# google-deepmind/spriteworld

Hardware: AMD Instinct MI355X
Metric: env-steps/sec (incl. 64x64 RGB render) at 8192 envs (higher is better)
Workload: dtype i32 fixed-point raster/resample + f64 state

## Files before the change

include/swb.h:

```cpp
#ifndef SWB_H_
#define SWB_H_

#include <stdint.h>

#ifdef __cplusplus
extern "C" {
#endif

#define SWB_MAX_SPRITES 64
#define SWB_MAX_TASKS 8
#define SWB_MAX_SHAPES 32
#define SWB_MAX_SHAPE_VERTS 64
#define SWB_MAX_CUTS 4
#define SWB_MAX_CELLS ((SWB_MAX_CUTS + 1) * (SWB_MAX_CUTS + 1))

enum swb_status {
  SWB_OK = 0,
  SWB_ERR_INVALID = -1,
  SWB_ERR_HIP = -2,
  SWB_ERR_NO_DEVICE = -3,
  SWB_ERR_STATE = -4
};

enum swb_action_space {
// ... 213 lines not shown
int swb_upload_shapes(swb_handle h, const double* verts, const int32_t* offsets, int32_t n_shapes);

int swb_upload_resample(swb_handle h, int32_t axis , int32_t out_size,
                        int32_t ksize, const int32_t* bounds, const int32_t* coeffs);

int swb_set_pool(swb_handle h, const swb_pool* pool);

int swb_sample_pool(swb_handle h, const swb_sampler* spec, int32_t n_entries, const int32_t* pool_base_host,
                    const int32_t* pool_len_host, uint64_t seed, uint64_t first_entry, void* stream);

int swb_resample_pool(swb_handle h, uint64_t seed, uint64_t first_entry, void* stream);

int swb_sample_pool_tree(swb_handle h, const swb_tree_sampler* spec, int32_t n_entries, const int32_t* pool_base_host,
                         const int32_t* pool_len_host, uint64_t seed, uint64_t first_entry, void* stream);

int swb_sampler_exhausted(swb_handle h, int64_t* sprites, void* stream);

int swb_get_pool(swb_handle h, const swb_pool* pool_host);

int swb_reset_all(swb_handle h, void* stream);

int swb_step(swb_handle h, const void* actions_dev, const swb_outputs* out, void* stream);

int swb_step_masked(swb_handle h, const void* actions_dev, const uint8_t* active_dev, const swb_outputs* out, void* stream);

int swb_reset_envs(swb_handle h, const uint8_t* mask_dev, void* stream);

int swb_render(swb_handle h, uint8_t* obs_dev, void* stream);

int swb_evaluate(swb_handle h, uint8_t* success_dev, void* stream);

typedef struct swb_rollout_outputs {
  double* reward;
  float* discount;
  uint8_t* step_type;
  uint8_t* success;
  uint8_t* error;
  double* x;
  double* y;
  int32_t* n_sprites;
} swb_rollout_outputs;
int swb_rollout(swb_handle h, const void* actions_dev, int32_t M, int32_t K, const swb_rollout_outputs* out, void* stream);

int swb_rollout_frames(swb_handle h, int32_t M, const int32_t* cand_dev, uint8_t* obs_dev, uint8_t* error_dev, void* stream);

typedef struct swb_rollout_step_outputs {
  double* x;
  double* y;
  int32_t* n_sprites;
} swb_rollout_step_outputs;
int swb_rollout_trajectory(swb_handle h, const void* actions_dev, int32_t M, int32_t K, const swb_rollout_outputs* out,
                           const swb_rollout_step_outputs* steps, void* stream);

#define SWB_ALL_STEPS (-1)
int swb_rollout_step_frames(swb_handle h, int32_t M, int32_t step, const int32_t* cand_dev, uint8_t* obs_dev, uint8_t* error_dev,
                            void* stream);

#define SWB_CONTAINED_MAX_TRIES 1024
enum swb_action_sampling { SWB_SAMPLE_UNIFORM = 0, SWB_SAMPLE_ON_SPRITE = 1 };
typedef struct swb_sampled_actions {
  void* actions;
  double* position;
  int32_t* sprite;
  int32_t* tries;
} swb_sampled_actions;
int swb_sample_actions(swb_handle h, int32_t mode, uint64_t seed, uint64_t first_env, const swb_sampled_actions* out, void* stream);

typedef struct swb_rollout_sampled_outputs {
  void*    actions;
  int32_t* sprite;
  int32_t* tries;
} swb_rollout_sampled_outputs;
int swb_rollout_sampled(swb_handle h, int32_t mode , uint64_t seed, uint64_t first_env,
                        int32_t M, int32_t K, int32_t keep_steps, const swb_rollout_outputs* out,
                        const swb_rollout_step_outputs* steps, const swb_rollout_sampled_outputs* sampled, void* stream);

int swb_trim_run_lists(swb_handle h, int32_t* run_cap_out, void* stream);

int swb_list_stats(swb_handle h, int64_t* kept, int64_t* built, void* stream);

int swb_frame_stats(swb_handle h, int64_t* copied, int64_t* filled, int64_t* resampled, void* stream);
int swb_frame_cycles(swb_handle h, int64_t* out3, void* stream);

int swb_split_stats(swb_handle h, int64_t* whole, int64_t* bands, int64_t* whole_copies, void* stream);

int swb_factors(swb_handle h, double* factors_dev, void* stream);

int swb_get_env_state(swb_handle h, int32_t env, int32_t* out5, void* stream);
int swb_get_sprite_types(swb_handle h, int32_t env, int32_t sprite, int32_t* flags, void* stream);

int swb_get_state(swb_handle h, const swb_state* host_state, void* stream);
int swb_set_positions(swb_handle h, const double* x_host, const double* y_host, void* stream);

typedef struct swb_snapshot {
  double *x, *y;
  int32_t *n_sprites, *pool_entry, *step_count, *episode, *pool_base, *pool_len;
  uint8_t *reset_next;
} swb_snapshot;
enum swb_state_source { SWB_STATE_LIVE = 0, SWB_STATE_ROLLOUT_END = 1 };
int swb_pool_id(swb_handle h, uint64_t* id);
int swb_save_state(swb_handle h, int32_t source, const int32_t* index_dev, int32_t C, const swb_snapshot* snap, void* stream);
int swb_load_state(swb_handle h, const swb_snapshot* snap, int32_t C, const int32_t* slot_dev, uint64_t pool_id,
                   int32_t* rejected_dev, void* stream);

int swb_copy_pool(swb_handle dst, swb_handle src, const int32_t* pool_base_host, const int32_t* pool_len_host, void* stream);

enum swb_sprite_attr { SWB_ATTR_SHAPE = 0, SWB_ATTR_ANGLE = 1, SWB_ATTR_SCALE = 2 };
int swb_set_sprite_attr(swb_handle h, int32_t env, int32_t sprite, int32_t attr, double value, const double* delta,
                        const int8_t* label, void* stream);

int swb_set_sprite_cell_labels(swb_handle h, int32_t env, int32_t sprite, const int8_t* cells, void* stream);

int swb_get_sprite(swb_handle h, int32_t env, int32_t sprite, int32_t* shape, double* angle, double* scale, int32_t* n_verts,
                   double* path_xy, void* stream);

int swb_sprite_path_op(int32_t attr, double a, double b, int32_t n, const double* in_xy, double* out_xy);

typedef struct swb_variant_info {
  int32_t nw;
  int32_t ncol;
  int32_t vs;
  int32_t lds_bytes_per_wave;
  int32_t waves_per_simd;
  int32_t resample_waves_per_simd;
  int32_t n_bands;
  int32_t n_column_groups;
  int32_t run_cap;
  int32_t paint_in_cover;
  int32_t arena_units;
  int32_t large_frames;
  int32_t many_sprites;
  int32_t reserved_;
  int64_t run_list_bytes;
  int64_t frame_cache_bytes;
  int32_t split_bands;
  int32_t split_pad_;
} swb_variant_info;
int swb_variant(swb_handle h, swb_variant_info* out);
const char* swb_build_id(void);

int swb_timing_enable(swb_handle h, int32_t enable);
int swb_step_time_ms(swb_handle h, double* total_ms, int64_t* launches);
int swb_kernel_times_ms(swb_handle h, double* cover_ms, double* resample_ms, int64_t* launches);

#ifdef __cplusplus
}
#endif
#endif
```

spriteworld_amd/_abi.py:

```python
import ctypes as C

SWB_MAX_SPRITES = 64
SWB_TUNED_SPRITES = 16
SWB_MAX_TASKS = 8
SWB_MAX_SHAPES = 32
SWB_MAX_SHAPE_VERTS = 64
SWB_MAX_GROUPS = 8
SWB_MAX_CUTS = 4
SWB_MAX_CELLS = (SWB_MAX_CUTS + 1) * (SWB_MAX_CUTS + 1)
SWB_MAX_CANDIDATES = 12

ACTION_SELECT_MOVE, ACTION_DRAG_AND_DROP, ACTION_EMBODIED = 0, 1, 2
TASK_NO_REWARD, TASK_FIND_GOAL, TASK_CLUSTERING = 0, 1, 2
AGG_SUM, AGG_MAX, AGG_MIN, AGG_MEAN = 0, 1, 2, 3
TERM_ALL, TERM_ANY = 0, 1
STEP_FIRST, STEP_MID, STEP_LAST = 0, 1, 2
ENV_ERR_DB_ZERO, ENV_ERR_DB_LABELS, ENV_ERR_SPAN_OVERFLOW = 1, 2, 4
ATTR_SHAPE, ATTR_ANGLE, ATTR_SCALE = 0, 1, 2
SAMPLE_UNIFORM, SAMPLE_ON_SPRITE = 0, 1
SWB_CONTAINED_MAX_TRIES = 1024


class SwbTask(C.Structure):
  _fields_ = [
# ... 67 lines not shown
      ('discount', C.c_void_p),
      ('step_type', C.c_void_p),
      ('success', C.c_void_p),
      ('error', C.c_void_p),
  ]


class SwbRolloutOutputs(C.Structure):
  _fields_ = [
      ('reward', C.c_void_p),
      ('discount', C.c_void_p),
      ('step_type', C.c_void_p),
      ('success', C.c_void_p),
      ('error', C.c_void_p),
      ('x', C.c_void_p),
      ('y', C.c_void_p),
      ('n_sprites', C.c_void_p),
  ]


class SwbRolloutStepOutputs(C.Structure):
  _fields_ = [
      ('x', C.c_void_p),
      ('y', C.c_void_p),
      ('n_sprites', C.c_void_p),
  ]


SWB_ALL_STEPS = -1


class SwbSampledActions(C.Structure):
  _fields_ = [
      ('actions', C.c_void_p),
      ('position', C.c_void_p),
      ('sprite', C.c_void_p),
      ('tries', C.c_void_p),
  ]


class SwbRolloutSampledOutputs(C.Structure):
  _fields_ = [
      ('actions', C.c_void_p),
      ('sprite', C.c_void_p),
      ('tries', C.c_void_p),
  ]


class SwbState(C.Structure):
  _fields_ = [
      ('x', C.c_void_p),
      ('y', C.c_void_p),
      ('n_sprites', C.c_void_p),
      ('pool_entry', C.c_void_p),
      ('step_count', C.c_void_p),
      ('reset_next', C.c_void_p),
      ('episode', C.c_void_p),
  ]


class SwbSnapshot(C.Structure):
  _fields_ = [
      ('x', C.c_void_p),
      ('y', C.c_void_p),
      ('n_sprites', C.c_void_p),
      ('pool_entry', C.c_void_p),
      ('step_count', C.c_void_p),
      ('episode', C.c_void_p),
      ('pool_base', C.c_void_p),
      ('pool_len', C.c_void_p),
      ('reset_next', C.c_void_p),
  ]


STATE_LIVE, STATE_ROLLOUT_END = 0, 1


class SwbVariantInfo(C.Structure):
  _fields_ = [('nw', C.c_int32), ('ncol', C.c_int32), ('vs', C.c_int32), ('lds_bytes_per_wave', C.c_int32),
              ('waves_per_simd', C.c_int32), ('resample_waves_per_simd', C.c_int32), ('n_bands', C.c_int32),
              ('n_column_groups', C.c_int32), ('run_cap', C.c_int32), ('paint_in_cover', C.c_int32),
              ('arena_units', C.c_int32), ('large_frames', C.c_int32), ('many_sprites', C.c_int32), ('reserved_', C.c_int32),
              ('run_list_bytes', C.c_int64), ('frame_cache_bytes', C.c_int64),
              ('split_bands', C.c_int32), ('split_pad_', C.c_int32)]


FACTOR_UNIFORM_F32, FACTOR_UNIFORM_INT, FACTOR_DISCRETE = 0, 1, 2


class SwbFactor(C.Structure):
  _fields_ = [
      ('kind', C.c_int32),
      ('n', C.c_int32),
      ('lo', C.c_double),
      ('hi', C.c_double),
      ('cand', C.c_double * SWB_MAX_CANDIDATES),
  ]


FACTOR_ORDER = ('x', 'y', 'scale', 'angle', 'c0', 'c1', 'c2', 'x_vel', 'y_vel')
SWB_N_FACTORS = len(FACTOR_ORDER)
SWB_MAX_HOLDOUTS = 2


class SwbHoldout(C.Structure):
  _fields_ = [
      ('redraw_mask', C.c_uint32),
      ('box_mask', C.c_uint32),
      ('lo', C.c_double * SWB_N_FACTORS),
      ('hi', C.c_double * SWB_N_FACTORS),
  ]


class SwbSpriteGroup(C.Structure):

  def factor(self, key):
    return self.factors[FACTOR_ORDER.index(key)]

  _fields_ = [
      ('count_min', C.c_int32),
      ('count_max', C.c_int32),
      ('factors', SwbFactor * SWB_N_FACTORS),
      ('n_holdouts', C.c_int32),
      ('reserved', C.c_int32),
      ('holdouts', SwbHoldout * SWB_MAX_HOLDOUTS),
      ('n_shapes', C.c_int32),
      ('shapes', C.c_int32 * SWB_MAX_CANDIDATES),
      ('cos_a', C.c_double * SWB_MAX_CANDIDATES),
      ('sin_a', C.c_double * SWB_MAX_CANDIDATES),
      ('label', C.c_int8 * SWB_MAX_TASKS),
  ]


SWB_MAX_ALTERNATIVES = 16


class SwbAlternative(C.Structure):
  _fields_ = [
      ('n', C.c_int32),
      ('group', C.c_int32 * SWB_MAX_GROUPS),
  ]


class SwbSampler(C.Structure):
  _fields_ = [
      ('n_groups', C.c_int32),
      ('shuffle', C.c_int32),
      ('color_map', C.c_int32),
      ('n_alternatives', C.c_int32),
      ('alternatives', SwbAlternative * SWB_MAX_ALTERNATIVES),
      ('deg_cos', C.c_double * 360),
      ('deg_sin', C.c_double * 360),
      ('groups', SwbSpriteGroup * SWB_MAX_GROUPS),
  ]


SWB_TREE_MAX_LEAVES, SWB_TREE_MAX_PRED_NODES, SWB_TREE_MAX_PREDS, SWB_TREE_MAX_OPS = 64, 128, 64, 128
SWB_TREE_MAX_CHOICES, SWB_TREE_MAX_STACK, SWB_TREE_MAX_CLUSTERS = 16, 32, 16
SWB_F_SHAPE = SWB_N_FACTORS
SWB_TREE_N_FACTORS = SWB_N_FACTORS + 1
TREE_FACTOR_ORDER = FACTOR_ORDER + ('shape',)
SWB_TREE_DEFAULT_MAX_TRIES = 10000
PRED_LEAF, PRED_AND, PRED_OR, PRED_ANDNOT, PRED_TRUE = 0, 1, 2, 3, 4
OP_DRAW, OP_CHOOSE, OP_JUMP, OP_TEST = 0, 1, 2, 3


class SwbTreeLeaf(C.Structure):
# ... 35 lines not shown
      ('target', C.c_int32 * SWB_MAX_CANDIDATES),
      ('cdf', C.c_double * SWB_MAX_CANDIDATES),
  ]


class SwbTreeGroup(C.Structure):
  _fields_ = [
      ('count_min', C.c_int32),
      ('count_max', C.c_int32),
      ('first_op', C.c_int32),
      ('n_ops', C.c_int32),
      ('defaults', C.c_double * SWB_TREE_N_FACTORS),
      ('default_cos', C.c_double),
      ('default_sin', C.c_double),
  ]


class SwbTreeTask(C.Structure):
  _fields_ = [
      ('kind', C.c_int32),
      ('n_preds', C.c_int32),
      ('pred', C.c_int16 * SWB_TREE_MAX_CLUSTERS),
  ]


class SwbTreeSampler(C.Structure):
  _fields_ = [
      ('n_groups', C.c_int32),
      ('shuffle', C.c_int32),
      ('color_map', C.c_int32),
      ('n_alternatives', C.c_int32),
      ('alternatives_weighted', C.c_int32),
      ('max_tries', C.c_int32),
      ('n_leaves', C.c_int32),
      ('n_pred_nodes', C.c_int32),
      ('n_preds', C.c_int32),
      ('n_ops', C.c_int32),
      ('n_choices', C.c_int32),
      ('n_tasks', C.c_int32),
      ('alternatives', SwbAlternative * SWB_MAX_ALTERNATIVES),
      ('alternative_cdf', C.c_double * SWB_MAX_ALTERNATIVES),
      ('deg_cos', C.c_double * 360),
      ('deg_sin', C.c_double * 360),
      ('groups', SwbTreeGroup * SWB_MAX_GROUPS),
      ('tasks', SwbTreeTask * SWB_MAX_TASKS),
      ('choices', SwbTreeChoice * SWB_TREE_MAX_CHOICES),
      ('preds', SwbTreePred * SWB_TREE_MAX_PREDS),
      ('pred_nodes', SwbPredNode * SWB_TREE_MAX_PRED_NODES),
      ('ops', SwbTreeOp * SWB_TREE_MAX_OPS),
      ('leaves', SwbTreeLeaf * SWB_TREE_MAX_LEAVES),
  ]


_P, _h, _p, _i32, _u64, _f64 = C.POINTER, C.c_void_p, C.c_void_p, C.c_int32, C.c_uint64, C.c_double

PROTOTYPES = {
    'swb_last_error': (C.c_char_p, []),
    'swb_version': (None, []),
    'swb_create': (None, [_P(SwbConfig), C.c_int, _P(C.c_void_p)]),
    'swb_destroy': (None, [_h]),
    'swb_upload_shapes': (None, [_h, _p, _p, _i32]),
    'swb_upload_resample': (None, [_h, _i32, _i32, _i32, _p, _p]),
    'swb_set_pool': (None, [_h, _P(SwbPool)]),
    'swb_sample_pool': (None, [_h, _P(SwbSampler), _i32, _p, _p, _u64, _u64, _h]),
    'swb_resample_pool': (None, [_h, _u64, _u64, _h]),
    'swb_sample_pool_tree': (None, [_h, _P(SwbTreeSampler), _i32, _p, _p, _u64, _u64, _h]),
    'swb_sampler_exhausted': (None, [_h, _P(C.c_int64), _h]),
    'swb_get_pool': (None, [_h, _P(SwbPool)]),
    'swb_reset_all': (None, [_h, _h]),
    'swb_step': (None, [_h, _p, _P(SwbOutputs), _h]),
    'swb_step_masked': (None, [_h, _p, _p, _P(SwbOutputs), _h]),
    'swb_reset_envs': (None, [_h, _p, _h]),
    'swb_render': (None, [_h, _p, _h]),
    'swb_evaluate': (None, [_h, _p, _h]),
    'swb_rollout': (None, [_h, _p, _i32, _i32, _P(SwbRolloutOutputs), _h]),
    'swb_rollout_frames': (None, [_h, _i32, _p, _p, _p, _h]),
    'swb_rollout_trajectory': (None, [_h, _p, _i32, _i32, _P(SwbRolloutOutputs), _P(SwbRolloutStepOutputs), _h]),
    'swb_rollout_step_frames': (None, [_h, _i32, _i32, _p, _p, _p, _h]),
    'swb_sample_actions': (None, [_h, _i32, _u64, _u64, _P(SwbSampledActions), _h]),
    'swb_rollout_sampled': (None, [_h, _i32, _u64, _u64, _i32, _i32, _i32, _P(SwbRolloutOutputs), _P(SwbRolloutStepOutputs),
                                   _P(SwbRolloutSampledOutputs), _h]),
    'swb_trim_run_lists': (None, [_h, _P(_i32), _h]),
    'swb_list_stats': (None, [_h, _P(C.c_int64), _P(C.c_int64), _h]),
    'swb_frame_stats': (None, [_h, _P(C.c_int64), _P(C.c_int64), _P(C.c_int64), _h]),
    'swb_split_stats': (None, [_h, _P(C.c_int64), _P(C.c_int64), _P(C.c_int64), _h]),
    'swb_frame_cycles': (None, [_h, _P(C.c_int64), _h]),
    'swb_factors': (None, [_h, _p, _h]),
    'swb_get_env_state': (None, [_h, _i32, _p, _h]),
    'swb_get_sprite_types': (None, [_h, _i32, _i32, _P(_i32), _h]),
    'swb_get_state': (None, [_h, _P(SwbState), _h]),
    'swb_set_positions': (None, [_h, _p, _p, _h]),
    'swb_pool_id': (None, [_h, _P(_u64)]),
    'swb_save_state': (None, [_h, _i32, _p, _i32, _P(SwbSnapshot), _h]),
    'swb_load_state': (None, [_h, _P(SwbSnapshot), _i32, _p, _u64, _p, _h]),
    'swb_copy_pool': (None, [_h, _h, _p, _p, _h]),
    'swb_set_sprite_attr': (None, [_h, _i32, _i32, _i32, _f64, _p, _p, _h]),
    'swb_set_sprite_cell_labels': (None, [_h, _i32, _i32, _p, _h]),
    'swb_get_sprite': (None, [_h, _i32, _i32, _p, _p, _p, _p, _p, _h]),
    'swb_sprite_path_op': (None, [_i32, _f64, _f64, _i32, _p, _p]),
    'swb_variant': (None, [_h, _P(SwbVariantInfo)]),
    'swb_build_id': (C.c_char_p, []),
    'swb_timing_enable': (None, [_h, _i32]),
    'swb_step_time_ms': (None, [_h, _P(_f64), _P(C.c_int64)]),
    'swb_kernel_times_ms': (None, [_h, _P(_f64), _P(_f64), _P(C.c_int64)]),
}


def declare(lib, tolerate_missing=False):
  for name, (restype, argtypes) in PROTOTYPES.items():
    if tolerate_missing and not hasattr(lib, name):
      continue
    fn = getattr(lib, name)
    fn.argtypes = argtypes
    if restype is not None:
      fn.restype = restype
  return lib


del _P, _h, _p, _i32, _u64, _f64
```

spriteworld_amd/csrc/swb.hip:

```cpp
#include <hip/hip_runtime.h>

#include <algorithm>
#include <atomic>
#include <cmath>
#include <cstdarg>
#include <cstdio>
#include <cstdlib>
#include <cstring>
#include <memory>
#include <string>
#include <vector>

#include "swb_kernels.hip.inc"
#include "swb_pow.hip.inc"
#include "swb_sampler.hip.inc"

extern template __global__ void swb_cover_kernel<20, false>(const swb_params);
extern template __global__ void swb_cover_kernel<20, true>(const swb_params);

namespace {

thread_local std::string g_err;

int fail(int code, const char* fmt, ...) {
// ... 27 lines not shown
  }
  int fill(const T* src, size_t n) {
    release();
    if (n == 0) n = 1;
    HIP_TRY(hipMalloc(reinterpret_cast<void**>(&ptr), n * sizeof(T)));
    count = n;
    if (src) HIP_TRY(hipMemcpy(ptr, src, n * sizeof(T), hipMemcpyHostToDevice));
    else HIP_TRY(hipMemset(ptr, 0, n * sizeof(T)));
    return 0;
  }
  int clone(const T* src, size_t n, hipStream_t st) {
    release();
    if (n == 0) n = 1;
    HIP_TRY(hipMalloc(reinterpret_cast<void**>(&ptr), n * sizeof(T)));
    count = n;
    HIP_TRY(hipMemcpyAsync(ptr, src, n * sizeof(T), hipMemcpyDeviceToDevice, st));
    return 0;
  }
  void swap(dev_buf& o) { std::swap(ptr, o.ptr); std::swap(count, o.count); }
};

std::atomic<uint64_t> g_pool_ids{0};
uint64_t next_pool_id() { return g_pool_ids.fetch_add(1) + 1; }

}

struct swb_engine {
  swb_config cfg;
  int device = 0;
  swb_params p;
  bool have_shapes = false, have_h = false, have_v = false, have_pool = false;
  int vslots = SWB_VSLOTS;
  int nbands = 1;
  bool tables_dirty = true;
  std::vector<int32_t> v_ymin_host, v_end_host, h_xmin_host, h_cnt_host;
  std::vector<int> shape_nverts;
  int ovf_lds_bytes = 0;
  void (*ovf_fn)(const swb_params) = nullptr;
  size_t lds_block = 0;
  dev_buf<double> d_shape_verts, d_shape_dmin;
  dev_buf<int32_t> d_shape_off;
  dev_buf<int32_t> d_h_xmin, d_h_cnt, d_h_tbl, d_h_pfx;
  dev_buf<int32_t> d_v_tab, d_v_end, d_v_pfx;
  dev_buf<int32_t> d_p_n;
  dev_buf<double> d_p_x, d_p_y, d_p_xv, d_p_yv, d_p_scale, d_p_ca, d_p_sa;
  dev_buf<int32_t> d_p_shape;
  dev_buf<uint32_t> d_p_rgb;
  dev_buf<int8_t> d_p_label;
  dev_buf<int8_t> d_p_cell_label;
  bool keyed = false;
  dev_buf<uint8_t> d_p_attr;
  dev_buf<int32_t> d_pool_base, d_pool_len;
  dev_buf<double> d_p_angle, d_p_color;
  dev_buf<swb_sampler> d_sampler;
  int pool_entries = 0;
  uint64_t pool_id = 0;
  bool pool_sampled = false, pool_uniform = false;
  dev_buf<swb_tree_dev> d_tree;
  dev_buf<unsigned long long> d_exhausted;
  bool pool_tree = false;
  dev_buf<double> d_x, d_y;
  dev_buf<int32_t> d_nspr, d_entry, d_step_count, d_episode;
  dev_buf<uint8_t> d_reset_next;
  dev_buf<uint32_t> d_ovf, d_ovf_bitmap;
  int ovf_slots = 0;
  dev_buf<uint32_t> d_cost_cnt;
  dev_buf<int32_t> d_cost_list;
  dev_buf<int32_t> d_ccost_list;
  bool cover_lists_filed = false;
  int launch_phase = 0;
  int launch_parity = 0;
  dev_buf<uint32_t> d_runs, d_rhdr, d_arena_head;
  dev_buf<int32_t> d_env_state;
  int arena_override = -1;
  int run_cap_worst = 0;
  bool lists_trimmed = false;
  bool lists_valid = false;
  uint32_t list_epoch = 1;
  bool no_keep_lists = false;
  dev_buf<unsigned long long> d_list_stats;
  dev_buf<uint8_t> d_frame_cache;
  int copy_cost = 0;
  dev_buf<unsigned long long> d_frame_stats;
  bool split_bands = false;
  dev_buf<unsigned long long> d_split_stats;
  dev_buf<int32_t> d_band_y0, d_band_first, d_band_lo, d_cg_lo, d_cg_hi;
  dev_buf<uint32_t> d_v_break;
  dev_buf<uint8_t> d_ov_flag;
  dev_buf<int32_t> d_ov_shape;
  dev_buf<double> d_ov_scale, d_ov_angle, d_ov_cpath;
  dev_buf<int8_t> d_ov_label;
  dev_buf<int8_t> d_ov_cell_label;
  bool timing = false;
  struct step_events { hipEvent_t e0, e1, e2; };
  std::vector<step_events> events;
  std::vector<step_events> event_pool;
  int cus = 0;
  bool no_paint_in_cover = false, force_cover_order = false;
  bool large_frames = false;
  bool many_sprites = false;
  size_t lf_scratch_budget = (size_t)256 << 20;
  dev_buf<int32_t> d_lf_hb, d_lf_hpo, d_lf_hp, d_lf_vb, d_lf_vk;
  int lf_vks = 0;
  dev_buf<uint8_t> d_lf_tmp;
  double timed_ms = 0.0, timed_cover_ms = 0.0;
  int64_t timed_launches = 0;
  dev_buf<unsigned char> d_rollout;
  dev_buf<swb_params> d_rollout_steps;
  int rollout_M = 0;
  bool rollout_stale = false;
  dev_buf<unsigned char> d_rollout_pick;
  dev_buf<unsigned char> d_rollout_traj;
  int rollout_kept_K = 0;
};

namespace {

typedef void (*kernel_fn)(const swb_params);

struct variant { int nw; kernel_fn fn, fn_ov, fn_paint, fn_paint_ov; size_t lds_fixed, outrow_bytes; };

template <int NW>
variant make_variant() {
  const size_t outrow = 528;
  kernel_fn paint = nullptr, paint_ov = nullptr;
  if constexpr (NW == 2) { paint = swb_cover_kernel<NW, false, true>; paint_ov = swb_cover_kernel<NW, true, true>; }
  return {NW, swb_cover_kernel<NW>, swb_cover_kernel<NW, true>, paint, paint_ov, (sizeof(wave_lds<NW>) + outrow + 15) & ~(size_t)15, outrow};
}

const variant kVariants[] = {make_variant<2>(), make_variant<4>(), make_variant<5>(), make_variant<10>(), make_variant<20>()};

const variant* pick_variant(int Wc) {
  for (const variant& v : kVariants)
    if (32 * v.nw >= Wc) return &v;
  return nullptr;
}

kernel_fn pick_resample(int AA, int vslots, int* vs_out) {
  if (AA == 1) { if (vs_out) *vs_out = 0; return swb_fill_kernel; }
  if (vslots <= 6) { if (vs_out) *vs_out = 6; return swb_resample_kernel<6>; }
  if (vs_out) *vs_out = 8;
  return swb_resample_kernel<8>;
}

size_t lds_per_wave(const swb_engine* h, const variant* v, int* cpath_in_masks) {
  const swb_params& p = h->p;
  const size_t cpath_bytes = (size_t)p.max_edges * 16;
  const int in_masks = (2 * (size_t)SWB_NWA(v->nw) * SWB_WAVE * 4 >= cpath_bytes) ? 1 : 0;
  if (cpath_in_masks) *cpath_in_masks = in_masks;
  return (v->lds_fixed + (((size_t)p.max_edges * sizeof(edge_rec) + 15) & ~(size_t)15) +
          (size_t)p.max_spans * SWB_WAVE * 4 + 15) & ~(size_t)15;
}

void bump_list_epoch(swb_engine* h) {
  if (++h->list_epoch == 0u) h->list_epoch = 1u;
}

int ensure_overflow_slots(swb_engine* h, kernel_fn fn, kernel_fn fn_alt, size_t lds_bytes) {
  if (h->d_ovf) return 0;
  int per_cu = 0;
  for (kernel_fn f : {fn, fn_alt}) {
    int n = 0;
    if (!f) continue;
    if (hipOccupancyMaxActiveBlocksPerMultiprocessor(&n, reinterpret_cast<const void*>(f), SWB_WAVE, lds_bytes) != hipSuccess || n < 1)
      n = 32;
    per_cu = std::max(per_cu, n);
  }
  long long slots = (long long)per_cu * h->cus;
  slots = std::min<long long>(2 * slots, (long long)h->p.N);
  slots = (slots + 31) / 32 * 32;
  h->ovf_slots = (int)slots;
  if (h->d_ovf.fill(nullptr, (size_t)slots * 64 * h->p.ovf_cap) || h->d_ovf_bitmap.fill(nullptr, (size_t)slots / 32)) return SWB_ERR_HIP;
  h->p.ovf = h->d_ovf; h->p.ovf_bitmap = h->d_ovf_bitmap; h->p.ovf_slots = h->ovf_slots;
  return 0;
}

int ensure_handoff_tables(swb_engine* h, bool need_lists = true) {
  if (!h->tables_dirty && (h->d_runs || !need_lists)) return 0;
  bump_list_epoch(h);
  swb_params& p = h->p;
  int nb = h->nbands;
  int vs = 0;
  (void)pick_resample(p.AA, h->vslots, &vs);
  auto first_in_flight = [&](int o_lo) {
    int f = o_lo;
    while (f > 0 && h->v_end_host[f - 1] >= h->v_ymin_host[o_lo]) --f;
    return f;
  };
  std::vector<int32_t> blo(1, 0);
  for (int b = 1; b < nb; ++b) {
    int want = (int)((long long)b * p.Ho / nb), best = -1;
    if (p.AA == 1) best = want;
    else
      for (int d = 0; d < p.Ho && best < 0; ++d)
        for (int c : {want + d, want - d})
          if (c > blo.back() && c < p.Ho && first_in_flight(c) % vs == 0) { best = c; break; }
    if (best > blo.back() && best < p.Ho) blo.push_back(best);
  }
  nb = (int)blo.size();
  blo.push_back(p.Ho);
  p.nbands = nb;
  std::vector<int32_t> y0(nb, 0), first(nb, 0), lo(p.ncg, 0), hi(p.ncg, 0);
  const size_t brk_words = (size_t)(p.Hc + 31) / 32 + 3;
  std::vector<uint32_t> brk(2 * brk_words, 0u);
  auto set_break = [&](int y) { if (y >= 0 && y < p.Hc) brk[y >> 5] |= 1u << (y & 31); };
  for (int b = 0; b < nb; ++b) {
    const int o_lo = blo[b];
    if (p.AA == 1) { y0[b] = o_lo; first[b] = o_lo; }
    else { y0[b] = h->v_ymin_host[o_lo]; first[b] = first_in_flight(o_lo); }
    set_break(y0[b]);
    if (y0[b] >= 0 && y0[b] < p.Hc) brk[brk_words + (y0[b] >> 5)] |= 1u << (y0[b] & 31);
  }
  if (p.AA != 1)
    for (int o = 0; o < p.Ho; ++o) set_break(h->v_end_host[o] + 1);
  for (int g = 0; g < p.ncg; ++g) {
    if (p.AA == 1) { lo[g] = 64 * g; hi[g] = std::min(64 * g + 64, p.Wo); continue; }
    lo[g] = 1 << 30; hi[g] = 0;
    for (int o = 64 * g; o < std::min(64 * g + 64, p.Wo); ++o) {
      lo[g] = std::min(lo[g], h->h_xmin_host[o]);
      hi[g] = std::max(hi[g], h->h_xmin_host[o] + h->h_cnt_host[o]);
    }
  }
  if (h->d_band_y0.fill(y0.data(), y0.size()) || h->d_band_first.fill(first.data(), first.size()) ||
      h->d_band_lo.fill(blo.data(), blo.size()) || h->d_v_break.fill(brk.data(), brk.size()) ||
      h->d_cg_lo.fill(lo.data(), lo.size()) || h->d_cg_hi.fill(hi.data(), hi.size()))
    return SWB_ERR_HIP;
  p.band_lo = h->d_band_lo;
  p.band_y0 = h->d_band_y0; p.band_first = h->d_band_first; p.v_break = h->d_v_break; p.cg_lo = h->d_cg_lo; p.cg_hi = h->d_cg_hi;
  if (!h->d_runs && need_lists) {
    const size_t fixed = (size_t)p.N * p.ncg * p.run_cap;
    size_t arena = std::max(h->lists_trimmed ? fixed / 2 : (size_t)0, (size_t)16 * h->run_cap_worst);
    if (h->arena_override >= 0) arena = (size_t)h->arena_override;
    const size_t units = fixed + arena + 4;
    if (units * 8 >= ((size_t)1 << 32))
      return fail(SWB_ERR_INVALID, "run lists of %zu MB (%d environments x %d column groups x %d units + an arena of %zu units) exceed "
                  "the 4 GB a list position can address: step fewer environments per engine", units * 8 >> 20, p.N, p.ncg, p.run_cap, arena);
    size_t free_b = 0, total_b = 0;
    if (hipMemGetInfo(&free_b, &total_b) == hipSuccess && units * 8 + (size_t)p.N * SWB_RHDR_DWORDS * 4 > free_b)
      return fail(SWB_ERR_HIP, "run lists need %zu MB of device memory (%d environments x %d column groups x %d units of 8 bytes + an "
                  "arena of %zu units), %zu MB are free", units * 8 >> 20, p.N, p.ncg, p.run_cap, arena, free_b >> 20);
    if (h->d_runs.fill(nullptr, units * 2) || h->d_rhdr.fill(nullptr, (size_t)p.N * SWB_RHDR_DWORDS) || h->d_arena_head.fill(nullptr, 2))
      return SWB_ERR_HIP;
    p.runs = h->d_runs; p.rhdr = h->d_rhdr;
    p.arena_head = h->d_arena_head;
    p.arena_base = (int64_t)fixed;
    p.arena_units = (int32_t)std::min(arena, (size_t)0x7fffffff);
  }
  h->tables_dirty = false;
  return 0;
}

int drop_run_lists(swb_engine* h) {
  if (!h->d_runs) return 0;
  HIP_TRY(hipDeviceSynchronize());
  h->d_runs.release(); h->d_rhdr.release(); h->d_arena_head.release();
  h->p.runs = nullptr; h->p.rhdr = nullptr; h->p.arena_head = nullptr;
  bump_list_epoch(h);
  h->lists_valid = false;
  h->tables_dirty = true;
  return 0;
}

int restore_run_list_reservation(swb_engine* h) {
  if (!h->lists_trimmed) return 0;
  if (int rc = drop_run_lists(h)) return rc;
  h->lists_trimmed = false;
  if (!getenv("SWB_RUN_CAP")) h->p.run_cap = h->run_cap_worst;
  return 0;
}

int flush_timing(swb_engine* h) {
  for (auto& ev : h->events) {
    HIP_TRY(hipEventSynchronize(ev.e2));
    float ms = 0.f, ms_cover = 0.f;
    HIP_TRY(hipEventElapsedTime(&ms, ev.e0, ev.e2));
    HIP_TRY(hipEventElapsedTime(&ms_cover, ev.e0, ev.e1));
    h->timed_ms += ms;
    h->timed_cover_ms += ms_cover;
    h->timed_launches += 1;
    h->event_pool.push_back(ev);
  }
  h->events.clear();
  return 0;
}


int check_ready(const swb_engine* h, const void* actions, int render_only) {
  if (!h->have_shapes) return fail(SWB_ERR_STATE, "swb_upload_shapes has not been called");
  if (!h->have_pool) return fail(SWB_ERR_STATE, "swb_set_pool has not been called");
  if (h->p.AA != 1 && !(h->have_h && h->have_v))
    return fail(SWB_ERR_STATE, "swb_upload_resample (both axes) is required when anti_aliasing > 1");
  if (!render_only && actions == nullptr) return fail(SWB_ERR_INVALID, "actions is NULL");
  return 0;
}

swb_params bind_step(const swb_engine* h, const void* actions, const swb_outputs* out, int render_only, const uint8_t* active) {
  swb_params p = h->p;
  p.actions = actions;
  p.active = active;
  p.obs = out ? out->obs : nullptr;
  p.reward = out ? out->reward : nullptr;
  p.discount = out ? out->discount : nullptr;
  p.step_type = out ? out->step_type : nullptr;
  p.success = out ? out->success : nullptr;
  p.error = out ? out->error : nullptr;
  p.render_only = render_only;
  return p;
}

void bind_view(swb_params* p, const swb_state_view* view) {
  if (!view) return;
  p->x = view->x; p->y = view->y; p->nspr = view->nspr; p->entry = view->entry; p->step_count = view->step_count;
  p->episode = view->episode; p->pool_base = view->pool_base; p->pool_len = view->pool_len; p->reset_next = view->reset_next;
}

int cover_launch_config(const swb_engine* h, const variant* v, kernel_fn fn, swb_params* p, size_t* lds_out) {
  int cpath_in_masks = 0;
  const size_t lds = lds_per_wave(h, v, &cpath_in_masks);
  p->cpath_in_masks = cpath_in_masks;
  p->lds_per_wave = (int32_t)lds;
  p->outrow_bytes = (int32_t)v->outrow_bytes;
  if (lds > 160 * 1024) return fail(SWB_ERR_INVALID, "LDS request %zu B exceeds 160 KiB", lds);
  if (lds > 64 * 1024)
    HIP_TRY(hipFuncSetAttribute(reinterpret_cast<const void*>(fn), hipFuncAttributeMaxDynamicSharedMemorySize, (int)lds));
  *lds_out = lds;
  return 0;
}

struct step_timer {
  swb_engine* h;
  hipStream_t stream;
  swb_engine::step_events ev = {nullptr, nullptr, nullptr};
  bool held = false;
  step_timer(swb_engine* h_, hipStream_t stream_) : h(h_), stream(stream_) {}
  ~step_timer() { if (held) h->event_pool.push_back(ev); }
  int begin() {
    if (!h->timing) return 0;
    if (!h->event_pool.empty()) { ev = h->event_pool.back(); h->event_pool.pop_back(); }
    else
      for (hipEvent_t* e : {&ev.e0, &ev.e1, &ev.e2}) HIP_TRY(hipEventCreate(e));
    held = true;
    HIP_TRY(hipEventRecord(ev.e0, stream));
    return 0;
  }
  int mid() {
    if (held) HIP_TRY(hipEventRecord(ev.e1, stream));
    return 0;
  }
  int end(bool counted) {
    if (!held) return 0;
    HIP_TRY(hipEventRecord(ev.e2, stream));
    if (!counted) return 0;
    held = false;
    h->events.push_back(ev);
    return h->events.size() >= 4096 ? flush_timing(h) : 0;
  }
};

bool paints_in_cover(const swb_engine* h, const variant* v, bool honour_switch = true) {
  return h->p.AA == 1 && h->p.ncg == 1 && v && v->fn_paint && !(honour_switch && h->no_paint_in_cover);
}

int launch_large(swb_engine* h, const void* actions, const swb_outputs* out, int render_only, hipStream_t stream,
                 const swb_state_view* view, const uint8_t* active);

int launch(swb_engine* h, const void* actions, const swb_outputs* out, int render_only, hipStream_t stream,
           const swb_state_view* view = nullptr, const uint8_t* active = nullptr) {
  if (h->large_frames) return launch_large(h, actions, out, render_only, stream, view, active);
  if (int rc = check_ready(h, actions, render_only)) return rc;
  const variant* v = pick_variant(h->p.Wc);
  if (!v) return fail(SWB_ERR_INVALID, "canvas %dx%d not supported", h->p.Wc, h->p.Hc);
  if (int rc = ensure_handoff_tables(h, !paints_in_cover(h, v))) return rc;
  int vs = 0;
  const kernel_fn fn2 = pick_resample(h->p.AA, h->vslots, &vs);
  swb_params p = bind_step(h, actions, out, render_only, active);
  bind_view(&p, view);
  if (p.v_tab && vs == 8) {
    p.v_tab += (size_t)p.Hc * SWB_VSLOTS;
    p.v_pfx += (size_t)(p.Hc + 1) * SWB_VSLOTS;
  }
  const bool paint = p.obs && paints_in_cover(h, v);
  const kernel_fn fn = paint ? (h->d_ov_flag ? v->fn_paint_ov : v->fn_paint) : (h->d_ov_flag ? v->fn_ov : v->fn);
  size_t lds = 0;
  if (int rc = cover_launch_config(h, v, fn, &p, &lds)) return rc;
  const kernel_fn fn_family = h->d_ov_flag ? v->fn_ov : v->fn;
  if (!h->d_ovf || (int)lds < h->ovf_lds_bytes || fn_family != h->ovf_fn) {
    if (h->d_ovf) {
      HIP_TRY(hipDeviceSynchronize());
      h->d_ovf.release(); h->d_ovf_bitmap.release();
    }
    if (int rc = ensure_overflow_slots(h, fn_family, h->d_ov_flag ? v->fn_paint_ov : v->fn_paint, lds)) return rc;
    bump_list_epoch(h);
    h->ovf_lds_bytes = (int)lds;
    h->ovf_fn = fn_family;
    p.ovf = h->p.ovf; p.ovf_bitmap = h->p.ovf_bitmap; p.ovf_slots = h->p.ovf_slots;
  }
// ... 398 lines not shown
      return fail(SWB_ERR_INVALID, "task %d: between 0 and %d position thresholds per axis supported", t, SWB_MAX_CUTS);
    for (int k = 1; k < tk.n_xcuts; ++k) if (!(tk.xcuts[k - 1] < tk.xcuts[k])) return fail(SWB_ERR_INVALID, "task %d: xcuts must ascend", t);
    for (int k = 1; k < tk.n_ycuts; ++k) if (!(tk.ycuts[k - 1] < tk.ycuts[k])) return fail(SWB_ERR_INVALID, "task %d: ycuts must ascend", t);
    if (tk.n_xcuts + tk.n_ycuts > 0) h->keyed = true;
  }
  {
    const char* lf = getenv("SWB_LARGE_FRAMES");
    const char* ms = getenv("SWB_MANY_SPRITES");
    h->many_sprites = p.S > SWB_TUNED_SPRITES || (ms && atoi(ms) != 0);
    h->large_frames = !pick_variant(p.Wc) || p.Wo > 64 * SWB_MAX_CG || (lf && atoi(lf) != 0) || h->many_sprites;
    if (const char* x = getenv("SWB_LF_SCRATCH_BYTES")) h->lf_scratch_budget = (size_t)std::max(1ll, atoll(x));
  }
  if (h->large_frames) {
    if (p.Wc > SWB_LF_MAX_CANVAS || p.Hc > SWB_LF_MAX_CANVAS)
      return fail(SWB_ERR_INVALID, "canvas %dx%d too large: at most %d px in either direction (anti_aliasing * image_size)", p.Wc, p.Hc,
                  SWB_LF_MAX_CANVAS);
    if (p.Wo > SWB_LF_MAX_COLUMNS) return fail(SWB_ERR_INVALID, "image width %d too large: at most %d columns", p.Wo, SWB_LF_MAX_COLUMNS);
  } else if (p.Hc > 65535) {
    return fail(SWB_ERR_INVALID, "canvas %dx%d too large", p.Wc, p.Hc);
  }
  const int ncg = (p.Wo + 63) / 64;
  if (!h->large_frames) p.ncg = ncg;
  const int cus = std::max(h->cus, 1);
  {
    const long long resident = (long long)cus * 4 * SWB_RS_WAVES_PER_SIMD;
    const long long tasks = (long long)p.N * ncg;
    int nb = 1;
    while (nb < SWB_MAX_BANDS && tasks * nb < resident && (p.Ho / (2 * nb) >= 16 || (p.Ho / (2 * nb) >= 8 && tasks * nb * 2 <= resident))) nb *= 2;
    if (const char* x = getenv("SWB_BANDS")) nb = std::max(1, std::min(atoi(x), (int)SWB_MAX_BANDS));
    h->nbands = std::min(nb, p.Ho);
    const bool cache_wanted = p.AA != 1 && !h->large_frames && !h->no_keep_lists && !getenv("SWB_NO_FRAME_CACHE");
    const bool cost_ordered = !getenv("SWB_NO_COST_ORDER") && p.N < (1 << 24) && !h->large_frames;
    int split = (nb == 1 && tasks <= 2 * resident && p.action_space != SWB_ACTION_EMBODIED) ? SWB_SPLIT_BANDS_DEFAULT : 0;
    if (const char* x = getenv("SWB_SPLIT_BANDS")) split = atoi(x) >= 2 ? std::min(atoi(x), (int)SWB_MAX_BANDS) : 0;
    if (getenv("SWB_BANDS") || !cache_wanted || !cost_ordered || std::min(split, p.Ho) < 2) split = 0;
    if (split) {
      h->split_bands = true;
      h->nbands = std::min(split, p.Ho);
      p.split_bands = 1;
      p.split_when = 2 * cus * 4;
      if (const char* x = getenv("SWB_SPLIT_WHEN")) p.split_when = (int32_t)std::max(0ll, std::min(atoll(x), 0x7fffffffll));
    }
  }
  const long long rs_waves = (long long)p.N * ncg * (h->split_bands ? 1 : h->nbands);
  p.cost_range0 = std::max(8 * p.Hc, SWB_KEY_BUCKETS_FITTED);
  if (!getenv("SWB_NO_COST_ORDER") && p.N < (1 << 24) && !h->large_frames) {
    p.band_tasks = (h->nbands > 1 && rs_waves >= 4ll * cus * 4 && !getenv("SWB_NO_BAND_TASKS")) ? 1 : 0;
    if (const char* x = getenv("SWB_BAND_TASKS")) p.band_tasks = (h->nbands > 1 && atoi(x) != 0) ? 1 : 0;
    if (h->split_bands) p.band_tasks = 1;
    p.cost_cap = ncg * ((p.N + SWB_COST_SHARDS - 1) / SWB_COST_SHARDS) * (p.band_tasks ? h->nbands : 1);
    std::vector<uint32_t> cnt0(5 * SWB_COST_SET + SWB_COST_WORDS, 0u);
    for (int par = 0; par < 2; ++par) cnt0[SWB_COST_WORD_SPLIT(par)] = (h->split_bands && p.split_when > 0 && (long long)p.N * ncg <= p.split_when) ? 1u : 0u;
    for (int ph = 0; ph < 3; ++ph) cnt0[SWB_COST_WORD_COVER_SHIFT(ph)] = 12;
    for (int par = 0; par < 2; ++par) {
      cnt0[SWB_COST_WORD_KEY_LO(par)] = 0u;
      cnt0[SWB_COST_WORD_KEY_RANGE(par)] = (uint32_t)p.cost_range0;
      cnt0[SWB_COST_WORD_KEY_SCALE(par)] = (uint32_t)(((unsigned long long)SWB_KEY_BUCKETS_FITTED << 16) / (uint32_t)p.cost_range0);
    }
    p.prio_div = 4;
    if (const char* x = getenv("SWB_PRIO_DIV")) p.prio_div = std::max(1, atoi(x));
    p.prio_levels = (!getenv("SWB_NO_PRIO") && rs_waves <= 2ll * cus * 4 * SWB_RS_WAVES_PER_SIMD) ? 1 : 0;
    if (!getenv("SWB_NO_COVER_PRIO")) p.prio_levels |= 2;
    const size_t ccap = (size_t)(p.N + SWB_COST_SHARDS - 1) / SWB_COST_SHARDS;
    if (h->d_cost_cnt.fill(cnt0.data(), cnt0.size()) ||
        h->d_ccost_list.fill(nullptr, (size_t)3 * SWB_COST_SHARDS * SWB_COST_BUCKETS * ccap) ||
        h->d_cost_list.fill(nullptr, (size_t)2 * SWB_COST_SHARDS * SWB_COST_BUCKETS * p.cost_cap))
      return SWB_ERR_HIP;
    p.cost_cnt = h->d_cost_cnt; p.cost_list = h->d_cost_list;
    if (!getenv("SWB_NO_COVER_ORDER")) p.ccost_list = h->d_ccost_list;
    const int per_xcd = h->cus / SWB_COST_SHARDS;
    if (per_xcd >= 2 && (per_xcd & (per_xcd - 1)) == 0 && rs_waves <= (long long)h->cus * 4 * SWB_RS_WAVES_PER_SIMD && !getenv("SWB_NO_SNAKE"))
      while ((1 << p.deal_shift) < per_xcd) ++p.deal_shift;
    if (const char* x = getenv("SWB_DEAL_SHIFT")) p.deal_shift = std::max(0, atoi(x));
  }
  h->run_cap_worst = std::max(4, p.S + 1) * p.Hc + 1;
  p.run_cap = h->run_cap_worst;
  if (const char* x = getenv("SWB_RUN_CAP")) p.run_cap = std::max(8, atoi(x));
  if (const char* x = getenv("SWB_ARENA_UNITS")) h->arena_override = std::max(0, atoi(x));
  const size_t NS = (size_t)p.N * p.S;
  if (h->d_x.fill(nullptr, NS) || h->d_y.fill(nullptr, NS) || h->d_nspr.fill(nullptr, p.N) || h->d_entry.fill(nullptr, p.N) ||
      h->d_step_count.fill(nullptr, p.N) || h->d_episode.fill(nullptr, p.N) || h->d_reset_next.fill(nullptr, p.N))
    return SWB_ERR_HIP;
  if (getenv("SWB_LIST_STATS")) {
    if (h->d_list_stats.fill(nullptr, 2) || h->d_frame_stats.fill(nullptr, 6)) return SWB_ERR_HIP;
    p.list_stats = h->d_list_stats;
    p.frame_stats = h->d_frame_stats;
    if (h->split_bands) {
      if (h->d_split_stats.fill(nullptr, 3)) return SWB_ERR_HIP;
      p.split_stats = h->d_split_stats;
    }
  }
  h->copy_cost = h->split_bands ? SWB_SPLIT_COPY_COST : SWB_COPY_COST;
  if (const char* x = getenv("SWB_COPY_COST")) h->copy_cost = std::max(0, atoi(x));
  if (p.AA != 1 && !h->large_frames && !h->no_keep_lists && !getenv("SWB_NO_FRAME_CACHE")) {
    const size_t bytes = (size_t)p.N * p.Wo * p.Ho * 3;
    if (hipMalloc(reinterpret_cast<void**>(&h->d_frame_cache.ptr), bytes) == hipSuccess) {
      h->d_frame_cache.count = bytes;
      p.frame_cache = h->d_frame_cache;
    } else {
      h->d_frame_cache.ptr = nullptr;
      (void)hipGetLastError();
    }
  }
  p.max_spans = SWB_MIN_SPANS;
  if (const char* ms = getenv("SWB_MAX_SPANS")) p.max_spans = atoi(ms) < SWB_MIN_SPANS ? SWB_MIN_SPANS : atoi(ms);
  p.span_cap = p.max_spans;
  if (const char* sc = getenv("SWB_LDS_SPAN_CAP")) p.span_cap = std::max(0, std::min(atoi(sc), p.max_spans));
  p.ovf_cap = std::min(p.Wc / 2 + 1, 32);
  p.ovf = nullptr;
  p.x = h->d_x; p.y = h->d_y; p.nspr = h->d_nspr; p.entry = h->d_entry; p.step_count = h->d_step_count;
  p.episode = h->d_episode; p.reset_next = h->d_reset_next;
  *out = owner.release();
  return SWB_OK;
}

int swb_destroy(swb_handle h) {
  if (!h) return SWB_OK;
  (void)hipSetDevice(h->device);
  for (auto* list : {&h->events, &h->event_pool})
    for (auto& ev : *list) { (void)hipEventDestroy(ev.e0); (void)hipEventDestroy(ev.e1); (void)hipEventDestroy(ev.e2); }
  delete h;
  return SWB_OK;
}

int swb_upload_shapes(swb_handle h, const double* verts, const int32_t* offsets, int32_t n_shapes) {
  if (!h || !verts || !offsets) return fail(SWB_ERR_INVALID, "null argument");
  bump_list_epoch(h);
  if (n_shapes < 1 || n_shapes > SWB_MAX_SHAPES) return fail(SWB_ERR_INVALID, "n_shapes must be in [1, %d]", SWB_MAX_SHAPES);
  HIP_TRY(hipSetDevice(h->device));
  int maxv = 0;
  for (int i = 0; i < n_shapes; ++i) {
    const int n = offsets[i + 1] - offsets[i];
    if (n < 3 || n > SWB_MAX_SHAPE_VERTS) return fail(SWB_ERR_INVALID, "shape %d has %d vertices (3..%d supported)", i, n, SWB_MAX_SHAPE_VERTS);
    if (n > maxv) maxv = n;
  }
  std::vector<double> dmin(n_shapes, 0.0);
  for (int i = 0; i < n_shapes; ++i) {
    double best = 1e300;
    for (int a = offsets[i]; a < offsets[i + 1]; ++a)
      for (int b = a + 1; b < offsets[i + 1]; ++b)
        best = std::min(best, std::hypot(verts[2 * a] - verts[2 * b], verts[2 * a + 1] - verts[2 * b + 1]));
    dmin[i] = best;
  }
  dmin.resize(SWB_MAX_SHAPES, 0.0);
  std::vector<int32_t> off_padded(offsets, offsets + n_shapes + 1);
  off_padded.resize(SWB_MAX_SHAPES + 1, offsets[n_shapes]);
  if (h->d_shape_dmin.fill(dmin.data(), dmin.size())) return SWB_ERR_HIP;
  h->p.shape_dmin = h->d_shape_dmin;
  if (h->d_shape_verts.fill(verts, (size_t)offsets[n_shapes] * 2)) return SWB_ERR_HIP;
  if (h->d_shape_off.fill(off_padded.data(), off_padded.size())) return SWB_ERR_HIP;
  h->p.shape_verts = h->d_shape_verts;
  h->p.shape_off = h->d_shape_off;
  h->p.max_verts = maxv;
  h->p.max_edges = maxv * h->p.S;
  h->shape_nverts.resize(n_shapes);
  for (int i = 0; i < n_shapes; ++i) h->shape_nverts[i] = offsets[i + 1] - offsets[i];
  h->have_shapes = true;
  return SWB_OK;
}

int swb_upload_resample(swb_handle h, int32_t axis, int32_t out_size, int32_t ksize, const int32_t* bounds,
                        const int32_t* coeffs) {
  if (!h || !bounds || !coeffs) return fail(SWB_ERR_INVALID, "null argument");
  bump_list_epoch(h);
  HIP_TRY(hipSetDevice(h->device));
  if (h->large_frames) return upload_resample_large(h, axis, out_size, ksize, bounds, coeffs);
  const swb_params& p = h->p;
  if (axis == 0) {
    if (out_size != p.Wo) return fail(SWB_ERR_INVALID, "horizontal table has %d outputs, image width is %d", out_size, p.Wo);
    std::vector<int32_t> xmin(out_size), cnt(out_size), tbl(out_size), pfx;
    std::vector<std::vector<int32_t>> uniq;
    std::vector<int32_t> uniq_off;
    for (int o = 0; o < out_size; ++o) {
      xmin[o] = bounds[2 * o]; cnt[o] = bounds[2 * o + 1];
      if (cnt[o] < 0 || cnt[o] > ksize || xmin[o] < 0 || xmin[o] + cnt[o] > p.Wc)
        return fail(SWB_ERR_INVALID, "bad horizontal bounds at %d", o);
      std::vector<int32_t> v(cnt[o] + 1, 0);
      for (int j = 0; j < cnt[o]; ++j) v[j + 1] = v[j] + coeffs[(size_t)o * ksize + j];
      int found = -1;
      for (size_t u = 0; u < uniq.size(); ++u) if (uniq[u] == v) { found = (int)u; break; }
      if (found < 0) { found = (int)uniq.size(); uniq.push_back(v); uniq_off.push_back((int32_t)pfx.size()); pfx.insert(pfx.end(), v.begin(), v.end()); }
      tbl[o] = uniq_off[found];
    }
    if (pfx.size() * 4 > 32 * 1024) return fail(SWB_ERR_INVALID, "horizontal prefix table too large (%zu entries)", pfx.size());
    if (h->d_h_xmin.fill(xmin.data(), xmin.size()) || h->d_h_cnt.fill(cnt.data(), cnt.size()) ||
        h->d_h_tbl.fill(tbl.data(), tbl.size()) || h->d_h_pfx.fill(pfx.data(), pfx.size()))
      return SWB_ERR_HIP;
    h->p.h_xmin = h->d_h_xmin; h->p.h_cnt = h->d_h_cnt; h->p.h_tbl = h->d_h_tbl; h->p.h_pfx = h->d_h_pfx;
    h->p.h_pfx_len = (int32_t)pfx.size();
    h->h_xmin_host = xmin; h->h_cnt_host = cnt;
    h->tables_dirty = true;
    h->have_h = true;
  } else if (axis == 1) {
    if (out_size != p.Ho) return fail(SWB_ERR_INVALID, "vertical table has %d outputs, image height is %d", out_size, p.Ho);
    const size_t tab_len = (size_t)p.Hc * SWB_VSLOTS;
    std::vector<int32_t> vend(out_size), vtab(2 * tab_len, 0);
    for (int r = 0; r < out_size; ++r) {
      const int ymin = bounds[2 * r], c = bounds[2 * r + 1];
      if (c < 1 || c > ksize || ymin < 0 || ymin + c > p.Hc) return fail(SWB_ERR_INVALID, "bad vertical bounds at %d", r);
      vend[r] = ymin + c - 1;
      if (r > 0 && (vend[r] < vend[r - 1] || ymin < bounds[2 * (r - 1)])) return fail(SWB_ERR_INVALID, "vertical windows are not monotone");
    }
    int used = 1;
    for (int y = 0; y < p.Hc; ++y) {
      int rf = 0;
      while (rf < out_size && vend[rf] < y) ++rf;
      for (int r = 0; r < out_size; ++r) {
        const int ymin = bounds[2 * r];
        if (y < ymin || y > vend[r]) continue;
        const int k = r - rf;
        if (k < 0 || k >= SWB_VSLOTS) return fail(SWB_ERR_INVALID, "more than %d output rows in flight at canvas row %d", SWB_VSLOTS, y);
        const int32_t cf = coeffs[(size_t)r * ksize + (y - ymin)];
        vtab[(size_t)y * SWB_VSLOTS + (r % 6)] = cf;
        vtab[tab_len + (size_t)y * SWB_VSLOTS + (r % 8)] = cf;
        if (k + 1 > used) used = k + 1;
      }
    }
    const size_t pfx_len = (size_t)(p.Hc + 1) * SWB_VSLOTS;
    std::vector<int32_t> vpfx(2 * pfx_len, 0);
    for (int t = 0; t < 2; ++t)
      for (int y = 0; y < p.Hc; ++y)
        for (int k = 0; k < SWB_VSLOTS; ++k)
          vpfx[t * pfx_len + (size_t)(y + 1) * SWB_VSLOTS + k] =
              vpfx[t * pfx_len + (size_t)y * SWB_VSLOTS + k] + vtab[t * tab_len + (size_t)y * SWB_VSLOTS + k];
    std::vector<int32_t> vend_padded(vend);
    vend_padded.push_back(0x7fffffff); vend_padded.push_back(0x7fffffff);
    if (h->d_v_tab.fill(vtab.data(), vtab.size()) || h->d_v_end.fill(vend_padded.data(), vend_padded.size()) ||
        h->d_v_pfx.fill(vpfx.data(), vpfx.size()))
      return SWB_ERR_HIP;
    h->p.v_tab = h->d_v_tab; h->p.v_end = h->d_v_end; h->p.v_pfx = h->d_v_pfx;
    h->vslots = used;
    h->v_end_host = vend;
    h->v_ymin_host.resize(out_size);
    for (int r = 0; r < out_size; ++r) h->v_ymin_host[r] = bounds[2 * r];
    h->tables_dirty = true;
    h->have_v = true;
  } else {
    return fail(SWB_ERR_INVALID, "axis must be 0 or 1");
  }
  return SWB_OK;
}

int swb_set_pool(swb_handle h, const swb_pool* pool) {
  if (!h || !pool) return fail(SWB_ERR_INVALID, "null argument");
  bump_list_epoch(h);
  HIP_TRY(hipSetDevice(h->device));
  const int P = pool->n_entries, S = h->p.S, T = h->p.n_tasks, N = h->p.N;
  if (P < 1) return fail(SWB_ERR_INVALID, "pool is empty");
  for (int i = 0; i < P; ++i)
    if (pool->n_sprites[i] < 0 || pool->n_sprites[i] > S) return fail(SWB_ERR_INVALID, "pool entry %d has %d sprites (max %d)", i, pool->n_sprites[i], S);
  for (int i = 0; i < N; ++i)
    if (pool->pool_len[i] < 1 || pool->pool_base[i] < 0 || pool->pool_base[i] + pool->pool_len[i] > P)
      return fail(SWB_ERR_INVALID, "env %d: pool range [%d, +%d) outside the pool of %d", i, pool->pool_base[i], pool->pool_len[i], P);
  const size_t PS = (size_t)P * S;
  int most_verts = -1;
  if (h->have_shapes) {
    int most = 1;
    for (int e = 0; e < P; ++e) {
      int tot = 0;
      for (int s2 = 0; s2 < pool->n_sprites[e]; ++s2) {
        const int sh = pool->shape[(size_t)e * S + s2];
        if (sh < 0 || sh >= (int)h->shape_nverts.size()) return fail(SWB_ERR_INVALID, "pool entry %d uses shape %d, %zu shapes uploaded", e, sh, h->shape_nverts.size());
        tot += h->shape_nverts[sh];
      }
      most = std::max(most, tot);
    }
    most_verts = (most + 3) & ~3;
    if (int rc = lf_check_vertices(h, most_verts, "swb_set_pool")) return rc;
  }
  std::vector<uint32_t> rgb(PS);
  for (size_t i = 0; i < PS; ++i)
    rgb[i] = (uint32_t)pool->rgb[4 * i] | ((uint32_t)pool->rgb[4 * i + 1] << 8) | ((uint32_t)pool->rgb[4 * i + 2] << 16);
  for (size_t i = 0; i < PS; ++i)
    if (pool->shape[i] < 0 || (h->have_shapes && pool->shape[i] >= SWB_MAX_SHAPES)) return fail(SWB_ERR_INVALID, "bad shape index in pool");
  int rc = 0;
  h->rollout_stale = true;
  h->pool_id = next_pool_id();
  rc |= h->d_p_n.fill(pool->n_sprites, P);
  rc |= h->d_p_x.fill(pool->x, PS); rc |= h->d_p_y.fill(pool->y, PS);
  rc |= h->d_p_xv.fill(pool->x_vel, PS); rc |= h->d_p_yv.fill(pool->y_vel, PS);
  rc |= h->d_p_scale.fill(pool->scale, PS); rc |= h->d_p_ca.fill(pool->cos_a, PS); rc |= h->d_p_sa.fill(pool->sin_a, PS);
  rc |= h->d_p_shape.fill(pool->shape, PS);
  rc |= h->d_p_rgb.fill(rgb.data(), PS);
  rc |= h->d_p_label.fill(pool->label, (size_t)P * T * S);
  if (h->keyed) {
    if (!pool->cell_label) return fail(SWB_ERR_INVALID, "a task of this handle keys on position (swb_task::n_xcuts / n_ycuts): swb_pool::cell_label is required");
    rc |= h->d_p_cell_label.fill(pool->cell_label, (size_t)P * T * S * SWB_MAX_CELLS);
  }
  rc |= h->d_p_attr.fill(pool->attr_f32, PS);
  rc |= h->d_pool_base.fill(pool->pool_base, N);
  rc |= h->d_pool_len.fill(pool->pool_len, N);
  if (pool->angle) rc |= h->d_p_angle.fill(pool->angle, PS);
  if (pool->color) rc |= h->d_p_color.fill(pool->color, PS * 3);
  if (rc) return SWB_ERR_HIP;
  bind_pool(h, pool->angle != nullptr, pool->color != nullptr);
  h->pool_entries = P;
  h->pool_sampled = false;
  if (most_verts > 0) h->p.max_edges = most_verts;
  HIP_TRY(hipMemset(h->d_reset_next, 1, N));
  HIP_TRY(hipMemset(h->d_episode, 0, sizeof(int32_t) * N));
  HIP_TRY(hipMemset(h->d_step_count, 0, sizeof(int32_t) * N));
  h->have_pool = true;
  if (int rc2 = restore_run_list_reservation(h)) return rc2;
  return SWB_OK;
}

int swb_sample_pool(swb_handle h, const swb_sampler* spec, int32_t n_entries, const int32_t* pool_base_host,
                    const int32_t* pool_len_host, uint64_t seed, uint64_t first_entry, void* stream) {
  if (!h || !spec || !pool_base_host || !pool_len_host) return fail(SWB_ERR_INVALID, "null argument");
  bump_list_epoch(h);
  HIP_TRY(hipSetDevice(h->device));
  const int P = n_entries, S = h->p.S, N = h->p.N;
  if (P < 1) return fail(SWB_ERR_INVALID, "pool is empty");
  if (h->keyed) return fail(SWB_ERR_INVALID, "a task of this handle keys on position: its labels depend on where a sprite is drawn -- sample such "
                            "generators on the host (swb_set_pool with swb_pool::cell_label)");
  if (spec->n_groups < 1 || spec->n_groups > SWB_MAX_GROUPS) return fail(SWB_ERR_INVALID, "n_groups must be in [1, %d]", SWB_MAX_GROUPS);
  if (spec->shuffle < 0) return fail(SWB_ERR_INVALID, "shuffle must be >= 0");
  if (spec->n_alternatives < 0 || spec->n_alternatives > SWB_MAX_ALTERNATIVES)
    return fail(SWB_ERR_INVALID, "n_alternatives must be in [0, %d]", SWB_MAX_ALTERNATIVES);
  for (int i = 0; i < spec->n_alternatives; ++i) {
    const swb_alternative& alt = spec->alternatives[i];
    if (alt.n < 1 || alt.n > SWB_MAX_GROUPS) return fail(SWB_ERR_INVALID, "alternative %d: 1..%d groups", i, SWB_MAX_GROUPS);
    for (int g = 0; g < alt.n; ++g)
      if (alt.group[g] < 0 || alt.group[g] >= spec->n_groups) return fail(SWB_ERR_INVALID, "alternative %d: bad group index", i);
  }
  int max_total = 0;
  for (int g = 0; g < spec->n_groups; ++g) {
    const swb_sprite_group& grp = spec->groups[g];
    if (grp.count_min < 0 || grp.count_max < grp.count_min) return fail(SWB_ERR_INVALID, "group %d: bad sprite count range", g);
    if (grp.n_shapes < 1 || grp.n_shapes > SWB_MAX_CANDIDATES)
      return fail(SWB_ERR_INVALID, "group %d: 1..%d shape candidates", g, SWB_MAX_CANDIDATES);
    for (const swb_factor* f = grp.factors; f != grp.factors + SWB_N_FACTORS; ++f) {
      if (f->kind < SWB_FACTOR_UNIFORM_F32 || f->kind > SWB_FACTOR_DISCRETE) return fail(SWB_ERR_INVALID, "group %d: bad factor kind", g);
      if (f->kind == SWB_FACTOR_DISCRETE && (f->n < 1 || f->n > SWB_MAX_CANDIDATES))
        return fail(SWB_ERR_INVALID, "group %d: Discrete factors take 1..%d candidates", g, SWB_MAX_CANDIDATES);
    }
    if (grp.factors[SWB_F_X].kind != SWB_FACTOR_UNIFORM_F32 || grp.factors[SWB_F_Y].kind != SWB_FACTOR_UNIFORM_F32)
      return fail(SWB_ERR_INVALID, "group %d: x and y must be float32 Continuous factors", g);
    const swb_factor& ang = grp.factors[SWB_F_ANGLE];
    if (ang.kind == SWB_FACTOR_UNIFORM_F32 ||
        (ang.kind == SWB_FACTOR_UNIFORM_INT && !(ang.lo >= 0.0 && ang.hi <= 360.0 && ang.lo <= ang.hi)))
      return fail(SWB_ERR_INVALID, "group %d: angle must be Discrete or integer degrees within [0, 360]", g);
    if (grp.n_holdouts < 0 || grp.n_holdouts > SWB_MAX_HOLDOUTS) return fail(SWB_ERR_INVALID, "group %d: at most %d hold-outs", g, SWB_MAX_HOLDOUTS);
    for (int i = 0; i < grp.n_holdouts; ++i)
      if (grp.holdouts[i].box_mask == 0 || (grp.holdouts[i].box_mask & ~grp.holdouts[i].redraw_mask) ||
          (grp.holdouts[i].redraw_mask >> SWB_N_FACTORS))
        return fail(SWB_ERR_INVALID, "group %d: hold-out keys must be a non-empty subset of the redrawn keys", g);
    if (spec->color_map == 1 && (grp.factors[SWB_F_C0].kind == SWB_FACTOR_UNIFORM_INT || grp.factors[SWB_F_C1].kind == SWB_FACTOR_UNIFORM_INT ||
                                 grp.factors[SWB_F_C2].kind == SWB_FACTOR_UNIFORM_INT))
      return fail(SWB_ERR_INVALID, "group %d: hsv colours must be float factors", g);
    for (int i = 0; i < grp.n_shapes; ++i)
      if (grp.shapes[i] < 0 || grp.shapes[i] >= SWB_MAX_SHAPES) return fail(SWB_ERR_INVALID, "group %d: bad shape index", g);
    max_total += grp.count_max;
  }
  if (spec->n_alternatives > 0) {
    max_total = 0;
    for (int i = 0; i < spec->n_alternatives; ++i) {
      int tot = 0;
      for (int g = 0; g < spec->alternatives[i].n; ++g) tot += spec->groups[spec->alternatives[i].group[g]].count_max;
      if (tot > max_total) max_total = tot;
    }
  }
  if (max_total > S) return fail(SWB_ERR_INVALID, "sampler can emit %d sprites (max_sprites %d)", max_total, S);
  if (h->have_shapes) {
    auto group_verts = [&](const swb_sprite_group& grp) {
      int mv = 0;
      for (int i = 0; i < grp.n_shapes; ++i)
        if (grp.shapes[i] < (int)h->shape_nverts.size()) mv = std::max(mv, h->shape_nverts[grp.shapes[i]]);
      return mv * grp.count_max;
    };
    int most = 0;
    if (spec->n_alternatives > 0) {
      for (int i = 0; i < spec->n_alternatives; ++i) {
        int tot = 0;
        for (int g = 0; g < spec->alternatives[i].n; ++g) tot += group_verts(spec->groups[spec->alternatives[i].group[g]]);
        most = std::max(most, tot);
      }
    } else {
      for (int g = 0; g < spec->n_groups; ++g) most += group_verts(spec->groups[g]);
    }
    if (int rc = lf_check_vertices(h, (std::max(most, 1) + 3) & ~3, "swb_sample_pool")) return rc;
    h->p.max_edges = (std::max(most, 1) + 3) & ~3;
  }
  for (int i = 0; i < N; ++i)
    if (pool_len_host[i] < 1 || pool_base_host[i] < 0 || pool_base_host[i] + pool_len_host[i] > P)
      return fail(SWB_ERR_INVALID, "env %d: pool range [%d, +%d) outside the pool of %d", i, pool_base_host[i], pool_len_host[i], P);
  if (alloc_sampled_pool(h, P, pool_base_host, pool_len_host) || h->d_sampler.fill(spec, 1)) return SWB_ERR_HIP;
  const swb_sampler_args a = sampler_args(h, seed, first_entry, false);
  hipStream_t st = (hipStream_t)stream;
  hipLaunchKernelGGL(swb_sample_pool_kernel, dim3((P + 255) / 256), dim3(256), 0, st, a);
  HIP_TRY(hipGetLastError());
  h->pool_tree = false;
  return finish_sampled_pool(h, pool_base_host, pool_len_host, st);
}

int swb_resample_pool(swb_handle h, uint64_t seed, uint64_t first_entry, void* stream) {
  if (!h) return fail(SWB_ERR_INVALID, "null handle");
  bump_list_epoch(h);
  if (!h->have_pool || !h->pool_sampled) return fail(SWB_ERR_STATE, "swb_sample_pool has not been called");
  if (!h->pool_uniform)
    return fail(SWB_ERR_STATE, "swb_resample_pool needs the env-major layout pool_base[n] = n * pool_len, equal pool_len");
  HIP_TRY(hipSetDevice(h->device));
  h->rollout_stale = true;
  h->pool_id = next_pool_id();
  if (h->pool_tree) return launch_tree_sampler(h, seed, first_entry, true, (hipStream_t)stream);
  const swb_sampler_args a = sampler_args(h, seed, first_entry, true);
  hipLaunchKernelGGL(swb_sample_pool_kernel, dim3((h->pool_entries + 255) / 256), dim3(256), 0, (hipStream_t)stream, a);
  HIP_TRY(hipGetLastError());
  return SWB_OK;
}

int swb_sample_pool_tree(swb_handle h, const swb_tree_sampler* spec, int32_t n_entries, const int32_t* pool_base_host,
                         const int32_t* pool_len_host, uint64_t seed, uint64_t first_entry, void* stream) {
  if (!h || !spec || !pool_base_host || !pool_len_host) return fail(SWB_ERR_INVALID, "null argument");
  bump_list_epoch(h);
  HIP_TRY(hipSetDevice(h->device));
  const int P = n_entries, S = h->p.S, N = h->p.N;
  if (P < 1) return fail(SWB_ERR_INVALID, "pool is empty");
  if (!h->cfg.pos_is_f32) return fail(SWB_ERR_INVALID, "the device sampler draws float32 positions (swb_config::pos_is_f32)");
  if (int rc = check_tree_sampler(h, spec)) return rc;
  auto over_lists = [&](auto per_group) {
    int most = 0;
    if (spec->n_alternatives > 0) {
      for (int i = 0; i < spec->n_alternatives; ++i) {
        int tot = 0;
        for (int g = 0; g < spec->alternatives[i].n; ++g) tot += per_group(spec->groups[spec->alternatives[i].group[g]]);
        most = std::max(most, tot);
      }
    } else {
      for (int g = 0; g < spec->n_groups; ++g) most += per_group(spec->groups[g]);
    }
    return most;
  };
  const int max_total = over_lists([](const swb_tree_group& grp) { return grp.count_max; });
  if (max_total > S) return fail(SWB_ERR_INVALID, "sampler can emit %d sprites (max_sprites %d)", max_total, S);
  if (h->have_shapes) {
    auto verts_of = [&](double shape) { return (int)shape < (int)h->shape_nverts.size() ? h->shape_nverts[(int)shape] : 0; };
    const int most = over_lists([&](const swb_tree_group& grp) {
      int mv = 0;
      bool drawn = false;
      for (int pc = grp.first_op; pc < grp.first_op + grp.n_ops; ++pc) {
        if (spec->ops[pc].kind != SWB_OP_DRAW || spec->leaves[spec->ops[pc].a].factor != SWB_F_SHAPE) continue;
        const swb_tree_leaf& lf = spec->leaves[spec->ops[pc].a];
        for (int i = 0; i < lf.n; ++i) mv = std::max(mv, verts_of(lf.cand[i]));
        drawn = true;
      }
      if (!drawn) mv = verts_of(grp.defaults[SWB_F_SHAPE]);
      return mv * grp.count_max;
    });
    if (int rc = lf_check_vertices(h, (std::max(most, 1) + 3) & ~3, "swb_sample_pool_tree")) return rc;
    h->p.max_edges = (std::max(most, 1) + 3) & ~3;
  }
  for (int i = 0; i < N; ++i)
    if (pool_len_host[i] < 1 || pool_base_host[i] < 0 || pool_base_host[i] + pool_len_host[i] > P)
      return fail(SWB_ERR_INVALID, "env %d: pool range [%d, +%d) outside the pool of %d", i, pool_base_host[i], pool_len_host[i], P);
  auto dev = std::make_unique<swb_tree_dev>();
  memset(dev.get(), 0, sizeof(swb_tree_dev));
  dev->spec = *spec;
  for (int t = 0; t < h->p.n_tasks; ++t) {
    const swb_task& tk = h->cfg.tasks[t];
    dev->n_xcuts[t] = tk.n_xcuts; dev->n_ycuts[t] = tk.n_ycuts;
    for (int k = 0; k < SWB_MAX_CUTS; ++k) { dev->xcuts[t][k] = tk.xcuts[k]; dev->ycuts[t][k] = tk.ycuts[k]; }
  }
  if (alloc_sampled_pool(h, P, pool_base_host, pool_len_host) || h->d_tree.fill(dev.get(), 1) ||
      (!h->d_exhausted && h->d_exhausted.fill(nullptr, 1)))
    return SWB_ERR_HIP;
  hipStream_t st = (hipStream_t)stream;
  if (int rc = launch_tree_sampler(h, seed, first_entry, false, st)) return rc;
  h->pool_tree = true;
  return finish_sampled_pool(h, pool_base_host, pool_len_host, st);
}

int swb_sampler_exhausted(swb_handle h, int64_t* sprites, void* stream) {
  if (!h || !sprites) return fail(SWB_ERR_INVALID, "null argument");
  *sprites = 0;
  if (!h->d_exhausted) return SWB_OK;
  HIP_TRY(hipSetDevice(h->device));
  HIP_TRY(hipStreamSynchronize((hipStream_t)stream));
  unsigned long long n = 0;
  HIP_TRY(hipMemcpy(&n, h->d_exhausted, sizeof(n), hipMemcpyDeviceToHost));
  *sprites = (int64_t)n;
  return SWB_OK;
}

int swb_get_pool(swb_handle h, const swb_pool* pool) {
  if (!h || !pool) return fail(SWB_ERR_INVALID, "null argument");
  if (!h->have_pool) return fail(SWB_ERR_STATE, "no pool on the device");
  if (pool->n_entries != h->pool_entries) return fail(SWB_ERR_INVALID, "pool has %d entries, not %d", h->pool_entries, pool->n_entries);
  HIP_TRY(hipSetDevice(h->device));
  HIP_TRY(hipDeviceSynchronize());
  const int P = h->pool_entries, S = h->p.S, T = h->p.n_tasks, N = h->p.N;
  const size_t PS = (size_t)P * S;
#define SWB_D2H(dst, src, count) \
  if (dst) HIP_TRY(hipMemcpy((void*)(dst), (src), (count) * sizeof(*(src)), hipMemcpyDeviceToHost))
  SWB_D2H(pool->n_sprites, h->d_p_n, (size_t)P);
  SWB_D2H(pool->x, h->d_p_x, PS); SWB_D2H(pool->y, h->d_p_y, PS);
  SWB_D2H(pool->x_vel, h->d_p_xv, PS); SWB_D2H(pool->y_vel, h->d_p_yv, PS);
  SWB_D2H(pool->scale, h->d_p_scale, PS); SWB_D2H(pool->cos_a, h->d_p_ca, PS); SWB_D2H(pool->sin_a, h->d_p_sa, PS);
// ... 272 lines not shown
    const swb_state_view picked = rollout_state_view(h->d_rollout_pick.ptr, (size_t)nk * N, S);
    hipLaunchKernelGGL(swb_rollout_pick_steps_kernel, dim3((unsigned)(((size_t)nk * N * S + 255) / 256)), dim3(256), 0, st, traj, scratch,
                       picked, cand_dev, (int)N, (int)S, (int)M, k0, nk);
    HIP_TRY(hipGetLastError());
    for (size_t kk = 0; kk < (size_t)nk; ++kk) {
      const swb_state_view chunk = advanced(picked, kk * N, kk * N, S);
      out.obs = obs_dev + kk * N * frame;
      out.error = error_dev ? error_dev + kk * N : nullptr;
      if (int rc = launch(h, nullptr, &out, 1, st, &chunk)) return rc;
    }
    return SWB_OK;
  }
  for (size_t c = 0; c < (size_t)M; ++c) {
    const swb_state_view chunk = advanced(traj, (size_t)step * NV + c * N, c * N, S);
    out.obs = obs_dev + c * N * frame;
    out.error = error_dev ? error_dev + c * N : nullptr;
    if (int rc = launch(h, nullptr, &out, 1, st, &chunk)) return rc;
  }
  return SWB_OK;
}

int swb_sample_actions(swb_handle h, int32_t mode, uint64_t seed, uint64_t first_env, const swb_sampled_actions* out, void* stream) {
  if (!h) return fail(SWB_ERR_INVALID, "null handle");
  if (mode != SWB_SAMPLE_UNIFORM && mode != SWB_SAMPLE_ON_SPRITE) return fail(SWB_ERR_INVALID, "swb_sample_actions: unknown mode %d", mode);
  if (!out || (!out->actions && !out->position && !out->sprite && !out->tries))
    return fail(SWB_ERR_INVALID, "swb_sample_actions: every output is NULL");
  if (mode == SWB_SAMPLE_UNIFORM && (out->position || out->sprite || out->tries))
    return fail(SWB_ERR_INVALID, "swb_sample_actions: position, sprite and tries are outputs of SWB_SAMPLE_ON_SPRITE only");
  if (mode == SWB_SAMPLE_ON_SPRITE) {
    if (!h->have_shapes) return fail(SWB_ERR_STATE, "swb_upload_shapes has not been called");
    if (!h->have_pool) return fail(SWB_ERR_STATE, "swb_set_pool has not been called");
  }
  HIP_TRY(hipSetDevice(h->device));
  swb_sample_actions_args a;
  memset(&a, 0, sizeof(a));
  a.mode = mode; a.seed = seed; a.first_env = first_env;
  a.actions = out->actions; a.position = out->position; a.sprite = out->sprite; a.tries = out->tries;
  hipLaunchKernelGGL(swb_sample_actions_kernel, dim3((unsigned)h->p.N), dim3(SWB_WAVE), SWB_MAX_SHAPE_VERTS * sizeof(double2),
                     (hipStream_t)stream, h->p, a);
  HIP_TRY(hipGetLastError());
  return SWB_OK;
}

int swb_trim_run_lists(swb_handle h, int32_t* run_cap_out, void* stream) {
  if (!h) return fail(SWB_ERR_INVALID, "null handle");
  HIP_TRY(hipSetDevice(h->device));
  if (h->large_frames) {
    if (run_cap_out) *run_cap_out = 0;
    return SWB_OK;
  }
  if (run_cap_out) *run_cap_out = h->p.run_cap;
  if (h->lists_trimmed || getenv("SWB_RUN_CAP") || getenv("SWB_NO_TRIM")) return SWB_OK;
  if (!h->d_runs && paints_in_cover(h, pick_variant(h->p.Wc), false)) return SWB_OK;
  if (!h->d_runs || !h->lists_valid) return fail(SWB_ERR_STATE, "swb_trim_run_lists: the last launch listed no runs (step or render first)");
  HIP_TRY(hipStreamSynchronize((hipStream_t)stream));
  const swb_params& p = h->p;
  std::vector<uint32_t> hdr((size_t)p.N * SWB_RHDR_DWORDS);
  HIP_TRY(hipMemcpy(hdr.data(), h->d_rhdr, hdr.size() * 4, hipMemcpyDeviceToHost));
  uint32_t longest = 0;
  for (int n = 0; n < p.N; ++n)
    for (int g = 0; g < p.ncg; ++g) longest = std::max(longest, hdr[(size_t)n * SWB_RHDR_DWORDS + SWB_RHDR_GROUPS + g * SWB_RHDR_GSTRIDE]);
  if (longest >= (uint32_t)p.run_cap) return SWB_OK;
  const int want = std::max(p.Hc / 2, (int)(longest + longest / 4 + 16)) + 1;
  if (want >= p.run_cap) return SWB_OK;
  if (int rc = drop_run_lists(h)) return rc;
  h->p.run_cap = want;
  h->lists_trimmed = true;
  if (int rc = ensure_handoff_tables(h)) return rc;
  if (run_cap_out) *run_cap_out = h->p.run_cap;
  return SWB_OK;
}

int swb_list_stats(swb_handle h, int64_t* kept, int64_t* built, void* stream) {
  if (!h || !kept || !built) return fail(SWB_ERR_INVALID, "null argument");
  if (!h->d_list_stats) return fail(SWB_ERR_STATE, "swb_list_stats: SWB_LIST_STATS was not set when the handle was created");
  HIP_TRY(hipSetDevice(h->device));
  HIP_TRY(hipStreamSynchronize((hipStream_t)stream));
  unsigned long long w[2] = {0ull, 0ull};
  HIP_TRY(hipMemcpy(w, h->d_list_stats, sizeof(w), hipMemcpyDeviceToHost));
  *kept = (int64_t)w[0]; *built = (int64_t)w[1];
  return SWB_OK;
}

int swb_frame_stats(swb_handle h, int64_t* copied, int64_t* filled, int64_t* resampled, void* stream) {
  if (!h || !copied || !filled || !resampled) return fail(SWB_ERR_INVALID, "null argument");
  if (!h->d_frame_stats) return fail(SWB_ERR_STATE, "swb_frame_stats: SWB_LIST_STATS was not set when the handle was created");
  HIP_TRY(hipSetDevice(h->device));
  HIP_TRY(hipStreamSynchronize((hipStream_t)stream));
  unsigned long long w[3] = {0ull, 0ull, 0ull};
  HIP_TRY(hipMemcpy(w, h->d_frame_stats, sizeof(w), hipMemcpyDeviceToHost));
  *copied = (int64_t)w[0]; *filled = (int64_t)w[1]; *resampled = (int64_t)w[2];
  return SWB_OK;
}

int swb_split_stats(swb_handle h, int64_t* whole, int64_t* bands, int64_t* whole_copies, void* stream) {
  if (!h || !whole || !bands || !whole_copies) return fail(SWB_ERR_INVALID, "null argument");
  if (!h->d_split_stats)
    return fail(SWB_ERR_STATE, "swb_split_stats: the handle is not in split-bands mode, or SWB_LIST_STATS was not set when it was created");
  HIP_TRY(hipSetDevice(h->device));
  HIP_TRY(hipStreamSynchronize((hipStream_t)stream));
  unsigned long long w[3] = {0ull, 0ull, 0ull};
  HIP_TRY(hipMemcpy(w, h->d_split_stats, sizeof(w), hipMemcpyDeviceToHost));
  *whole = (int64_t)w[0]; *bands = (int64_t)w[1]; *whole_copies = (int64_t)w[2];
  return SWB_OK;
}

int swb_frame_cycles(swb_handle h, int64_t* out3, void* stream) {
  if (!h || !out3) return fail(SWB_ERR_INVALID, "null argument");
  if (!h->d_frame_stats) return fail(SWB_ERR_STATE, "swb_frame_cycles: SWB_LIST_STATS was not set when the handle was created");
  HIP_TRY(hipSetDevice(h->device));
  HIP_TRY(hipStreamSynchronize((hipStream_t)stream));
  unsigned long long w[3] = {0ull, 0ull, 0ull};
  HIP_TRY(hipMemcpy(w, h->d_frame_stats + 3, sizeof(w), hipMemcpyDeviceToHost));
  for (int i = 0; i < 3; ++i) out3[i] = (int64_t)w[i];
  return SWB_OK;
}

int swb_factors(swb_handle h, double* factors_dev, void* stream) {
  if (!h || !factors_dev) return fail(SWB_ERR_INVALID, "null argument");
  if (!h->have_pool) return fail(SWB_ERR_STATE, "swb_set_pool has not been called");
  HIP_TRY(hipSetDevice(h->device));
  const int total = h->p.N * h->p.S;
  hipLaunchKernelGGL(swb_factors_kernel, dim3((total + 255) / 256), dim3(256), 0, (hipStream_t)stream, h->p, factors_dev);
  HIP_TRY(hipGetLastError());
  return SWB_OK;
}

int swb_get_state(swb_handle h, const swb_state* st, void* stream) {
  if (!h || !st) return fail(SWB_ERR_INVALID, "null argument");
  HIP_TRY(hipSetDevice(h->device));
  HIP_TRY(hipStreamSynchronize((hipStream_t)stream));
  const size_t N = h->p.N, NS = N * h->p.S;
  if (st->x) HIP_TRY(hipMemcpy(st->x, h->d_x, NS * 8, hipMemcpyDeviceToHost));
  if (st->y) HIP_TRY(hipMemcpy(st->y, h->d_y, NS * 8, hipMemcpyDeviceToHost));
  if (st->n_sprites) HIP_TRY(hipMemcpy(st->n_sprites, h->d_nspr, N * 4, hipMemcpyDeviceToHost));
  if (st->pool_entry) HIP_TRY(hipMemcpy(st->pool_entry, h->d_entry, N * 4, hipMemcpyDeviceToHost));
  if (st->step_count) HIP_TRY(hipMemcpy(st->step_count, h->d_step_count, N * 4, hipMemcpyDeviceToHost));
  if (st->reset_next) HIP_TRY(hipMemcpy(st->reset_next, h->d_reset_next, N, hipMemcpyDeviceToHost));
  if (st->episode) HIP_TRY(hipMemcpy(st->episode, h->d_episode, N * 4, hipMemcpyDeviceToHost));
  return SWB_OK;
}

int swb_get_env_state(swb_handle h, int32_t env, int32_t* out5, void* stream) {
  if (!h || !out5) return fail(SWB_ERR_INVALID, "null argument");
  if (env < 0 || env >= h->p.N) return fail(SWB_ERR_INVALID, "environment %d out of range", env);
  HIP_TRY(hipSetDevice(h->device));
  if (!h->d_env_state && h->d_env_state.fill(nullptr, 8)) return SWB_ERR_HIP;
  hipLaunchKernelGGL(swb_env_state_kernel, dim3(1), dim3(64), 0, (hipStream_t)stream, h->p, env, h->d_env_state);
  HIP_TRY(hipGetLastError());
  HIP_TRY(hipMemcpyAsync(out5, h->d_env_state, 5 * sizeof(int32_t), hipMemcpyDeviceToHost, (hipStream_t)stream));
  HIP_TRY(hipStreamSynchronize((hipStream_t)stream));
  return SWB_OK;
}

int swb_get_sprite_types(swb_handle h, int32_t env, int32_t sprite, int32_t* flags, void* stream) {
  if (!h || !flags) return fail(SWB_ERR_INVALID, "null argument");
  if (!h->have_pool) return fail(SWB_ERR_STATE, "no pool on the device");
  if (env < 0 || env >= h->p.N) return fail(SWB_ERR_INVALID, "environment %d out of range", env);
  if (sprite < 0 || sprite >= h->p.S) return fail(SWB_ERR_INVALID, "sprite %d out of range", sprite);
  HIP_TRY(hipSetDevice(h->device));
  HIP_TRY(hipStreamSynchronize((hipStream_t)stream));
  int32_t en = 0;
  uint8_t f = 0;
  HIP_TRY(hipMemcpy(&en, h->d_entry + env, 4, hipMemcpyDeviceToHost));
  if (en < 0 || en >= h->pool_entries) return fail(SWB_ERR_STATE, "environment %d has not been reset yet", env);
  HIP_TRY(hipMemcpy(&f, h->d_p_attr + (size_t)en * h->p.S + sprite, 1, hipMemcpyDeviceToHost));
  *flags = f;
  return SWB_OK;
}

int swb_set_positions(swb_handle h, const double* x_host, const double* y_host, void* stream) {
  if (!h || !x_host || !y_host) return fail(SWB_ERR_INVALID, "null argument");
  bump_list_epoch(h);
  HIP_TRY(hipSetDevice(h->device));
  HIP_TRY(hipStreamSynchronize((hipStream_t)stream));
  const size_t NS = (size_t)h->p.N * h->p.S;
  HIP_TRY(hipMemcpy(h->d_x, x_host, NS * 8, hipMemcpyHostToDevice));
  HIP_TRY(hipMemcpy(h->d_y, y_host, NS * 8, hipMemcpyHostToDevice));
  return SWB_OK;
}

static swb_state_view live_state_view(swb_engine* h) {
  swb_state_view v;
  v.x = h->d_x; v.y = h->d_y; v.nspr = h->d_nspr; v.entry = h->d_entry; v.step_count = h->d_step_count; v.episode = h->d_episode;
  v.pool_base = h->d_pool_base; v.pool_len = h->d_pool_len; v.reset_next = h->d_reset_next;
  return v;
}

static int check_snapshot_call(swb_handle h, const char* name, const swb_snapshot* snap, int32_t C, swb_state_view* v) {
  if (!h) return fail(SWB_ERR_INVALID, "%s: null handle", name);
  if (!snap) return fail(SWB_ERR_INVALID, "%s: snapshot is NULL", name);
  if (!snap->x || !snap->y || !snap->n_sprites || !snap->pool_entry || !snap->step_count || !snap->episode || !snap->pool_base ||
      !snap->pool_len || !snap->reset_next)
    return fail(SWB_ERR_INVALID, "%s: a pointer of the snapshot is NULL (every array is required)", name);
  if (C < 1) return fail(SWB_ERR_INVALID, "%s: C must be positive (C = %d)", name, C);
  if ((long long)C * h->p.S > 0x7fffffffll)
    return fail(SWB_ERR_INVALID, "%s: C x max_sprites = %d x %d does not fit an int (the slots are indexed with one)", name, C, h->p.S);
  v->x = snap->x; v->y = snap->y; v->nspr = snap->n_sprites; v->entry = snap->pool_entry; v->step_count = snap->step_count;
  v->episode = snap->episode; v->pool_base = snap->pool_base; v->pool_len = snap->pool_len; v->reset_next = snap->reset_next;
  return 0;
}

int swb_pool_id(swb_handle h, uint64_t* id) {
  if (!h || !id) return fail(SWB_ERR_INVALID, "swb_pool_id: null argument");
  *id = h->have_pool ? h->pool_id : 0;
  return SWB_OK;
}

int swb_save_state(swb_handle h, int32_t source, const int32_t* index_dev, int32_t C, const swb_snapshot* snap, void* stream) {
  swb_state_view dst;
  if (int rc = check_snapshot_call(h, "swb_save_state", snap, C, &dst)) return rc;
  if (source != SWB_STATE_LIVE && source != SWB_STATE_ROLLOUT_END) return fail(SWB_ERR_INVALID, "swb_save_state: unknown source %d", source);
  if (!h->have_pool) return fail(SWB_ERR_STATE, "swb_save_state: swb_set_pool has not been called");
  if (h->d_ov_flag)
    return fail(SWB_ERR_STATE, "swb_save_state: sprite setters have been called on this handle; snapshots under live overrides are not supported");
  long long n_src = h->p.N;
  swb_state_view src = live_state_view(h);
  if (source == SWB_STATE_ROLLOUT_END) {
    if (!h->rollout_M) return fail(SWB_ERR_STATE, "swb_save_state: no rollout has run on this handle (swb_rollout first)");
    if (h->rollout_stale)
      return fail(SWB_ERR_STATE, "swb_save_state: the pool has changed since the last rollout (swb_set_pool, swb_sample_pool or "
                  "swb_resample_pool): its candidates may sit in entries that have been redrawn; roll out again");
    n_src = (long long)h->p.N * h->rollout_M;
    src = rollout_state_view(h->d_rollout.ptr, (size_t)n_src, (size_t)h->p.S);
  }
  if (!index_dev && C != n_src)
    return fail(SWB_ERR_INVALID, "swb_save_state: index is NULL (slot c takes element c) but C = %d and the source has %lld", C, n_src);
  HIP_TRY(hipSetDevice(h->device));
  const size_t threads = (size_t)C * h->p.S;
  hipLaunchKernelGGL(swb_state_save_kernel, dim3((unsigned)((threads + 255) / 256)), dim3(256), 0, (hipStream_t)stream, src, dst,
                     index_dev, (int)C, (int)h->p.S, (int)n_src);
  HIP_TRY(hipGetLastError());
  return SWB_OK;
}

int swb_load_state(swb_handle h, const swb_snapshot* snap, int32_t C, const int32_t* slot_dev, uint64_t pool_id,
                   int32_t* rejected_dev, void* stream) {
  swb_state_view src;
  if (int rc = check_snapshot_call(h, "swb_load_state", snap, C, &src)) return rc;
  if (!slot_dev && C != h->p.N)
    return fail(SWB_ERR_INVALID, "swb_load_state: slot is NULL (environment n takes slot n) but C = %d and the handle has %d environments",
                C, h->p.N);
  if (!h->have_pool) return fail(SWB_ERR_STATE, "swb_load_state: swb_set_pool has not been called");
  if (h->d_ov_flag)
    return fail(SWB_ERR_STATE, "swb_load_state: sprite setters have been called on this handle; snapshots under live overrides are not supported");
  if (pool_id != 0 && pool_id != h->pool_id)
    return fail(SWB_ERR_STATE, "swb_load_state: the snapshot was saved under pool %llu, the handle holds pool %llu (a pool call since "
                "may have redrawn the entries it plays; pool_id = 0 skips the check)", (unsigned long long)pool_id,
                (unsigned long long)h->pool_id);
  HIP_TRY(hipSetDevice(h->device));
  uint32_t* const rhdr = h->d_rhdr ? h->d_rhdr.ptr : nullptr;
  h->pool_uniform = false;
  const size_t threads = (size_t)h->p.N * h->p.S;
  hipLaunchKernelGGL(swb_state_load_kernel, dim3((unsigned)((threads + 255) / 256)), dim3(256), 0, (hipStream_t)stream, src,
                     live_state_view(h), slot_dev, (int)C, (int)h->p.N, (int)h->p.S, rhdr, rejected_dev);
  HIP_TRY(hipGetLastError());
  return SWB_OK;
}

int swb_copy_pool(swb_handle dst, swb_handle src, const int32_t* pool_base_host, const int32_t* pool_len_host, void* stream) {
  if (!dst || !src || !pool_base_host || !pool_len_host) return fail(SWB_ERR_INVALID, "swb_copy_pool: null argument");
  if (dst == src) return fail(SWB_ERR_INVALID, "swb_copy_pool: dst and src are the same handle");
  if (dst->device != src->device || dst->p.S != src->p.S || dst->p.n_tasks != src->p.n_tasks || dst->p.pos_is_f32 != src->p.pos_is_f32 ||
      dst->keyed != src->keyed)
    return fail(SWB_ERR_INVALID, "swb_copy_pool: the handles differ (device %d / %d, max_sprites %d / %d, n_tasks %d / %d, pos_is_f32 %d / %d, "
                "a task keys on position %d / %d)", dst->device, src->device, dst->p.S, src->p.S, dst->p.n_tasks, src->p.n_tasks,
                dst->p.pos_is_f32, src->p.pos_is_f32, (int)dst->keyed, (int)src->keyed);
  if (!src->have_pool) return fail(SWB_ERR_STATE, "swb_copy_pool: src has no pool (swb_set_pool has not been called on it)");
  if (dst->d_ov_flag || src->d_ov_flag)
    return fail(SWB_ERR_STATE, "swb_copy_pool: sprite setters have been called on one of the handles; snapshots under live overrides are not supported");
  const int P = src->pool_entries, N = dst->p.N;
  for (int i = 0; i < N; ++i)
    if (pool_len_host[i] < 1 || pool_base_host[i] < 0 || pool_base_host[i] + pool_len_host[i] > P)
      return fail(SWB_ERR_INVALID, "swb_copy_pool: env %d: pool range [%d, +%d) outside the pool of %d", i, pool_base_host[i], pool_len_host[i], P);
  const int verts = src->have_shapes ? src->p.max_edges : 0;
  if (verts > 0)
    if (int rc = lf_check_vertices(dst, verts, "swb_copy_pool")) return rc;
  HIP_TRY(hipSetDevice(dst->device));
  const hipStream_t st = (hipStream_t)stream;
  dev_buf<int32_t> t_n, t_shape, t_base, t_len;
  dev_buf<double> t_x, t_y, t_xv, t_yv, t_scale, t_ca, t_sa, t_angle, t_color;
  dev_buf<uint32_t> t_rgb;
  dev_buf<int8_t> t_label, t_cell_label;
  dev_buf<uint8_t> t_attr;
  const bool have_angle = src->p.p_angle != nullptr, have_color = src->p.p_color != nullptr;
  int made = 0, fail_at = -1;
  if (const char* x = getenv("SWB_COPY_POOL_FAIL_AT")) fail_at = atoi(x);
#define SWB_CLONE(tmp, from)                                                                                               \
  do {                                                                                                                     \
    if (made++ == fail_at) return fail(SWB_ERR_HIP, "swb_copy_pool: allocation %d refused (SWB_COPY_POOL_FAIL_AT)", made - 1); \
    if (tmp.clone(src->from.ptr, src->from.count, st)) return SWB_ERR_HIP;                                                 \
  } while (0)
  SWB_CLONE(t_n, d_p_n);
  SWB_CLONE(t_x, d_p_x); SWB_CLONE(t_y, d_p_y); SWB_CLONE(t_xv, d_p_xv); SWB_CLONE(t_yv, d_p_yv);
  SWB_CLONE(t_scale, d_p_scale); SWB_CLONE(t_ca, d_p_ca); SWB_CLONE(t_sa, d_p_sa);
  SWB_CLONE(t_shape, d_p_shape); SWB_CLONE(t_rgb, d_p_rgb); SWB_CLONE(t_label, d_p_label); SWB_CLONE(t_attr, d_p_attr);
  if (src->keyed) SWB_CLONE(t_cell_label, d_p_cell_label);
  if (have_angle) SWB_CLONE(t_angle, d_p_angle);
  if (have_color) SWB_CLONE(t_color, d_p_color);
#undef SWB_CLONE
  if (t_base.fill(pool_base_host, N) || t_len.fill(pool_len_host, N)) return SWB_ERR_HIP;
  HIP_TRY(hipDeviceSynchronize());
  dst->d_p_n.swap(t_n); dst->d_p_x.swap(t_x); dst->d_p_y.swap(t_y); dst->d_p_xv.swap(t_xv); dst->d_p_yv.swap(t_yv);
  dst->d_p_scale.swap(t_scale); dst->d_p_ca.swap(t_ca); dst->d_p_sa.swap(t_sa); dst->d_p_shape.swap(t_shape); dst->d_p_rgb.swap(t_rgb);
  dst->d_p_label.swap(t_label); dst->d_p_attr.swap(t_attr);
  if (src->keyed) dst->d_p_cell_label.swap(t_cell_label);
  if (have_angle) dst->d_p_angle.swap(t_angle);
  if (have_color) dst->d_p_color.swap(t_color);
  dst->d_pool_base.swap(t_base); dst->d_pool_len.swap(t_len);
  bump_list_epoch(dst);
  dst->rollout_stale = true;
  bind_pool(dst, have_angle, have_color);
  dst->pool_entries = P;
  dst->pool_id = src->pool_id;
  dst->pool_sampled = false;
  dst->pool_tree = false;
  dst->pool_uniform = false;
  if (verts > 0) dst->p.max_edges = verts;
  HIP_TRY(hipMemsetAsync(dst->d_reset_next, 1, N, st));
  HIP_TRY(hipMemsetAsync(dst->d_episode, 0, sizeof(int32_t) * N, st));
  HIP_TRY(hipMemsetAsync(dst->d_step_count, 0, sizeof(int32_t) * N, st));
  dst->have_pool = true;
  return restore_run_list_reservation(dst);
}

static void affine2(double sx, double shx, double shy, double sy, int n, const double* in, double* out) {
  for (int i = 0; i < n; ++i) {
    const double x = in[2 * i], y = in[2 * i + 1];
    double t0 = sx * x, t1 = shx * y;
    const double ox = t0 + t1 + 0.0;
    t0 = shy * x; t1 = sy * y;
    out[2 * i] = ox;
    out[2 * i + 1] = t0 + t1 + 0.0;
  }
}
static double deg2rad(double d) { return d * (3.14159265358979323846 / 180.0); }

int swb_sprite_path_op(int32_t attr, double a, double b, int32_t n, const double* in_xy, double* out_xy) {
  if (!in_xy || !out_xy || n < 0) return fail(SWB_ERR_INVALID, "bad argument");
  if (attr == SWB_ATTR_SHAPE) {
    const double th = deg2rad(b), ca = std::cos(th), sa = std::sin(th);
    affine2(ca * a, -sa * a, sa * a, ca * a, n, in_xy, out_xy);
  } else if (attr == SWB_ATTR_ANGLE) {
    const double th = deg2rad(a - b), ca = std::cos(th), sa = std::sin(th);
    affine2(ca, -sa, sa, ca, n, in_xy, out_xy);
  } else if (attr == SWB_ATTR_SCALE) {
    const double f = a - b;
    affine2(f, 0.0, 0.0, f, n, in_xy, out_xy);
  } else {
    return fail(SWB_ERR_INVALID, "unknown sprite attribute %d", attr);
  }
  return SWB_OK;
}

namespace {

struct env_override {
  std::vector<int32_t> shape;
  std::vector<double> scale, angle, cpath;
  std::vector<int8_t> label;
};

int ov_allocate(swb_engine* h) {
  if (h->d_ov_flag) return 0;
  const size_t N = h->p.N, NS = N * h->p.S, T = h->p.n_tasks;
  int rc = 0;
  rc |= h->d_ov_shape.fill(nullptr, NS);
  rc |= h->d_ov_scale.fill(nullptr, NS);
  rc |= h->d_ov_angle.fill(nullptr, NS);
  rc |= h->d_ov_label.fill(nullptr, NS * T);
  rc |= h->d_ov_cpath.fill(nullptr, NS * SWB_MAX_SHAPE_VERTS * 2);
  if (h->keyed) rc |= h->d_ov_cell_label.fill(nullptr, NS * T * SWB_MAX_CELLS);
  rc |= h->d_ov_flag.fill(nullptr, N);
  if (rc) return SWB_ERR_HIP;
  swb_params& p = h->p;
  p.ov_flag = h->d_ov_flag; p.ov_shape = h->d_ov_shape; p.ov_scale = h->d_ov_scale; p.ov_angle = h->d_ov_angle;
  p.ov_label = h->d_ov_label; p.ov_cpath = h->d_ov_cpath;
  p.ov_cell_label = h->d_ov_cell_label;
  return 0;
}

int ov_fetch(swb_engine* h, int env, env_override* r, int* n, bool* was_set, bool for_write = true) {
  const int S = h->p.S, T = h->p.n_tasks;
  r->shape.assign(S, 0); r->scale.assign(S, 1.0); r->angle.assign(S, 0.0);
  r->cpath.assign((size_t)S * SWB_MAX_SHAPE_VERTS * 2, 0.0); r->label.assign((size_t)T * S, 0);
  uint8_t flag = 0, rn = 0;
  int32_t en = 0, ns = 0;
  if (h->d_ov_flag) HIP_TRY(hipMemcpy(&flag, h->d_ov_flag + env, 1, hipMemcpyDeviceToHost));
  HIP_TRY(hipMemcpy(&rn, h->d_reset_next + env, 1, hipMemcpyDeviceToHost));
  HIP_TRY(hipMemcpy(&en, h->d_entry + env, 4, hipMemcpyDeviceToHost));
  HIP_TRY(hipMemcpy(&ns, h->d_nspr + env, 4, hipMemcpyDeviceToHost));
  int32_t ep = 0;
  HIP_TRY(hipMemcpy(&ep, h->d_episode + env, 4, hipMemcpyDeviceToHost));
  if (ep == 0) return fail(SWB_ERR_STATE, "environment %d has not been reset yet: it has no sprites", env);
  if (rn && for_write)
    return fail(SWB_ERR_STATE, "environment %d is about to reset (its episode ended): its sprites are gone at the next step", env);
  *n = ns;
  *was_set = flag != 0;
  const size_t o = (size_t)env * S, pe = (size_t)en * S;
  if (flag) {
    HIP_TRY(hipMemcpy(r->shape.data(), h->d_ov_shape + o, S * 4, hipMemcpyDeviceToHost));
    HIP_TRY(hipMemcpy(r->scale.data(), h->d_ov_scale + o, S * 8, hipMemcpyDeviceToHost));
    HIP_TRY(hipMemcpy(r->angle.data(), h->d_ov_angle + o, S * 8, hipMemcpyDeviceToHost));
    HIP_TRY(hipMemcpy(r->label.data(), h->d_ov_label + o * T, (size_t)T * S, hipMemcpyDeviceToHost));
    HIP_TRY(hipMemcpy(r->cpath.data(), h->d_ov_cpath + o * SWB_MAX_SHAPE_VERTS * 2, (size_t)S * SWB_MAX_SHAPE_VERTS * 16,
                      hipMemcpyDeviceToHost));
    return 0;
  }
  if (!h->p.p_angle) return fail(SWB_ERR_STATE, "the pool carries no angle column (swb_pool.angle)");
  std::vector<double> ca(S), sa(S);
  HIP_TRY(hipMemcpy(r->shape.data(), h->d_p_shape + pe, S * 4, hipMemcpyDeviceToHost));
  HIP_TRY(hipMemcpy(r->scale.data(), h->d_p_scale + pe, S * 8, hipMemcpyDeviceToHost));
  HIP_TRY(hipMemcpy(r->angle.data(), h->d_p_angle + pe, S * 8, hipMemcpyDeviceToHost));
  HIP_TRY(hipMemcpy(ca.data(), h->d_p_ca + pe, S * 8, hipMemcpyDeviceToHost));
  HIP_TRY(hipMemcpy(sa.data(), h->d_p_sa + pe, S * 8, hipMemcpyDeviceToHost));
  HIP_TRY(hipMemcpy(r->label.data(), h->d_p_label + pe * T, (size_t)T * S, hipMemcpyDeviceToHost));
  std::vector<double> sv((size_t)h->p.max_verts * 2 + 2);
  std::vector<int32_t> off(h->shape_nverts.size() + 1);
  HIP_TRY(hipMemcpy(off.data(), h->d_shape_off, off.size() * 4, hipMemcpyDeviceToHost));
  for (int s2 = 0; s2 < ns; ++s2) {
    const int sh = r->shape[s2];
    if (sh < 0 || sh >= (int)h->shape_nverts.size()) return fail(SWB_ERR_STATE, "pool entry %d uses shape %d", en, sh);
    const int nv = h->shape_nverts[sh];
    HIP_TRY(hipMemcpy(sv.data(), h->d_shape_verts + 2 * (size_t)off[sh], (size_t)nv * 16, hipMemcpyDeviceToHost));
    affine2(ca[s2] * r->scale[s2], -sa[s2] * r->scale[s2], sa[s2] * r->scale[s2], ca[s2] * r->scale[s2], nv, sv.data(),
            r->cpath.data() + (size_t)s2 * SWB_MAX_SHAPE_VERTS * 2);
  }
  return 0;
}

int ov_store(swb_engine* h, int env, const env_override& r) {
  const int S = h->p.S, T = h->p.n_tasks;
  const size_t o = (size_t)env * S;
  HIP_TRY(hipMemcpy(h->d_ov_shape + o, r.shape.data(), S * 4, hipMemcpyHostToDevice));
  HIP_TRY(hipMemcpy(h->d_ov_scale + o, r.scale.data(), S * 8, hipMemcpyHostToDevice));
  HIP_TRY(hipMemcpy(h->d_ov_angle + o, r.angle.data(), S * 8, hipMemcpyHostToDevice));
  HIP_TRY(hipMemcpy(h->d_ov_label + o * T, r.label.data(), (size_t)T * S, hipMemcpyHostToDevice));
  HIP_TRY(hipMemcpy(h->d_ov_cpath + o * SWB_MAX_SHAPE_VERTS * 2, r.cpath.data(), (size_t)S * SWB_MAX_SHAPE_VERTS * 16,
                    hipMemcpyHostToDevice));
  const uint8_t one = 1;
  HIP_TRY(hipMemcpy(h->d_ov_flag + env, &one, 1, hipMemcpyHostToDevice));
  return 0;
}

}

int swb_set_sprite_attr(swb_handle h, int32_t env, int32_t sprite, int32_t attr, double value, const double* delta,
                        const int8_t* label, void* stream) {
  if (!h) return fail(SWB_ERR_INVALID, "null handle");
  bump_list_epoch(h);
  if (!h->have_pool || !h->have_shapes) return fail(SWB_ERR_STATE, "no pool / shape table installed");
  if (env < 0 || env >= h->p.N) return fail(SWB_ERR_INVALID, "environment %d out of range", env);
  if (attr < SWB_ATTR_SHAPE || attr > SWB_ATTR_SCALE) return fail(SWB_ERR_INVALID, "unknown sprite attribute %d", attr);
  HIP_TRY(hipSetDevice(h->device));
  HIP_TRY(hipStreamSynchronize((hipStream_t)stream));
  env_override r;
  int n = 0;
  bool was_set = false;
  if (int rc = ov_fetch(h, env, &r, &n, &was_set)) return rc;
  if (sprite < 0 || sprite >= n) return fail(SWB_ERR_INVALID, "environment %d has %d sprites: sprite %d out of range", env, n, sprite);
  const int S = h->p.S, T = h->p.n_tasks;
  double* path = r.cpath.data() + (size_t)sprite * SWB_MAX_SHAPE_VERTS * 2;
  const int nv_old = h->shape_nverts[r.shape[sprite]];
  std::vector<double> out((size_t)SWB_MAX_SHAPE_VERTS * 2, 0.0);
  if (attr == SWB_ATTR_SHAPE) {
    const int sh = (int)value;
    if ((double)sh != value || sh < 0 || sh >= (int)h->shape_nverts.size()) return fail(SWB_ERR_INVALID, "bad shape index %g", value);
    const int nv = h->shape_nverts[sh];
    std::vector<int32_t> off(h->shape_nverts.size() + 1);
    HIP_TRY(hipMemcpy(off.data(), h->d_shape_off, off.size() * 4, hipMemcpyDeviceToHost));
    std::vector<double> sv((size_t)nv * 2);
    HIP_TRY(hipMemcpy(sv.data(), h->d_shape_verts + 2 * (size_t)off[sh], (size_t)nv * 16, hipMemcpyDeviceToHost));
    if (int rc = swb_sprite_path_op(SWB_ATTR_SHAPE, r.scale[sprite], r.angle[sprite], nv, sv.data(), out.data())) return rc;
    r.shape[sprite] = sh;
  } else if (attr == SWB_ATTR_ANGLE) {
    const double a = delta ? *delta : value, b = delta ? 0.0 : r.angle[sprite];
    if (int rc = swb_sprite_path_op(SWB_ATTR_ANGLE, a, b, nv_old, path, out.data())) return rc;
    r.angle[sprite] = value;
  } else {
    const double a = delta ? *delta : value, b = delta ? 0.0 : r.scale[sprite];
    if (int rc = swb_sprite_path_op(SWB_ATTR_SCALE, a, b, nv_old, path, out.data())) return rc;
    r.scale[sprite] = value;
  }
  memcpy(path, out.data(), out.size() * sizeof(double));
  if (label) for (int t = 0; t < T; ++t) r.label[(size_t)t * S + sprite] = label[t];
  int tot = 0;
  for (int s2 = 0; s2 < n; ++s2) tot += h->shape_nverts[r.shape[s2]];
  if (int rc = lf_check_vertices(h, std::max(h->p.max_edges, (tot + 3) & ~3), "swb_set_sprite_attr")) return rc;
  h->p.max_edges = std::max(h->p.max_edges, (tot + 3) & ~3);
  if (int rc = ov_allocate(h)) return rc;
  if (!was_set && h->keyed) {
    int32_t en = 0;
    HIP_TRY(hipMemcpy(&en, h->d_entry + env, 4, hipMemcpyDeviceToHost));
    const size_t blk = (size_t)T * S * SWB_MAX_CELLS;
    HIP_TRY(hipMemcpy(h->d_ov_cell_label + (size_t)env * blk, h->d_p_cell_label + (size_t)en * blk, blk, hipMemcpyDeviceToDevice));
  }
  return ov_store(h, env, r);
}

int swb_set_sprite_cell_labels(swb_handle h, int32_t env, int32_t sprite, const int8_t* cells, void* stream) {
  if (!h || !cells) return fail(SWB_ERR_INVALID, "null argument");
  bump_list_epoch(h);
  if (!h->keyed) return fail(SWB_ERR_INVALID, "no task of this handle keys on position");
  if (env < 0 || env >= h->p.N || sprite < 0 || sprite >= h->p.S) return fail(SWB_ERR_INVALID, "environment %d / sprite %d out of range", env, sprite);
  HIP_TRY(hipSetDevice(h->device));
  HIP_TRY(hipStreamSynchronize((hipStream_t)stream));
  uint8_t flag = 0;
  if (h->d_ov_flag) HIP_TRY(hipMemcpy(&flag, h->d_ov_flag + env, 1, hipMemcpyDeviceToHost));
  if (!flag) return fail(SWB_ERR_STATE, "swb_set_sprite_cell_labels follows swb_set_sprite_attr on the same environment");
  const int S = h->p.S, T = h->p.n_tasks;
  for (int t = 0; t < T; ++t)
    HIP_TRY(hipMemcpy(h->d_ov_cell_label + (((size_t)env * T + t) * S + sprite) * SWB_MAX_CELLS, cells + (size_t)t * SWB_MAX_CELLS,
                      SWB_MAX_CELLS, hipMemcpyHostToDevice));
  return SWB_OK;
}

int swb_get_sprite(swb_handle h, int32_t env, int32_t sprite, int32_t* shape, double* angle, double* scale, int32_t* n_verts,
                   double* path_xy, void* stream) {
  if (!h) return fail(SWB_ERR_INVALID, "null handle");
  if (!h->have_pool || !h->have_shapes) return fail(SWB_ERR_STATE, "no pool / shape table installed");
  if (env < 0 || env >= h->p.N) return fail(SWB_ERR_INVALID, "environment %d out of range", env);
  HIP_TRY(hipSetDevice(h->device));
  HIP_TRY(hipStreamSynchronize((hipStream_t)stream));
  env_override r;
  int n = 0;
  bool was_set = false;
  if (int rc = ov_fetch(h, env, &r, &n, &was_set, false)) return rc;
  if (sprite < 0 || sprite >= n) return fail(SWB_ERR_INVALID, "environment %d has %d sprites: sprite %d out of range", env, n, sprite);
  const int nv = h->shape_nverts[r.shape[sprite]];
  if (shape) *shape = r.shape[sprite];
  if (angle) *angle = r.angle[sprite];
  if (scale) *scale = r.scale[sprite];
  if (n_verts) *n_verts = nv;
  if (path_xy) memcpy(path_xy, r.cpath.data() + (size_t)sprite * SWB_MAX_SHAPE_VERTS * 2, (size_t)nv * 16);
  return SWB_OK;
}

int swb_variant(swb_handle h, swb_variant_info* out) {
  if (!h || !out) return fail(SWB_ERR_INVALID, "null argument");
  if (h->large_frames) {
    const variant* v0 = &kVariants[0];
    out->nw = v0->nw; out->ncol = 1; out->vs = 0;
    out->lds_bytes_per_wave = (int32_t)lds_per_wave(h, v0, nullptr);
    out->waves_per_simd = SWB_COVER_WAVES(v0->nw);
    out->resample_waves_per_simd = 0;
    out->n_bands = 0;
    out->n_column_groups = 0;
    out->run_cap = 0;
    out->paint_in_cover = 0;
    out->arena_units = 0;
    out->large_frames = 1;
    out->many_sprites = h->many_sprites ? 1 : 0;
    out->reserved_ = 0;
    if (h->many_sprites) {
      out->nw = 0;
      out->lds_bytes_per_wave = (int32_t)sizeof(swb_ms_lds);
      out->waves_per_simd = 0;
    }
    out->run_list_bytes = 0;
    out->frame_cache_bytes = 0;
    out->split_bands = 0;
    out->split_pad_ = 0;
    return SWB_OK;
  }
  const variant* v = pick_variant(h->p.Wc);
  if (!v) return fail(SWB_ERR_INVALID, "canvas %dx%d not supported", h->p.Wc, h->p.Hc);
  int vs = 0;
  (void)pick_resample(h->p.AA, h->vslots, &vs);
  out->nw = v->nw; out->ncol = 1; out->vs = vs;
  out->lds_bytes_per_wave = (int32_t)lds_per_wave(h, v, nullptr);
  out->waves_per_simd = SWB_COVER_WAVES(v->nw);
  out->resample_waves_per_simd = SWB_RS_WAVES_PER_SIMD;
  out->n_bands = h->split_bands ? 1 : (h->p.nbands ? h->p.nbands : h->nbands);
  out->split_bands = h->split_bands ? (h->p.nbands ? h->p.nbands : h->nbands) : 0;
  out->split_pad_ = 0;
  out->n_column_groups = h->p.ncg;
  out->run_cap = h->p.run_cap;
  out->paint_in_cover = paints_in_cover(h, v) ? 1 : 0;
  out->arena_units = h->d_runs ? h->p.arena_units : 0;
  out->large_frames = 0;
  out->many_sprites = 0;
  out->reserved_ = 0;
  out->run_list_bytes = h->d_runs ? ((int64_t)h->p.arena_base + h->p.arena_units + 4) * 8 : 0;
  out->frame_cache_bytes = (int64_t)h->d_frame_cache.count;
  return SWB_OK;
}

#ifndef SWB_BUILD_ID
#define SWB_BUILD_ID "unknown"
#endif
const char* swb_build_id(void) { return SWB_BUILD_ID; }

int swb_timing_enable(swb_handle h, int32_t enable) {
  if (!h) return fail(SWB_ERR_INVALID, "null handle");
  HIP_TRY(hipSetDevice(h->device));
  if (flush_timing(h)) return SWB_ERR_HIP;
  h->timing = enable != 0;
  h->timed_ms = 0.0;
  h->timed_cover_ms = 0.0;
  h->timed_launches = 0;
  return SWB_OK;
}

int swb_step_time_ms(swb_handle h, double* total_ms, int64_t* launches) {
  if (!h) return fail(SWB_ERR_INVALID, "null handle");
  HIP_TRY(hipSetDevice(h->device));
  if (flush_timing(h)) return SWB_ERR_HIP;
  if (total_ms) *total_ms = h->timed_ms;
  if (launches) *launches = h->timed_launches;
  return SWB_OK;
}

int swb_kernel_times_ms(swb_handle h, double* cover_ms, double* resample_ms, int64_t* launches) {
  if (!h) return fail(SWB_ERR_INVALID, "null handle");
  HIP_TRY(hipSetDevice(h->device));
  if (flush_timing(h)) return SWB_ERR_HIP;
  if (cover_ms) *cover_ms = h->timed_cover_ms;
  if (resample_ms) *resample_ms = h->timed_ms - h->timed_cover_ms;
  if (launches) *launches = h->timed_launches;
  return SWB_OK;
}

// ... 2 lines not shown
```

spriteworld_amd/csrc/swb_kernels.hip.inc:

```
#include <hip/hip_runtime.h>
#include <stdint.h>

#include "../../include/swb.h"

#define SWB_WAVE 64
#ifndef SWB_WORD_GROUPS
#define SWB_WORD_GROUPS 4
#endif
#ifndef SWB_AES_MIN_ITERS
#define SWB_AES_MIN_ITERS 4
#endif
#ifndef SWB_AES_MAX_NARROW_NW
#define SWB_AES_MAX_NARROW_NW 10
#endif
#ifndef SWB_COVER_WAVES_PER_SIMD
#define SWB_COVER_WAVES_PER_SIMD 5
#endif
#ifndef SWB_COVER_WAVES_PER_SIMD_NARROW
#define SWB_COVER_WAVES_PER_SIMD_NARROW 6
#endif
#ifndef SWB_COVER_WAVES_PER_SIMD_WIDE
#define SWB_COVER_WAVES_PER_SIMD_WIDE 4
#endif
#ifndef SWB_RS_WAVES_PER_SIMD
#define SWB_RS_WAVES_PER_SIMD 8
#endif
#define SWB_COVER_WAVES(NW) ((NW) <= 2 ? SWB_COVER_WAVES_PER_SIMD_NARROW : ((NW) <= 10 ? SWB_COVER_WAVES_PER_SIMD : SWB_COVER_WAVES_PER_SIMD_WIDE))
#define SWB_RS_WAVES_PER_BLOCK 4
#define SWB_VSLOTS 8
#define SWB_TUNED_SPRITES 16
#define PRECISION_BITS 22

struct swb_params {
  int32_t N, S, AA;
  int32_t Wo, Ho;
  int32_t Wc, Hc;
  uint32_t bg;
  int32_t action_space, keep_in_frame, max_episode_length, pos_is_f32, action_is_f32;
  double action_scale, motion_cost;
  int32_t n_tasks, is_meta, meta_aggregator, meta_termination;
  double meta_terminate_bonus;
  swb_task tasks[SWB_MAX_TASKS];
  const double* shape_verts;
  const int32_t* shape_off;
  int32_t max_verts;
  const double* shape_dmin;
  const int32_t* h_xmin;
  const int32_t* h_cnt;
  const int32_t* h_tbl;
  const int32_t* h_pfx;
  int32_t h_pfx_len;
  const int32_t* v_tab;
  const int32_t* v_pfx;
  const int32_t* v_end;
  const int32_t* p_n;
  const double *p_x, *p_y, *p_xv, *p_yv, *p_scale, *p_ca, *p_sa;
  const int32_t* p_shape;
  const uint32_t* p_rgb;
  const int8_t* p_label;
  const int8_t* p_cell_label;
  const int32_t *pool_base, *pool_len;
  const double *p_angle, *p_color;
  double *x, *y;
  int32_t *nspr, *entry, *step_count, *episode;
  uint8_t* reset_next;
  const void* actions;
  uint8_t* obs;
  double* reward;
  float* discount;
  uint8_t *step_type, *success, *error;
  int32_t render_only;
  int32_t lds_per_wave;
  int32_t outrow_bytes;
  int32_t max_edges;
  int32_t cpath_in_masks;
  int32_t max_spans;
  int32_t span_cap;
  uint32_t* ovf;
  uint32_t* ovf_bitmap;
  int32_t ovf_slots;
  int32_t ovf_cap;
  uint32_t* runs;
  uint32_t* rhdr;
  int32_t run_cap;
  uint32_t* arena_head;
  int64_t arena_base;
  int32_t arena_units;
  int32_t arena_pad_;
  int32_t ncg;
  int32_t nbands;
  const int32_t* band_lo;
  const int32_t* band_y0;
  const int32_t* band_first;
  const uint32_t* v_break;
  const int32_t* cg_lo;
  const int32_t* cg_hi;
  uint32_t* cost_cnt;
  int32_t* cost_list;
  int32_t cost_cap;
  int32_t cost_range0;
  int32_t parity;
  int32_t deal_shift;
  int32_t* ccost_list;
  int32_t cover_order;
  int32_t cphase;
  int32_t prio_div;
  int32_t prio_levels;
  int32_t paint_in_cover;
  int32_t band_tasks;
  uint8_t* ov_flag;
  const int32_t* ov_shape;
  const double* ov_scale;
  const double* ov_angle;
  const int8_t* ov_label;
  const double* ov_cpath;
  const int8_t* ov_cell_label;
  uint32_t list_epoch;
  uint32_t list_pad_;
  unsigned long long* list_stats;
  uint8_t* frame_cache;
  unsigned long long* frame_stats;
  int32_t obs_aligned16;
  int32_t copy_cost;
  int32_t split_bands;
  int32_t split_when;
  int32_t split_carry;
  int32_t split_pad_;
  unsigned long long* split_stats;
  const uint8_t* active;
};

template <typename T>
using cptr = const T __attribute__((address_space(4)))*;
template <typename T>
__device__ __forceinline__ cptr<T> as_const(const T* q) { return (cptr<T>)(uintptr_t)q; }

__device__ __forceinline__ int lane_id() { return threadIdx.x & (SWB_WAVE - 1); }
__device__ __forceinline__ int rfl(int v) { return __builtin_amdgcn_readfirstlane(v); }
__device__ __forceinline__ float rflf(float v) { return __int_as_float(__builtin_amdgcn_readfirstlane(__float_as_int(v))); }
__device__ __forceinline__ double rfld(double v) {
  const long long b = __double_as_longlong(v);
  const int lo = __builtin_amdgcn_readfirstlane((int)(b & 0xffffffffll));
  const int hi = __builtin_amdgcn_readfirstlane((int)(b >> 32));
  return __longlong_as_double(((long long)hi << 32) | (unsigned int)lo);
}
__device__ __forceinline__ double readlane_d(double v, int src) {
  const long long b = __double_as_longlong(v);
  const int lo = __builtin_amdgcn_readlane((int)(b & 0xffffffffll), src);
  const int hi = __builtin_amdgcn_readlane((int)(b >> 32), src);
  return __longlong_as_double(((long long)hi << 32) | (unsigned int)lo);
}
__device__ __forceinline__ void wave_sync() {
  __builtin_amdgcn_fence(__ATOMIC_ACQ_REL, "wavefront");
  __builtin_amdgcn_wave_barrier();
}
__device__ __forceinline__ int wave_min_i(int v) {
  for (int o = 32; o > 0; o >>= 1) v = min(v, __shfl_xor(v, o, 64));
  return v;
}
__device__ __forceinline__ int wave_max_i(int v) {
  for (int o = 32; o > 0; o >>= 1) v = max(v, __shfl_xor(v, o, 64));
  return v;
}

__device__ __forceinline__ int pil_round_up(float f) {
  if (f >= 0.0f) return (int)floorf(__fadd_rn(f, 0.5f));
  return (int)(-floor(__dadd_rn(fabs((double)f), 0.5)));
}
__device__ __forceinline__ int pil_round_down(float f) {
  if (f >= 0.0f) return (int)ceilf(__fsub_rn(f, 0.5f));
  return (int)(-ceil(__dsub_rn(fabs((double)f), 0.5)));
}
__device__ __forceinline__ float pil_cross(int y, int y0, float dx, int x0) {
  return __fadd_rn(__fmul_rn((float)(y - y0), dx), (float)x0);
}

__device__ __forceinline__ void centered_vertex(const swb_params& p, int shape_o, int i, double scale,
                                                double ca, double sa, double& cx, double& cy) {
  const double vx = p.shape_verts[2 * (shape_o + i)], vy = p.shape_verts[2 * (shape_o + i) + 1];
  const double m00 = __dmul_rn(ca, scale), m01 = __dmul_rn(-sa, scale);
  const double m10 = __dmul_rn(sa, scale), m11 = __dmul_rn(ca, scale);
  cx = __dadd_rn(__dadd_rn(__dmul_rn(m00, vx), __dmul_rn(m01, vy)), 0.0);
  cy = __dadd_rn(__dadd_rn(__dmul_rn(m10, vx), __dmul_rn(m11, vy)), 0.0);
}

__device__ __forceinline__ bool contains_point_wave(const double2* cpath, int n, double tx, double ty) {
  const int l = lane_id();
  bool cross = false;
  if (l < n) {
    const double2 v0 = cpath[l], v1 = cpath[(l + 1 == n) ? 0 : l + 1];
    const bool f0 = (v0.y >= ty), f1 = (v1.y >= ty);
    if (f0 != f1) {
      const double lhs = __dmul_rn(__dsub_rn(v1.y, ty), __dsub_rn(v0.x, v1.x));
      const double rhs = __dmul_rn(__dsub_rn(v1.x, tx), __dsub_rn(v0.y, v1.y));
      cross = ((lhs >= rhs) == f1);
    }
  }
  return (__popcll(__ballot(cross)) & 1) != 0;
}

__device__ __forceinline__ double move1(int pos_f32, double pv, double motion, int keep) {
  double q = __dadd_rn(pv, motion);
  if (pos_f32) q = (double)(float)q;
  if (keep) {
    if (q < 0.0) q = 0.0;
    if (q > 1.0) q = 1.0;
  }
  return q;
}

__device__ __forceinline__ double np_sum_d(const double* a, int n) {
  if (n < 8) {
// ... 153 lines not shown
      float df = (float)d;
      if (!(df > 0.0f)) df = 0.0f;
      sc->tmpf[l] = sqrtf(df);
    } else {
      double d = __dmul_rn(-2.0, sc->cnt[c] == 1 ? dot2_hi(x, y, m0, m1) : dot2_lo(x, y, m0, m1));
      d = __dadd_rn(d, xxn);
      d = __dadd_rn(d, yy);
      if (!(d > 0.0)) d = 0.0;
      sc->tmp[l] = __dsqrt_rn(d);
    }
  }
  wave_sync();
  double* sorted_d = sc->px0;
  float* sorted_f = reinterpret_cast<float*>(sc->px0);
  if (l < k) {
    int off = 0;
    for (int c = 0; c < k; ++c) if (c < l) off += sc->cnt[c];
    const int cnt = sc->cnt[l];
    int j = 0;
    for (int i = 0; i < m; ++i)
      if (sc->lab[i] == l) {
        if (pos_f32) sorted_f[off + j] = sc->tmpf[i]; else sorted_d[off + j] = sc->tmp[i];
        ++j;
      }
    double intra;
    if (pos_f32) intra = (double)__fdiv_rn(np_sum_f(sorted_f + off, cnt), (float)cnt);
    else intra = __ddiv_rn(np_sum_d(sorted_d + off, cnt), (double)cnt);
    sc->intra[l] = intra;
  }
  wave_sync();
  if (l < k) sc->tmp[l] = 0.0;
  wave_sync();
  const int all_i_zero = __ballot(l < k && !(fabs(sc->intra[l < k ? l : 0]) <= 1e-8)) == 0ull;
  int all_d_zero = 1;
  unsigned long long* best_bits = reinterpret_cast<unsigned long long*>(sc->tmp);
  const int rows_per_pass = 64 / k;
  const int ar = (int)(((uint32_t)l * (uint32_t)((65536 + k - 1) / k)) >> 16), b = l - ar * k;
  for (int a_base = 0; a_base < k; a_base += rows_per_pass) {
    const int a = a_base + ar;
    bool dnz = false;
    if (ar < rows_per_pass && a < k) {
      const double a0 = sc->c0[a], a1 = sc->c1[a], b0 = sc->c0[b], b1 = sc->c1[b];
      const double na = norm2(a0, a1), nb = norm2(b0, b1);
      double d = __dmul_rn(-2.0, dot2_hi(a0, a1, b0, b1));
      d = __dadd_rn(d, na);
      d = __dadd_rn(d, nb);
      if (!(d > 0.0)) d = 0.0;
      if (a == b) d = 0.0;
      const double D = __dsqrt_rn(d);
      dnz = !(fabs(D) <= 1e-8);
      const double den = (D == 0) ? __longlong_as_double(0x7ff0000000000000ll) : D;
      const double v = __ddiv_rn(__dadd_rn(sc->intra[a], sc->intra[b]), den);
      atomicMax(&best_bits[a], (unsigned long long)__double_as_longlong(v));
    }
    if (__ballot(dnz)) all_d_zero = 0;
  }
  wave_sync();
  if (all_i_zero || all_d_zero) { *score_out = 0.0; return SWB_ENV_ERR_DB_ZERO; }
  const double score = __ddiv_rn(np_sum_d(sc->tmp, k), (double)k);
  *score_out = score;
  wave_sync();
  if (score == 0.0) return SWB_ENV_ERR_DB_ZERO;
  return 0;
}

template <typename SC>
__device__ __forceinline__ int task_clustering_wave(const swb_task& t, int pos_f32, int n, double px, double py,
                                                    const int8_t* label, SC* sc, double* reward, int* success) {
  double score = 0.0;
  const int err = davies_bouldin_wave(pos_f32, n, px, py, label, sc, &score);
  if (err) { *reward = __longlong_as_double(0x7ff8000000000000ll); *success = 0; return err; }
  const double metric = __ddiv_rn(1.0, score);
  const double dense = __ddiv_rn(__dmul_rn(__dsub_rn(metric, t.termination_threshold), t.reward_range), 2.0);
  const int ok = metric >= t.termination_threshold;
  double r = 0.0;
  if (ok) { r = __dadd_rn(r, t.terminate_bonus); r = __dadd_rn(r, dense); }
  else if (!t.sparse_reward) { r = __dadd_rn(r, dense); }
  *reward = r;
  *success = ok;
  return 0;
}

template <typename SC>
__device__ __forceinline__ int eval_task_wave(const swb_params& p, int n, double px, double py, const int8_t* label,
                                              SC* sc, double* reward, int* success) {
  const int l = lane_id();
  int err = 0;
  double r0 = 0.0;
  int ok0 = 0;
  for (int t = 0; t < p.n_tasks; ++t) {
    const swb_task& tk = p.tasks[t];
    const int8_t* lab = label + t * p.S;
    double r = 0.0;
    int ok = 0;
    if (tk.kind == SWB_TASK_FIND_GOAL) task_find_goal_wave(tk, n, px, py, lab, sc, &r, &ok);
    else if (tk.kind == SWB_TASK_CLUSTERING) err |= task_clustering_wave(tk, p.pos_is_f32, n, px, py, lab, sc, &r, &ok);
    if (t == 0) { r0 = r; ok0 = ok; }
    if (p.is_meta && l == 0) { sc->tr[t] = r; sc->tok[t] = ok; }
  }
  if (!p.is_meta) { *reward = r0; *success = ok0; return err; }
  wave_sync();
  const double* r = sc->tr;
  const int* ok = sc->tok;
  int succ = (p.meta_termination == SWB_TERM_ALL);
  for (int t = 0; t < p.n_tasks; ++t) succ = (p.meta_termination == SWB_TERM_ALL) ? (succ && ok[t]) : (succ || ok[t]);
  double agg;
  const double qnan = __longlong_as_double(0x7ff8000000000000ll);
  if (p.meta_aggregator == SWB_AGG_SUM || p.meta_aggregator == SWB_AGG_MEAN) {
    int cnt = 0;
    double v[SWB_MAX_TASKS];
#pragma unroll
    for (int t = 0; t < SWB_MAX_TASKS; ++t) {
      const double x = (t < p.n_tasks) ? r[t] : 0.0;
      const bool isn = (x != x);
      v[t] = isn ? 0.0 : x;
      cnt += (t < p.n_tasks) && !isn;
    }
    if (p.n_tasks < 8) {
      agg = -0.0;
#pragma unroll
      for (int t = 0; t < SWB_MAX_TASKS; ++t) if (t < p.n_tasks) agg = __dadd_rn(agg, v[t]);
    } else {
      agg = __dadd_rn(__dadd_rn(__dadd_rn(v[0], v[1]), __dadd_rn(v[2], v[3])), __dadd_rn(__dadd_rn(v[4], v[5]), __dadd_rn(v[6], v[7])));
    }
    if (p.meta_aggregator == SWB_AGG_MEAN) agg = __ddiv_rn(agg, (double)cnt);
  } else {
    agg = qnan;
    for (int t = 0; t < p.n_tasks; ++t) {
      if (r[t] != r[t]) continue;
      if (agg != agg) agg = r[t];
      else if (p.meta_aggregator == SWB_AGG_MAX ? (r[t] > agg) : (r[t] < agg)) agg = r[t];
    }
  }
  agg = __dadd_rn(agg, __dmul_rn(p.meta_terminate_bonus, (double)succ));
  *reward = agg;
  *success = succ;
  wave_sync();
  return err;
}

struct env_state {
  bool first, ov;
  bool active;
  int en, n, sc_old;
  double px, py;
  double scale_l, ca_l, sa_l, xv_l, yv_l;
  int sh_idx, so_l, nv_l;
  double act;
  int acti;
};
struct step_cost { double cost; float cost_f32; bool cost_is_f32; int step_count; bool changed; };

template <bool OV, bool MASK = true, typename SC>
__device__ __forceinline__ env_state load_env_state(const swb_params& p, int env, SC* tscratch) {
  const int l = lane_id();
  const int S = p.S;
  double* gx = p.x + (size_t)env * S;
  double* gy = p.y + (size_t)env * S;
  bool active = true;
  if constexpr (MASK) { if (p.active != nullptr) active = rfl((int)as_const(p.active)[env]) != 0; }
  const int rn = (p.render_only || !active) ? 0 : (int)p.reset_next[env];
  const int ep = p.episode[env], pbase = as_const(p.pool_base)[env], plen = as_const(p.pool_len)[env];
  const int en_old = p.entry[env], n_old = p.nspr[env], sc_old = p.step_count[env];
  double px = 0.0, py = 0.0;
  if (l < S) { px = gx[l]; py = gy[l]; }
  static_assert(SWB_MAX_SHAPES + 1 <= SWB_WAVE, "one lane per entry of the shape table");
  const int shoff_tab_l = (l <= SWB_MAX_SHAPES) ? p.shape_off[l] : 0;
  double act = 0.0;
  int acti = 0;
  if (!p.render_only && active) {
    if (p.action_space == SWB_ACTION_EMBODIED) { if (l < 2) acti = reinterpret_cast<const int32_t*>(p.actions)[2 * (size_t)env + l]; }
    else if (l < 4) {
      act = p.action_is_f32 ? (double)reinterpret_cast<const float*>(p.actions)[4 * (size_t)env + l]
                            : reinterpret_cast<const double*>(p.actions)[4 * (size_t)env + l];
    }
  }
  const bool first = rn != 0;
  bool ov = false;
  if constexpr (OV) {
    ov = rfl((int)p.ov_flag[env]) != 0;
    if (ov && first) {
      ov = false;
      if (l == 0) p.ov_flag[env] = 0;
    }
  }
  const int en = rfl(first ? pbase + (ep % plen) : en_old);
  const size_t pe = (size_t)en * S;
  int n = first ? as_const(p.p_n)[en] : n_old;
  int shape_l = 0;
  double scale_l = 1.0, ca_l = 1.0, sa_l = 0.0, xv_l = 0.0, yv_l = 0.0;
  if (l < S) {
    shape_l = p.p_shape[pe + l]; scale_l = p.p_scale[pe + l]; ca_l = p.p_ca[pe + l]; sa_l = p.p_sa[pe + l];
    xv_l = p.p_xv[pe + l]; yv_l = p.p_yv[pe + l];
    if (first) { px = p.p_x[pe + l]; py = p.p_y[pe + l]; gx[l] = px; gy[l] = py; }
    if constexpr (OV) {
      if (ov) { shape_l = p.ov_shape[(size_t)env * S + l]; scale_l = p.ov_scale[(size_t)env * S + l]; }
    }
  }
  if (p.render_only != 1 && active) {
    const int8_t* lab_src = p.p_label + (size_t)en * p.n_tasks * S;
    if constexpr (OV) { if (ov) lab_src = p.ov_label + (size_t)env * p.n_tasks * S; }
    for (int i = l; i < p.n_tasks * S; i += SWB_WAVE) tscratch->labels[i] = lab_src[i];
  }
  n = rfl(n);
  if (first && l == 0) { p.episode[env] = ep + 1; p.entry[env] = en; p.nspr[env] = n; p.step_count[env] = 0; p.reset_next[env] = 0; }
  const int sh_idx = (int)min((uint32_t)shape_l, (uint32_t)(SWB_MAX_SHAPES - 1));
  const int so_any = __shfl(shoff_tab_l, sh_idx, 64), so_next = __shfl(shoff_tab_l, sh_idx + 1, 64);
  const int so_l = (l < n) ? so_any : 0;
  const int nv_l = (l < n) ? so_next - so_any : 0;
  return env_state{first, ov, active, en, n, sc_old, px, py, scale_l, ca_l, sa_l, xv_l, yv_l, sh_idx, so_l, nv_l, act, acti};
}
// ... 4 lines not shown
  double &px = es.px, &py = es.py;
  double* gx = p.x + (size_t)env * p.S;
  double* gy = p.y + (size_t)env * p.S;
  double cost = 0.0;
  float cost_f32 = 0.0f;
  bool cost_is_f32 = false;
  int step_count = 0;
  bool changed = false;
  if (!p.render_only && !es.first && es.active) {
    const double ox = px, oy = py;
    step_count = es.sc_old + 1;
    int moved = -1;
    double m0 = 0.0, m1 = 0.0;
    if (p.action_space == SWB_ACTION_EMBODIED) {
      const int carry = __builtin_amdgcn_readlane(es.acti, 0), dir = __builtin_amdgcn_readlane(es.acti, 1);
      const double st = p.action_scale;
      if (dir == 0) m1 = st; else if (dir == 1) m0 = -st; else if (dir == 2) m1 = -st; else m0 = st;
      if (n > 0) {
        const int body = n - 1;
        const double bx = readlane_d(px, body), by = readlane_d(py, body);
        if (carry) {
          for (int s2 = body - 1; s2 >= 0; --s2) {
            const double sx = readlane_d(px, s2), sy = readlane_d(py, s2);
            double tx, ty;
            if (p.pos_is_f32) { tx = (double)__fsub_rn((float)bx, (float)sx); ty = (double)__fsub_rn((float)by, (float)sy); }
            else { tx = __dsub_rn(bx, sx); ty = __dsub_rn(by, sy); }
            if (hit(s2, tx, ty)) {
              moved = s2;
              break;
            }
          }
        }
        if (l == moved || l == body) {
          px = move1(p.pos_is_f32, px, m0, p.keep_in_frame);
          py = move1(p.pos_is_f32, py, m1, p.keep_in_frame);
        }
      }
      cost = __dmul_rn(-p.motion_cost, st);
    } else {
      const double a0 = readlane_d(es.act, 0), a1 = readlane_d(es.act, 1);
      const double a2 = readlane_d(es.act, 2), a3 = readlane_d(es.act, 3);
      const bool af = p.action_is_f32 != 0;
      if (af) {
        const float f0 = (float)a0, f1 = (float)a1, f2 = (float)a2, f3 = (float)a3, sc = (float)p.action_scale;
        float m0f, m1f;
        if (p.action_space == SWB_ACTION_DRAG_AND_DROP) { m0f = __fmul_rn(__fsub_rn(f2, f0), sc); m1f = __fmul_rn(__fsub_rn(f3, f1), sc); }
        else { m0f = __fmul_rn(__fsub_rn(f2, 0.5f), sc); m1f = __fmul_rn(__fsub_rn(f3, 0.5f), sc); }
        m0 = (double)m0f; m1 = (double)m1f;
        cost_f32 = __fmul_rn((float)(-p.motion_cost), sqrtf(__fadd_rn(__fmul_rn(m0f, m0f), __fmul_rn(m1f, m1f))));
        cost = (double)cost_f32;
        cost_is_f32 = true;
      } else if (p.action_space == SWB_ACTION_DRAG_AND_DROP) {
        m0 = __dmul_rn(__dsub_rn(a2, a0), p.action_scale); m1 = __dmul_rn(__dsub_rn(a3, a1), p.action_scale);
      } else {
        m0 = __dmul_rn(__dsub_rn(a2, 0.5), p.action_scale); m1 = __dmul_rn(__dsub_rn(a3, 0.5), p.action_scale);
      }
      for (int s2 = n - 1; s2 >= 0; --s2) {
        const double sx = readlane_d(px, s2), sy = readlane_d(py, s2);
        double tx, ty;
        if (af && p.pos_is_f32) { tx = (double)__fsub_rn((float)a0, (float)sx); ty = (double)__fsub_rn((float)a1, (float)sy); }
        else { tx = __dsub_rn(a0, sx); ty = __dsub_rn(a1, sy); }
        if (hit(s2, tx, ty)) {
          moved = s2;
          break;
        }
      }
      if (l == moved) {
        px = move1(p.pos_is_f32, px, m0, p.keep_in_frame);
        py = move1(p.pos_is_f32, py, m1, p.keep_in_frame);
      }
      if (!af) cost = __dmul_rn(-p.motion_cost, __dsqrt_rn(dot2_hi(m0, m1, m0, m1)));
    }
    if (l < n) {
      px = move1(p.pos_is_f32, px, es.xv_l, p.keep_in_frame);
      py = move1(p.pos_is_f32, py, es.yv_l, p.keep_in_frame);
      gx[l] = px; gy[l] = py;
    }
    changed = __ballot(l < n && (__double_as_longlong(px) != __double_as_longlong(ox) ||
                                 __double_as_longlong(py) != __double_as_longlong(oy))) != 0ull;
  }
  return step_cost{cost, cost_f32, cost_is_f32, step_count, changed};
}

template <bool OV, typename SC>
__device__ __forceinline__ uint32_t finish_step(const swb_params& p, int env, const env_state& es, const step_cost& c, SC* tscratch) {
  const int l = lane_id(), S = p.S, n = es.n;
  const double px = es.px, py = es.py;
  wave_sync();
  if (p.p_cell_label != nullptr) {
    const int8_t* cells = p.p_cell_label + (size_t)es.en * p.n_tasks * S * SWB_MAX_CELLS;
    if constexpr (OV) { if (es.ov && p.ov_cell_label) cells = p.ov_cell_label + (size_t)env * p.n_tasks * S * SWB_MAX_CELLS; }
    for (int t = 0; t < p.n_tasks; ++t) {
      const swb_task& tk = p.tasks[t];
      if (tk.n_xcuts + tk.n_ycuts == 0) continue;
      if (l < n) {
        int cx = 0, cy = 0;
        for (int k = 0; k < tk.n_xcuts; ++k) cx += (px >= tk.xcuts[k]) ? 1 : 0;
        for (int k = 0; k < tk.n_ycuts; ++k) cy += (py >= tk.ycuts[k]) ? 1 : 0;
        tscratch->labels[t * S + l] = cells[((size_t)t * S + l) * SWB_MAX_CELLS + cy * (tk.n_xcuts + 1) + cx];
      }
    }
    wave_sync();
  }
  const bool oof_l = (l < n) && !(px >= 0. && py >= 0. && px <= 1. && py <= 1.);
  const int oof = __ballot(oof_l) != 0ull;
  double tr = 0.0; int ok = 0;
  const int terr = eval_task_wave(p, n, px, py, tscratch->labels, tscratch, &tr, &ok);
  if (l == 0) {
    if (p.success) p.success[env] = (uint8_t)ok;
    if (p.render_only) {
    } else if (es.first) {
      if (p.reward) p.reward[env] = __longlong_as_double(0x7ff8000000000000ll);
      if (p.discount) p.discount[env] = __int_as_float(0x7fc00000);
      if (p.step_type) p.step_type[env] = SWB_STEP_FIRST;
    } else {
      const bool task_is_pyfloat = !p.is_meta && p.tasks[0].kind != SWB_TASK_FIND_GOAL;
      const double rew = (c.cost_is_f32 && task_is_pyfloat) ? (double)__fadd_rn(c.cost_f32, (float)tr) : __dadd_rn(c.cost, tr);
      if (p.reward) p.reward[env] = rew;
      const int timeout = c.step_count >= p.max_episode_length;
      const int last = ok || oof || timeout;
      p.step_count[env] = c.step_count;
      if (last) p.reset_next[env] = 1;
      if (p.step_type) p.step_type[env] = last ? SWB_STEP_LAST : SWB_STEP_MID;
      if (p.discount) p.discount[env] = last ? 0.0f : 1.0f;
    }
  }
  return l == 0 ? (uint32_t)terr : 0u;
}

struct edge_rec {
  int16_t x0, y0, y1;
  int16_t xtop;
  float dx;
  int16_t xbot;
  int16_t pad;
};
#define SWB_NO_REPL (-32768)

__device__ __forceinline__ float repl_to_float(int v) { return v == SWB_NO_REPL ? __int_as_float(0x7fc00000) : (float)v; }
__device__ __forceinline__ int repl_to_int(float v) { return (v == v) ? (int)v : SWB_NO_REPL; }

struct sprite_rec {
  int32_t edge_off, n_edges;
  int32_t ymin, ymax;
  uint32_t rgb;
  int32_t w0, w1;
  int32_t max_edge_rows;
};

#define SWB_NWA(NW) ((NW) <= 5 ? (NW) : ((NW) <= 10 ? 5 : 6))
template <int NW>
struct wave_lds {
  uint32_t T[SWB_NWA(NW)][SWB_WAVE];
  uint32_t Px[SWB_NWA(NW)][SWB_WAVE];
  sprite_rec spr[SWB_TUNED_SPRITES];
  int32_t ovf_slot;
  int32_t pad_[3];
  uint32_t outrow[];
};

struct corner_end {
  int row, adj;
  float xc, repl;
  bool live;
};
__device__ __forceinline__ void corner_try(corner_end& c, int cx0, int cy0, float cdx, int ox0, int oy0, int oy1, float odx,
                                           bool want) {
  if (want) {
    const int oymin = min(oy0, oy1), oymax = max(oy0, oy1);
    const float xo = pil_cross(c.row, oy0, odx, ox0);
    if (roundf(c.xc) == roundf(xo) && c.adj >= oymin && c.adj <= oymax) {
      const float a = pil_cross(c.adj, cy0, cdx, cx0);
      const float b = pil_cross(c.adj, oy0, odx, ox0);
      if (c.xc > __fadd_rn(a, 1.0f) && c.xc > __fadd_rn(b, 1.0f)) c.repl = __fadd_rn(roundf(fmaxf(a, b)), 1.0f);
      else if (c.xc < __fsub_rn(a, 1.0f) && c.xc < __fsub_rn(b, 1.0f)) c.repl = __fsub_rn(roundf(fminf(a, b)), 1.0f);
      c.live = false;
    }
  }
}

#define SWB_ROWTAB_SLOTS 8
#define SWB_ROWTAB_DWORDS (SWB_TUNED_SPRITES * SWB_ROWTAB_SLOTS * 2)
static_assert(SWB_ROWTAB_DWORDS * 4 <= SWB_MIN_SPANS * 256, "the row table borrows the span lists");
template <int NW>
__device__ __forceinline__ void build_all_edges(const swb_params& p, wave_lds<NW>* L, edge_rec* edges, const double2* cpath,
                                                uint32_t* rowtab, int nspr, int vtotal, int voff_l, int nv_l, double px, double py,
                                                double dmin_l, double scale_l, uint32_t rgb_reg, uint32_t& err) {
  const int l = lane_id();
  double* posx = reinterpret_cast<double*>(L->outrow);
  double* posy = posx + SWB_TUNED_SPRITES;
  int* nvs = reinterpret_cast<int*>(posy + SWB_TUNED_SPRITES);
// ... 778 lines not shown

#define SWB_RESCAN_WITH_OVERFLOW_SLOT()                                                          \
  if (__ballot((err & SWB_INT_NEED_SLOT) != 0u)) {                                               \
    err &= ~SWB_INT_NEED_SLOT;                                                                   \
    if (rfl(*ovf) == -1) {                                                                       \
      if (l == 0) *ovf = ovf_slot_alloc(p);                                                      \
      wave_sync();                                                                               \
      if (rfl(*ovf) >= 0) { yb -= 64; continue; }                                                \
    }                                                                                            \
    err |= SWB_ENV_ERR_SPAN_OVERFLOW;                                                            \
  }

template <int NW, bool OV = false, bool PAINT = false>
__global__ void __launch_bounds__(SWB_WAVE, SWB_COVER_WAVES(NW))
swb_cover_kernel(const swb_params p) {
  static_assert(!PAINT || NW == 2, "painting in the cover kernel: images of up to 64 columns at anti_aliasing = 1");
  extern __shared__ __attribute__((aligned(16))) unsigned char smem[];
  const int l = lane_id();
  const uint32_t cycles0 = (uint32_t)__builtin_amdgcn_s_memtime();
  int env = blockIdx.x;
  uint32_t predicted = 0u, prio_q = 0u;
  int prio = 0;
  const int ph = p.cphase, ph_prev = ph == 0 ? 2 : ph - 1, ph_next = ph == 2 ? 0 : ph + 1;
  uint32_t filing_words_l = 0u;
  if (p.cost_cnt != nullptr && l < ((!PAINT && p.split_bands) ? 4 : 3))
    filing_words_l = p.cost_cnt[l == 0 ? SWB_COST_WORD_KEY_LO(p.parity) : (l == 1 ? SWB_COST_WORD_KEY_SCALE(p.parity) : ((PAINT || l == 2) ? SWB_COST_WORD_COVER_SHIFT(ph) : SWB_COST_WORD_SPLIT(p.parity)))];
  if (p.ccost_list) cover_cost_housekeeping(p, ph_prev, ph, ph_next);
  if (p.arena_head != nullptr && blockIdx.x == 0 && l == 0) p.arena_head[p.parity ^ 1] = 0u;
  if (p.cover_order) {
    const int sh = (int)(blockIdx.x & (SWB_COST_SHARDS - 1)), cap = (p.N + SWB_COST_SHARDS - 1) / SWB_COST_SHARDS;
    int bucket = 0;
    env = cost_ordered_entry(p.cost_cnt + cost_row1(ph_prev, sh),
                             as_const(p.ccost_list) + (size_t)(ph_prev * SWB_COST_SHARDS + sh) * SWB_COST_BUCKETS * cap, cap,
                             (int)(blockIdx.x >> 3), &bucket);
    if (env < 0) return;
    prio_q = (p.prio_levels & 2) ? as_const(p.cost_cnt)[SWB_COST_WORD_COVER_PRIO(ph)] : 0u;
    if (prio_q) predicted = (uint32_t)(2 * bucket + 1) << (as_const(p.cost_cnt)[SWB_COST_WORD_COVER_SHIFT(ph_prev)] - 1u);
  }
  auto file_cover_cost = [&]() __attribute__((always_inline)) {
    if (p.ccost_list) {
      const uint32_t cycles = (uint32_t)__builtin_amdgcn_s_memtime() - cycles0;
      const uint32_t width = (uint32_t)__builtin_amdgcn_readlane((int)filing_words_l, 2);
      if (l == 0) {
        const int key = (int)min(cycles >> width, (uint32_t)(SWB_COST_BUCKETS - 1));
        const int sh = env & (SWB_COST_SHARDS - 1);
        if ((cycles >> width) >= (uint32_t)SWB_COST_BUCKETS) atomicMax(&p.cost_cnt[SWB_COST_WORD_COVER_MAX(ph, sh)], cycles);
        const uint32_t pos = atomicAdd(&p.cost_cnt[cost_row1(ph, sh) + key], 1u);
        p.ccost_list[((size_t)(ph * SWB_COST_SHARDS + sh) * SWB_COST_BUCKETS + key) * ((p.N + SWB_COST_SHARDS - 1) / SWB_COST_SHARDS) + pos] = env;
      }
    }
  };
  auto reprioritise = [&]() __attribute__((always_inline)) {
    if (predicted) {
      const uint32_t elapsed = (uint32_t)__builtin_amdgcn_s_memtime() - cycles0;
      const int level = elapsed >= predicted ? 0 : (int)min((predicted - elapsed) >> prio_q, 3u);
      if (level != prio) {
        prio = level;
        if (level == 3) __builtin_amdgcn_s_setprio(3);
        else if (level == 2) __builtin_amdgcn_s_setprio(2);
        else if (level == 1) __builtin_amdgcn_s_setprio(1);
        else __builtin_amdgcn_s_setprio(0);
      }
    }
  };
  reprioritise();
  unsigned char* wbase = smem;
  wave_lds<NW>* L = reinterpret_cast<wave_lds<NW>*>(wbase);
  edge_rec* edges = reinterpret_cast<edge_rec*>(wbase + ((sizeof(wave_lds<NW>) + (size_t)p.outrow_bytes + 15) & ~(size_t)15));
  uint32_t* spans = reinterpret_cast<uint32_t*>(reinterpret_cast<unsigned char*>(edges) +
                                                (((size_t)p.max_edges * sizeof(edge_rec) + 15) & ~(size_t)15));
  task_scratch* tscratch = reinterpret_cast<task_scratch*>(spans);
  int32_t* ovf = &L->ovf_slot;
  if (l == 0) *ovf = -1;
  const int S = p.S;

  double2* cpath = p.cpath_in_masks ? reinterpret_cast<double2*>(L->T) : reinterpret_cast<double2*>(edges);
  static_assert(sizeof(double2) == sizeof(edge_rec), "centred paths alias the edge records");

  uint32_t err = 0;
  const double shdmin_tab_l = (l < SWB_MAX_SHAPES) ? p.shape_dmin[l] : 0.0;
  if constexpr (!PAINT) {
    if (p.list_epoch != 0u && l <= SWB_MAX_CG + 2) L->outrow[l] = p.rhdr[(size_t)env * SWB_RHDR_DWORDS + SWB_RHDR_COST + l];
  }
  env_state es = load_env_state<OV>(p, env, tscratch);
  const int n = es.n, nv_l = es.nv_l;
  const double scale_l = es.scale_l;
  uint32_t rgb_reg = 0u;
  if (l < S) rgb_reg = p.p_rgb[(size_t)es.en * S + l];
  if (l >= n) rgb_reg = 0u;

  const double dmin_any = __shfl(shdmin_tab_l, es.sh_idx, 64);
  double dmin_l = (l < n) ? dmin_any : 0.0;
  if constexpr (OV) { if (es.ov) dmin_l = 0.0; }
  int voff_l = nv_l;
  for (int o = 1; o < SWB_TUNED_SPRITES; o <<= 1) { const int t = __shfl_up(voff_l, o, 64); if (l >= o) voff_l += t; }
  const int vtotal = __builtin_amdgcn_readlane(voff_l, SWB_TUNED_SPRITES - 1);
  voff_l -= nv_l;
  for (int base = 0; base < vtotal; base += 64) {
    const int k = base + l;
    int sid = 0;
    for (int s2 = 1; s2 < n; ++s2) if (k >= __builtin_amdgcn_readlane(voff_l, s2)) sid = s2;
    const int i = k - __shfl(voff_l, sid, 64);
    const int so = __shfl(es.so_l, sid, 64);
    const double sc = __shfl(scale_l, sid, 64), ca = __shfl(es.ca_l, sid, 64), sa = __shfl(es.sa_l, sid, 64);
    if (k < vtotal) {
      double cx, cy;
      bool from_table = true;
      if constexpr (OV) {
        if (es.ov) {
          const double* q = p.ov_cpath + (((size_t)env * S + sid) * SWB_MAX_SHAPE_VERTS + i) * 2;
          cx = q[0]; cy = q[1];
          from_table = false;
        }
      }
      if (from_table) centered_vertex(p, so, i, sc, ca, sa, cx, cy);
      cpath[k] = make_double2(cx, cy);
    }
  }
  wave_sync();
  SWB_HOOK_PHASE_END(3)

  auto hit = [&](int s2, double tx, double ty) __attribute__((always_inline)) {
    return contains_point_wave(cpath + __builtin_amdgcn_readlane(voff_l, s2), __builtin_amdgcn_readlane(nv_l, s2), tx, ty);
  };
  const step_cost sc = act_and_move(p, env, es, hit);
  const double px = es.px, py = es.py;
  SWB_HOOK_PHASE_END(4)
  if (p.render_only != 1 && es.active) {
    err |= finish_step<OV>(p, env, es, sc, tscratch);
    wave_sync();
  }
  SWB_HOOK_PHASE_END(5)
  if (p.obs == nullptr) {
    if (l == 0 && p.error && err) p.error[env] |= (uint8_t)err;
    return;
  }

  [[maybe_unused]] auto file_lists = [&](int cost_l, const uint32_t* bst, uint32_t built_cycles, bool copies) __attribute__((always_inline)) {
    const bool whole = p.split_bands && (copies || __builtin_amdgcn_readlane((int)filing_words_l, 3) == 0);
    const bool bt = bst != nullptr && !whole;
    const int ntask = bt ? p.ncg * p.nbands : p.ncg;
    const bool file0 = p.cost_cnt != nullptr && l < ntask, file1 = p.ccost_list != nullptr && l == 0;
    const int sh = env & (SWB_COST_SHARDS - 1);
    int task_cost = cost_l, task_bits = l << 24;
    if (bt) {
      wave_sync();
      const int g2 = min(l / p.nbands, p.ncg - 1), b2 = l - (l / p.nbands) * p.nbands;
      const uint32_t* bg = bst + g2 * SWB_BST_STRIDE;
      const int u0 = (int)bg[b2], u1 = (int)bg[min(b2 + 1, p.nbands)], u2 = (int)bg[min(b2 + 2, p.nbands)];
      task_cost = 4 * max((u1 - u0) + (p.AA == 1 ? 0 : (((u2 - u1) * 5) >> 4)), 0);
      task_bits = (g2 << 24) | (b2 << 26);
    }
    if (whole) task_bits |= SWB_TASK_WHOLE;
    if (copies) task_cost = p.copy_cost;
    const int key0 = cost_key(task_cost, (uint32_t)__builtin_amdgcn_readlane((int)filing_words_l, 0), (uint32_t)__builtin_amdgcn_readlane((int)filing_words_l, 1));
    int key1 = 0;
    uint32_t cycles = built_cycles;
    if (p.ccost_list) {
      if (built_cycles == 0u) cycles = (uint32_t)__builtin_amdgcn_s_memtime() - cycles0;
      const uint32_t width = (uint32_t)__builtin_amdgcn_readlane((int)filing_words_l, 2);
      key1 = (int)min(cycles >> width, (uint32_t)(SWB_COST_BUCKETS - 1));
      if (l == 0 && (cycles >> width) >= (uint32_t)SWB_COST_BUCKETS) atomicMax(&p.cost_cnt[SWB_COST_WORD_COVER_MAX(ph, sh)], cycles);
    }
    uint32_t pos0 = 0u, pos1 = 0u;
    if (copies) { if (file0 && l == 0) pos0 = atomicAdd(&p.cost_cnt[cost_row0(p.parity, sh) + key0], (uint32_t)ntask); }
    else if (file0) pos0 = atomicAdd(&p.cost_cnt[cost_row0(p.parity, sh) + key0], 1u);
    if (file1) pos1 = atomicAdd(&p.cost_cnt[cost_row1(ph, sh) + key1], 1u);
// ... 692 lines not shown
    for (int w = l; w < a.mask_words; w += SWB_WAVE) {
      uint32_t bits = 0u;
      const int xb = 32 * w;
      int prev = (xb >= 1 && xb - 1 < Wc) ? row[xb - 1] : -1;
      for (int b = 0; b < 32; ++b) {
        const int x = xb + b;
        if (x > Wc) break;
        if (x == Wc) { bits |= 1u << b; break; }
        const int c = row[x];
        if (x >= 1 && c != prev) bits |= 1u << b;
        prev = c;
      }
      bmask[w] = bits;
    }
    wave_sync();
    uint8_t* out_row = a.tmp + ((size_t)(env - a.e0) * Hc + (size_t)y) * (size_t)Wo * 3;
    for (int o = l; o < Wo; o += SWB_WAVE) {
      const int xmin = as_const(a.hb)[2 * o], xend = xmin + as_const(a.hb)[2 * o + 1];
      cptr<int32_t> pf = as_const(a.hp) + as_const(a.hpo)[o];
      int s0 = SWB_HALF, s1 = SWB_HALF, s2 = SWB_HALF;
      int x = xmin, wlo = 0;
      while (x < xend) {
        int wi = (x + 1) >> 5;
        uint32_t bits = bmask[wi] & (0xffffffffu << ((x + 1) & 31));
        while (bits == 0u && 32 * (wi + 1) < xend) bits = bmask[++wi];
        int nx = bits ? 32 * wi + __ffs((int)bits) - 1 : xend;
        nx = min(nx, xend);
        const int whi = pf[nx - xmin];
        const int k = whi - wlo;
        const uint32_t c = B->col[row[x]];
        s0 += (int)(c & 255u) * k; s1 += (int)((c >> 8) & 255u) * k; s2 += (int)((c >> 16) & 255u) * k;
        wlo = whi;
        x = nx;
      }
      out_row[3 * o] = (uint8_t)clip8_fix(s0);
      out_row[3 * o + 1] = (uint8_t)clip8_fix(s1);
      out_row[3 * o + 2] = (uint8_t)clip8_fix(s2);
    }
    wave_sync();
  }
}

__global__ void __launch_bounds__(SWB_WAVE * SWB_LF_WAVES)
swb_lf_vertical_kernel(const swb_params p, const swb_lf_args a) {
  const int wave = rfl(threadIdx.x >> 6);
  const int r = (int)blockIdx.y * SWB_LF_WAVES + wave;
  const int env = a.e0 + (int)blockIdx.z;
  const int nd = (p.Wo * 3) >> 2;
  const int d = (int)blockIdx.x * SWB_WAVE + lane_id();
  if (r >= p.Ho || d >= nd) return;
  const int ymin = as_const(a.vb)[2 * r], cnt = as_const(a.vb)[2 * r + 1];
  cptr<int32_t> k = as_const(a.vk) + (size_t)r * a.vks;
  const uint32_t* src = reinterpret_cast<const uint32_t*>(a.tmp + (size_t)(env - a.e0) * p.Hc * (size_t)p.Wo * 3) +
                        (size_t)ymin * nd + d;
  int s0 = SWB_HALF, s1 = SWB_HALF, s2 = SWB_HALF, s3 = SWB_HALF;
  for (int i = 0; i < cnt; ++i) {
    const uint32_t w = src[(size_t)i * nd];
    const int c = k[i];
    s0 += (int)(w & 255u) * c; s1 += (int)((w >> 8) & 255u) * c;
    s2 += (int)((w >> 16) & 255u) * c; s3 += (int)(w >> 24) * c;
  }
  const uint32_t out = (uint32_t)clip8_fix(s0) | ((uint32_t)clip8_fix(s1) << 8) | ((uint32_t)clip8_fix(s2) << 16) |
                       ((uint32_t)clip8_fix(s3) << 24);
  reinterpret_cast<uint32_t*>(p.obs + ((size_t)env * p.Ho + (size_t)(p.Ho - 1 - r)) * (size_t)p.Wo * 3)[d] = out;
}

#endif

struct swb_ms_lds {
  task_scratch_t<SWB_MAX_SPRITES> ts;
  double2 path[SWB_MAX_SHAPE_VERTS];
};
static_assert(SWB_MAX_SPRITES <= SWB_WAVE && SWB_MAX_SHAPE_VERTS <= SWB_WAVE, "one lane per sprite / per vertex");

template <bool OV>
__global__ void __launch_bounds__(SWB_WAVE)
swb_ms_state_kernel(const swb_params p) {
  extern __shared__ __attribute__((aligned(16))) unsigned char smem[];
  const int l = lane_id();
  const int env = blockIdx.x;
  swb_ms_lds* M = reinterpret_cast<swb_ms_lds*>(smem);
  task_scratch_t<SWB_MAX_SPRITES>* tscratch = &M->ts;
  double2* cpath = M->path;
  env_state es = load_env_state<OV>(p, env, tscratch);
  auto hit = [&](int s2, double tx, double ty) __attribute__((always_inline)) {
    const int nv = __builtin_amdgcn_readlane(es.nv_l, s2), so = __builtin_amdgcn_readlane(es.so_l, s2);
    const double sc = readlane_d(es.scale_l, s2), ca = readlane_d(es.ca_l, s2), sa = readlane_d(es.sa_l, s2);
    wave_sync();
    if (l < nv) {
      double cx, cy;
      bool from_table = true;
      if constexpr (OV) {
        if (es.ov) {
          const double* q = p.ov_cpath + (((size_t)env * p.S + s2) * SWB_MAX_SHAPE_VERTS + l) * 2;
          cx = q[0]; cy = q[1];
          from_table = false;
        }
      }
      if (from_table) centered_vertex(p, so, l, sc, ca, sa, cx, cy);
      cpath[l] = make_double2(cx, cy);
    }
    wave_sync();
    return contains_point_wave(cpath, nv, tx, ty);
  };
  const step_cost sc = act_and_move(p, env, es, hit);
  if (p.render_only != 1 && es.active) {
    const uint32_t err = finish_step<OV>(p, env, es, sc, tscratch);
    if (l == 0 && p.error && err) p.error[env] |= (uint8_t)err;
  }
}

#ifndef SWB_WIDE_TU
struct swb_rollout_args {
  int32_t M, K;
  double *x, *y;
  int32_t *nspr, *entry, *step_count, *episode, *pool_base, *pool_len;
  uint8_t* reset_next;
  swb_params* steps;
  const void* actions;
  double* reward;
  float* discount;
  uint8_t *step_type, *success;
  uint8_t* error;
  double *out_x, *out_y;
  int32_t* out_n;
};
static_assert(sizeof(swb_params) + sizeof(swb_rollout_args) <= 4096, "kernel arguments of the rollout kernels");

__global__ void __launch_bounds__(256)
swb_rollout_fork_kernel(const swb_params p, const swb_rollout_args a) {
  const int idx = (int)(blockIdx.x * blockDim.x + threadIdx.x);
  if (idx < a.K) {
    const size_t o = (size_t)idx * p.N * a.M;
    const size_t action_bytes = p.action_space == SWB_ACTION_EMBODIED ? 2 * sizeof(int32_t) : (p.action_is_f32 ? 4 * sizeof(float) : 4 * sizeof(double));
    swb_params q = p;
    q.x = a.x; q.y = a.y; q.nspr = a.nspr; q.entry = a.entry; q.step_count = a.step_count; q.episode = a.episode;
    q.reset_next = a.reset_next; q.pool_base = a.pool_base; q.pool_len = a.pool_len;
    q.obs = nullptr; q.error = nullptr; q.render_only = 0; q.active = nullptr;
    q.actions = reinterpret_cast<const unsigned char*>(a.actions) + o * action_bytes;
    q.reward = a.reward ? a.reward + o : nullptr;
    q.discount = a.discount ? a.discount + o : nullptr;
    q.step_type = a.step_type ? a.step_type + o : nullptr;
    q.success = a.success ? a.success + o : nullptr;
    a.steps[idx] = q;
  }
  if (idx >= p.N * a.M * p.S) return;
  const int v = idx / p.S, s = idx - v * p.S, n = v / a.M;
  a.x[idx] = p.x[(size_t)n * p.S + s];
  a.y[idx] = p.y[(size_t)n * p.S + s];
  if (s == 0) {
    a.nspr[v] = p.nspr[n]; a.entry[v] = p.entry[n]; a.step_count[v] = p.step_count[n]; a.episode[v] = p.episode[n];
    a.reset_next[v] = p.reset_next[n];
    a.pool_base[v] = p.pool_base[n]; a.pool_len[v] = p.pool_len[n];
  }
}

__global__ void __launch_bounds__(256)
swb_reset_envs_kernel(uint8_t* reset_next, const uint8_t* mask, int N) {
  const int n = (int)(blockIdx.x * blockDim.x + threadIdx.x);
  if (n < N && mask[n] != 0) reset_next[n] = 1;
}

struct swb_state_view {
  double *x, *y;
  int32_t *nspr, *entry, *step_count, *episode, *pool_base, *pool_len;
  uint8_t* reset_next;
};
// ... 45 lines not shown
  if (s == 0) {
    dst.nspr[n] = src.nspr[c]; dst.entry[n] = src.entry[c]; dst.step_count[n] = src.step_count[c]; dst.episode[n] = src.episode[c];
    dst.reset_next[n] = src.reset_next[c];
    dst.pool_base[n] = src.pool_base[c]; dst.pool_len[n] = src.pool_len[c];
    if (rhdr) rhdr[(size_t)n * SWB_RHDR_DWORDS + SWB_RHDR_STAMP] = 0u;
  }
}

struct swb_rollout_keep {
  swb_state_view traj;
  double *out_x, *out_y;
  int32_t* out_n;
};
static_assert(sizeof(swb_params) + sizeof(swb_rollout_args) + sizeof(swb_rollout_keep) <= 4096, "kernel arguments of the rollout kernels");

__global__ void __launch_bounds__(256)
swb_rollout_pick_steps_kernel(const swb_state_view src, const swb_state_view pool, const swb_state_view dst, const int32_t* cand, int N,
                              int S, int M, int k0, int nk) {
  const int idx = (int)(blockIdx.x * blockDim.x + threadIdx.x);
  if (idx >= nk * N * S) return;
  const int e = idx / S, s = idx - e * S, kk = e / N, n = e - kk * N;
  const size_t v = (size_t)n * M + (size_t)min(max(cand[n], 0), M - 1);
  const size_t slot = (size_t)(k0 + kk) * N * M + v;
  dst.x[idx] = src.x[slot * S + s];
  dst.y[idx] = src.y[slot * S + s];
  if (s == 0) {
    dst.nspr[e] = src.nspr[slot]; dst.entry[e] = src.entry[slot]; dst.step_count[e] = src.step_count[slot];
    dst.episode[e] = src.episode[slot]; dst.reset_next[e] = src.reset_next[slot];
    dst.pool_base[e] = pool.pool_base[v]; dst.pool_len[e] = pool.pool_len[v];
  }
}

#ifndef SWB_ROLLOUT_WAVES_PER_SIMD
#define SWB_ROLLOUT_WAVES_PER_SIMD 6
#endif
#ifndef SWB_ROLLOUT_KEEP_WAVES_PER_SIMD
#define SWB_ROLLOUT_KEEP_WAVES_PER_SIMD 6
#endif
#ifndef SWB_ROLLOUT_SAMPLED_WAVES_PER_SIMD
#define SWB_ROLLOUT_SAMPLED_WAVES_PER_SIMD 6
#endif
struct swb_rollout_sample_args {
  int32_t mode;
  uint64_t seed, first_env;
  void* actions;
  int32_t *sprite, *tries;
};
static_assert(sizeof(swb_rollout_args) + sizeof(swb_rollout_keep) + sizeof(swb_rollout_sample_args) + 8 <= 4096,
              "kernel arguments of swb_rollout_kernel");
template <bool SAMPLE> struct rollout_drawer {};
template <> struct rollout_drawer<true>;
template <bool KEEP, bool SAMPLE>
__global__ void __launch_bounds__(SWB_WAVE, SAMPLE ? SWB_ROLLOUT_SAMPLED_WAVES_PER_SIMD
                                                   : (KEEP ? SWB_ROLLOUT_KEEP_WAVES_PER_SIMD : SWB_ROLLOUT_WAVES_PER_SIMD))
swb_rollout_kernel(const swb_rollout_args a, int S, const swb_rollout_keep keep, const swb_rollout_sample_args sa) {
  extern __shared__ __attribute__((aligned(16))) unsigned char smem[];
  const int l = lane_id();
  const int v = blockIdx.x;
  swb_ms_lds* M = reinterpret_cast<swb_ms_lds*>(smem);
  task_scratch_t<SWB_MAX_SPRITES>* tscratch = &M->ts;
  double2* cpath = M->path;
  uint32_t err = 0;
  int ep = 0;
  if constexpr (KEEP) ep = a.episode[v];
  rollout_drawer<SAMPLE> drawer;
  if constexpr (SAMPLE) drawer.start(sa, v / a.M, v % a.M);
  for (int k = 0; k < a.K; ++k) {
    const swb_params& q = *(const swb_params*)as_const(a.steps + k);
    env_state es = load_env_state<false, false>(q, v, tscratch);
    if constexpr (SAMPLE) drawer.draw(sa, q, k, es, cpath);
    auto hit = [&](int s2, double tx, double ty) __attribute__((always_inline)) {
      const int nv = __builtin_amdgcn_readlane(es.nv_l, s2), so = __builtin_amdgcn_readlane(es.so_l, s2);
      const double sc = readlane_d(es.scale_l, s2), ca = readlane_d(es.ca_l, s2), sa = readlane_d(es.sa_l, s2);
      wave_sync();
      if (l < nv) {
        double cx, cy;
        centered_vertex(q, so, l, sc, ca, sa, cx, cy);
        cpath[l] = make_double2(cx, cy);
      }
      wave_sync();
      return contains_point_wave(cpath, nv, tx, ty);
    };
    const step_cost sc = act_and_move(q, v, es, hit);
    err |= finish_step<false>(q, v, es, sc, tscratch);
    if constexpr (KEEP) {
      const size_t slot = (size_t)k * gridDim.x + v;
      ep += es.first ? 1 : 0;
      if (l < S) {
        keep.traj.x[slot * S + l] = es.px;
        keep.traj.y[slot * S + l] = es.py;
        if (keep.out_x) keep.out_x[slot * S + l] = es.px;
        if (keep.out_y) keep.out_y[slot * S + l] = es.py;
      }
      if (l == 0) {
        keep.traj.nspr[slot] = es.n; keep.traj.entry[slot] = es.en; keep.traj.step_count[slot] = sc.step_count;
        keep.traj.episode[slot] = ep;
        if (k > 0) keep.traj.reset_next[slot - gridDim.x] = es.first ? 1 : 0;
        if (keep.out_n) keep.out_n[slot] = es.n;
      }
    }
    wave_sync();
  }
  if constexpr (KEEP) {
    if (l == 0) keep.traj.reset_next[(size_t)(a.K - 1) * gridDim.x + v] = a.reset_next[v];
  }
  if (l < S) {
    if (a.out_x) a.out_x[(size_t)v * S + l] = a.x[(size_t)v * S + l];
    if (a.out_y) a.out_y[(size_t)v * S + l] = a.y[(size_t)v * S + l];
  }
  if (l == 0) {
    if (a.out_n) a.out_n[v] = a.nspr[v];
    if (a.error && err) a.error[v] |= (uint8_t)err;
  }
}
#endif
```

spriteworld_amd/engine.py:

```python
import ctypes as C

import numpy as np
import torch

from spriteworld_amd import _abi
from spriteworld_amd import _lib
from spriteworld_amd import lanczos
from spriteworld_amd import shapes as _shapes


def _ptr(a):
  return None if a is None else C.c_void_p(a.ctypes.data)


class Snapshot(object):

  FIELDS = ('x', 'y', 'n_sprites', 'pool_entry', 'step_count', 'episode', 'pool_base', 'pool_len', 'reset_next')
  _DTYPES = dict(x=torch.float64, y=torch.float64, reset_next=torch.uint8)

  def __init__(self, tensors, pool_id, max_sprites):
    self.pool_id, self.max_sprites = int(pool_id), int(max_sprites)
    for k in self.FIELDS:
      setattr(self, k, tensors[k])

# ... 269 lines not shown
      drawn = {k: new(*layout[k]) for k in set(outputs) | {'actions'}}
    o, so, sa = _abi.SwbRolloutOutputs(), _abi.SwbRolloutStepOutputs(), _abi.SwbRolloutSampledOutputs()
    for k, t in res.items():
      setattr(o, k, t.data_ptr())
    for k, t in steps.items():
      setattr(so, k, t.data_ptr())
    for k, t in drawn.items():
      setattr(sa, k, t.data_ptr())
    self._last_rollout_actions = drawn['actions']
    self._check(self.lib.swb_rollout_sampled(self._h, int(mode), C.c_uint64(int(seed) & 0xFFFFFFFFFFFFFFFF), C.c_uint64(int(first_env)),
                                             M, K, int(bool(keep_steps)), C.byref(o), C.byref(so) if keep_steps else None, C.byref(sa),
                                             self._stream()))
    self._rollout_M, self._rollout_K = M, (K if keep_steps else 0)
    res.update((k + '_steps', t) for k, t in steps.items())
    res.update((k, drawn[k]) for k in outputs)
    return res

  def rollout_frames(self, candidates=None, step=None):
    if isinstance(step, str):
      if step != 'all':
        raise ValueError("rollout_frames step must be an int or 'all', got %r" % (step,))
      if candidates is None:
        raise ValueError("rollout_frames step='all' needs candidates: loop over the steps for the frames of all candidates")
      step = _abi.SWB_ALL_STEPS
    elif step is not None and int(step) < 0:
      raise ValueError('rollout_frames step must be in [0, K), got %d' % int(step))
    M = self._rollout_M
    if not M or (step is not None and not self._rollout_K):
      if step is None:
        self._check(self.lib.swb_rollout_frames(self._h, 0, None, None, None, self._stream()))
      self._check(self.lib.swb_rollout_step_frames(self._h, M, int(step), None, None, None, self._stream()))
    cand = None
    if candidates is not None:
      cand = candidates if isinstance(candidates, torch.Tensor) else torch.as_tensor(np.ascontiguousarray(candidates))
      if cand.dim() != 1 or cand.shape[0] != self.N or cand.is_floating_point():
        raise ValueError('rollout_frames candidates must be int[%d], got %s %s' % (self.N, cand.dtype, tuple(cand.shape)))
      cand = cand.to(device=self.device, dtype=torch.int32).contiguous()
    lead = (self.N,) if cand is not None else (self.N, M)
    if step == _abi.SWB_ALL_STEPS:
      lead = (self._rollout_K,) + lead
    with self._device_scope():
      res = {'obs': torch.empty(lead + self.obs_shape, dtype=torch.uint8, device=self.device),
             'error': torch.zeros(lead, dtype=torch.uint8, device=self.device)}
    self._last_rollout_candidates = cand
    cand_p, obs_p, err_p = (None if cand is None else C.c_void_p(cand.data_ptr()), C.c_void_p(res['obs'].data_ptr()),
                            C.c_void_p(res['error'].data_ptr()))
    if step is None:
      self._check(self.lib.swb_rollout_frames(self._h, M, cand_p, obs_p, err_p, self._stream()))
    else:
      self._check(self.lib.swb_rollout_step_frames(self._h, M, int(step), cand_p, obs_p, err_p, self._stream()))
    return res

  def sample_actions(self, mode, seed, first_env=0, outputs=('actions',)):
    if self.cfg.action_space == _abi.ACTION_EMBODIED:
      shape, dtype = (self.N, 2), torch.int32
    else:
      shape, dtype = (self.N, 4), (torch.float32 if self.cfg.action_is_f32 else torch.float64)
    layout = {'actions': (shape, dtype), 'position': ((self.N, 2), torch.float64), 'sprite': ((self.N,), torch.int32),
              'tries': ((self.N,), torch.int32)}
    unknown = [k for k in outputs if k not in layout]
    if unknown:
      raise ValueError('sample_actions outputs must be among %s, got %s' % (sorted(layout), unknown))
    with self._device_scope():
      res = {k: torch.empty(layout[k][0], dtype=layout[k][1], device=self.device) for k in outputs}
    o = _abi.SwbSampledActions()
    for k, t in res.items():
      setattr(o, k, t.data_ptr())
    self._check(self.lib.swb_sample_actions(self._h, int(mode), C.c_uint64(int(seed) & 0xFFFFFFFFFFFFFFFF),
                                            C.c_uint64(int(first_env)), C.byref(o), self._stream()))
    return res

  def trim(self):
    if not hasattr(self.lib, 'swb_trim_run_lists'):
      return None
    cap = C.c_int32(0)
    self._check(self.lib.swb_trim_run_lists(self._h, C.byref(cap), self._stream()))
    return cap.value

  def list_stats(self):
    kept, built = C.c_int64(0), C.c_int64(0)
    self._check(self.lib.swb_list_stats(self._h, C.byref(kept), C.byref(built), self._stream()))
    return kept.value, built.value

  def frame_stats(self):
    w = [C.c_int64(0) for _ in range(3)]
    self._check(self.lib.swb_frame_stats(self._h, C.byref(w[0]), C.byref(w[1]), C.byref(w[2]), self._stream()))
    return tuple(x.value for x in w)

  def split_stats(self):
    w = [C.c_int64(0) for _ in range(3)]
    self._check(self.lib.swb_split_stats(self._h, C.byref(w[0]), C.byref(w[1]), C.byref(w[2]), self._stream()))
    return tuple(x.value for x in w)

  def frame_cycles(self):
    w = (C.c_int64 * 3)()
    self._check(self.lib.swb_frame_cycles(self._h, w, self._stream()))
    return tuple(w)

  def render(self):
    self._check(self.lib.swb_render(self._h, C.c_void_p(self.obs.data_ptr()), self._stream()))
    return self.obs

  def evaluate(self):
    self._check(self.lib.swb_evaluate(self._h, C.c_void_p(self.success.data_ptr()), self._stream()))
    return self.success

  def factors(self):
    if getattr(self, '_factors', None) is None:
      self._factors = torch.zeros((self.N, self.S, 10), dtype=torch.float64, device=self.device)
    self._check(self.lib.swb_factors(self._h, C.c_void_p(self._factors.data_ptr()), self._stream()))
    return self._factors

  def state(self):
    st = {
        'x': np.zeros((self.N, self.S)), 'y': np.zeros((self.N, self.S)),
        'n_sprites': np.zeros(self.N, np.int32), 'pool_entry': np.zeros(self.N, np.int32),
        'step_count': np.zeros(self.N, np.int32), 'reset_next': np.zeros(self.N, np.uint8),
        'episode': np.zeros(self.N, np.int32),
    }
    cs = _abi.SwbState(*[a.ctypes.data for a in (st['x'], st['y'], st['n_sprites'], st['pool_entry'],
                                                  st['step_count'], st['reset_next'], st['episode'])])
    self._check(self.lib.swb_get_state(self._h, C.byref(cs), self._stream()))
    return st

  def env_state(self, env):
    out = np.zeros(5, np.int32)
    self._check(self.lib.swb_get_env_state(self._h, int(env), _ptr(out), self._stream()))
    return dict(zip(('n_sprites', 'pool_entry', 'step_count', 'episode', 'reset_next'), (int(v) for v in out)))

  def sprite_types(self, env, sprite):
    f = C.c_int32(0)
    self._check(self.lib.swb_get_sprite_types(self._h, int(env), int(sprite), C.byref(f), self._stream()))
    return bool(f.value & 1), bool(f.value & 2)

  def set_positions(self, x, y):
    x = np.ascontiguousarray(x, dtype=np.float64)
    y = np.ascontiguousarray(y, dtype=np.float64)
    self._check(self.lib.swb_set_positions(self._h, _ptr(x), _ptr(y), self._stream()))

  def pool_id(self):
    v = C.c_uint64(0)
    self._check(self.lib.swb_pool_id(self._h, C.byref(v)))
    return v.value

  def _index_tensor(self, values, what):
    t = values if isinstance(values, torch.Tensor) else torch.as_tensor(np.ascontiguousarray(values))
    if t.dim() != 1 or t.is_floating_point():
      raise ValueError('%s must be a 1-D integer tensor or array, got %s %s' % (what, t.dtype, tuple(t.shape)))
    return t.to(device=self.device, dtype=torch.int32).contiguous()

  def save_state(self, index=None, source='live'):
    if source not in ('live', 'rollout'):
      raise ValueError("save_state source is 'live' or 'rollout', got %r" % (source,))
    idx = None if index is None else self._index_tensor(index, 'save_state index')
    n_src = self.N * self._rollout_M if source == 'rollout' else self.N
    count = int(idx.shape[0]) if idx is not None else max(n_src, 1)
    with self._device_scope():
      snap = Snapshot.empty(count, self.S, self.device, self.pool_id())
    cs = snap.as_struct()
    self._last_state_index = idx
    self._check(self.lib.swb_save_state(self._h, _abi.STATE_ROLLOUT_END if source == 'rollout' else _abi.STATE_LIVE,
                                        None if idx is None else C.c_void_p(idx.data_ptr()), count, C.byref(cs), self._stream()))
    return snap

  def load_state(self, snapshot, slots=None, check_pool=True):
    if snapshot.max_sprites != self.S:
# ... 86 lines not shown
```

Measured before the change: 79.48 million.

## Cache per-env task evaluation results and reuse them when sprites did not move

Result: faster. 81.41 million (median of 6 runs) (+2.4%).

```diff
diff --git a/include/swb.h b/include/swb.h
--- a/include/swb.h
+++ b/include/swb.h
@@ -319,6 +319,8 @@
 int swb_frame_stats(swb_handle h, int64_t* copied, int64_t* filled, int64_t* resampled, void* stream);
 int swb_frame_cycles(swb_handle h, int64_t* out3, void* stream);
 
+int swb_task_stats(swb_handle h, int64_t* reused, int64_t* evaluated, void* stream);
+
 int swb_split_stats(swb_handle h, int64_t* whole, int64_t* bands, int64_t* whole_copies, void* stream);
 
 int swb_factors(swb_handle h, double* factors_dev, void* stream);
@@ -372,6 +374,7 @@
   int64_t frame_cache_bytes;
   int32_t split_bands;
   int32_t split_pad_;
+  int64_t task_cache_bytes;
 } swb_variant_info;
 int swb_variant(swb_handle h, swb_variant_info* out);
 const char* swb_build_id(void);
diff --git a/spriteworld_amd/_abi.py b/spriteworld_amd/_abi.py
--- a/spriteworld_amd/_abi.py
+++ b/spriteworld_amd/_abi.py
@@ -173,7 +173,7 @@
               ('n_column_groups', C.c_int32), ('run_cap', C.c_int32), ('paint_in_cover', C.c_int32),
               ('arena_units', C.c_int32), ('large_frames', C.c_int32), ('many_sprites', C.c_int32), ('reserved_', C.c_int32),
               ('run_list_bytes', C.c_int64), ('frame_cache_bytes', C.c_int64),
-              ('split_bands', C.c_int32), ('split_pad_', C.c_int32)]
+              ('split_bands', C.c_int32), ('split_pad_', C.c_int32), ('task_cache_bytes', C.c_int64)]
 
 
 FACTOR_UNIFORM_F32, FACTOR_UNIFORM_INT, FACTOR_DISCRETE = 0, 1, 2
@@ -375,6 +375,7 @@
                                    _P(SwbRolloutSampledOutputs), _h]),
     'swb_trim_run_lists': (None, [_h, _P(_i32), _h]),
     'swb_list_stats': (None, [_h, _P(C.c_int64), _P(C.c_int64), _h]),
+    'swb_task_stats': (None, [_h, _P(C.c_int64), _P(C.c_int64), _h]),
     'swb_frame_stats': (None, [_h, _P(C.c_int64), _P(C.c_int64), _P(C.c_int64), _h]),
     'swb_split_stats': (None, [_h, _P(C.c_int64), _P(C.c_int64), _P(C.c_int64), _h]),
     'swb_frame_cycles': (None, [_h, _P(C.c_int64), _h]),
diff --git a/spriteworld_amd/csrc/swb.hip b/spriteworld_amd/csrc/swb.hip
--- a/spriteworld_amd/csrc/swb.hip
+++ b/spriteworld_amd/csrc/swb.hip
@@ -133,6 +133,9 @@
   dev_buf<uint8_t> d_frame_cache;
   int copy_cost = 0;
   dev_buf<unsigned long long> d_frame_stats;
+  dev_buf<swb_task_record> d_task_cache;
+  uint32_t task_epoch = 1;
+  dev_buf<unsigned long long> d_task_stats;
   bool split_bands = false;
   dev_buf<unsigned long long> d_split_stats;
   dev_buf<int32_t> d_band_y0, d_band_first, d_band_lo, d_cg_lo, d_cg_hi;
@@ -207,6 +210,11 @@
   if (++h->list_epoch == 0u) h->list_epoch = 1u;
 }
 
+void bump_state_epochs(swb_engine* h) {
+  bump_list_epoch(h);
+  if (++h->task_epoch == 0u) h->task_epoch = 1u;
+}
+
 int ensure_overflow_slots(swb_engine* h, kernel_fn fn, kernel_fn fn_alt, size_t lds_bytes) {
   if (h->d_ovf) return 0;
   int per_cu = 0;
@@ -356,6 +364,11 @@
   p.success = out ? out->success : nullptr;
   p.error = out ? out->error : nullptr;
   p.render_only = render_only;
+  if (render_only == 0) {
+    p.task_cache = h->d_task_cache.ptr;
+    p.task_stats = h->d_task_stats.ptr;
+    p.task_epoch = h->task_epoch;
+  }
   return p;
 }
 
@@ -363,6 +376,7 @@
   if (!view) return;
   p->x = view->x; p->y = view->y; p->nspr = view->nspr; p->entry = view->entry; p->step_count = view->step_count;
   p->episode = view->episode; p->pool_base = view->pool_base; p->pool_len = view->pool_len; p->reset_next = view->reset_next;
+  p->task_cache = nullptr; p->task_stats = nullptr;
 }
 
 int cover_launch_config(const swb_engine* h, const variant* v, kernel_fn fn, swb_params* p, size_t* lds_out) {
@@ -927,7 +941,7 @@
       h->d_step_count.fill(nullptr, p.N) || h->d_episode.fill(nullptr, p.N) || h->d_reset_next.fill(nullptr, p.N))
     return SWB_ERR_HIP;
   if (getenv("SWB_LIST_STATS")) {
-    if (h->d_list_stats.fill(nullptr, 2) || h->d_frame_stats.fill(nullptr, 6)) return SWB_ERR_HIP;
+    if (h->d_list_stats.fill(nullptr, 2) || h->d_frame_stats.fill(nullptr, 6) || h->d_task_stats.fill(nullptr, 2)) return SWB_ERR_HIP;
     p.list_stats = h->d_list_stats;
     p.frame_stats = h->d_frame_stats;
     if (h->split_bands) {
@@ -947,6 +961,16 @@
       (void)hipGetLastError();
     }
   }
+  if (!getenv("SWB_NO_TASK_CACHE")) {
+    const size_t bytes = (size_t)p.N * sizeof(swb_task_record);
+    if (hipMalloc(reinterpret_cast<void**>(&h->d_task_cache.ptr), bytes) == hipSuccess && hipMemset(h->d_task_cache.ptr, 0, bytes) == hipSuccess) {
+      h->d_task_cache.count = (size_t)p.N;
+    } else {
+      if (h->d_task_cache.ptr) (void)hipFree(h->d_task_cache.ptr);
+      h->d_task_cache.ptr = nullptr;
+      (void)hipGetLastError();
+    }
+  }
   p.max_spans = SWB_MIN_SPANS;
   if (const char* ms = getenv("SWB_MAX_SPANS")) p.max_spans = atoi(ms) < SWB_MIN_SPANS ? SWB_MIN_SPANS : atoi(ms);
   p.span_cap = p.max_spans;
@@ -970,7 +994,7 @@
 
 int swb_upload_shapes(swb_handle h, const double* verts, const int32_t* offsets, int32_t n_shapes) {
   if (!h || !verts || !offsets) return fail(SWB_ERR_INVALID, "null argument");
-  bump_list_epoch(h);
+  bump_state_epochs(h);
   if (n_shapes < 1 || n_shapes > SWB_MAX_SHAPES) return fail(SWB_ERR_INVALID, "n_shapes must be in [1, %d]", SWB_MAX_SHAPES);
   HIP_TRY(hipSetDevice(h->device));
   int maxv = 0;
@@ -1088,7 +1112,7 @@
 
 int swb_set_pool(swb_handle h, const swb_pool* pool) {
   if (!h || !pool) return fail(SWB_ERR_INVALID, "null argument");
-  bump_list_epoch(h);
+  bump_state_epochs(h);
   HIP_TRY(hipSetDevice(h->device));
   const int P = pool->n_entries, S = h->p.S, T = h->p.n_tasks, N = h->p.N;
   if (P < 1) return fail(SWB_ERR_INVALID, "pool is empty");
@@ -1153,7 +1177,7 @@
 int swb_sample_pool(swb_handle h, const swb_sampler* spec, int32_t n_entries, const int32_t* pool_base_host,
                     const int32_t* pool_len_host, uint64_t seed, uint64_t first_entry, void* stream) {
   if (!h || !spec || !pool_base_host || !pool_len_host) return fail(SWB_ERR_INVALID, "null argument");
-  bump_list_epoch(h);
+  bump_state_epochs(h);
   HIP_TRY(hipSetDevice(h->device));
   const int P = n_entries, S = h->p.S, N = h->p.N;
   if (P < 1) return fail(SWB_ERR_INVALID, "pool is empty");
@@ -1241,7 +1265,7 @@
 
 int swb_resample_pool(swb_handle h, uint64_t seed, uint64_t first_entry, void* stream) {
   if (!h) return fail(SWB_ERR_INVALID, "null handle");
-  bump_list_epoch(h);
+  bump_state_epochs(h);
   if (!h->have_pool || !h->pool_sampled) return fail(SWB_ERR_STATE, "swb_sample_pool has not been called");
   if (!h->pool_uniform)
     return fail(SWB_ERR_STATE, "swb_resample_pool needs the env-major layout pool_base[n] = n * pool_len, equal pool_len");
@@ -1258,7 +1282,7 @@
 int swb_sample_pool_tree(swb_handle h, const swb_tree_sampler* spec, int32_t n_entries, const int32_t* pool_base_host,
                          const int32_t* pool_len_host, uint64_t seed, uint64_t first_entry, void* stream) {
   if (!h || !spec || !pool_base_host || !pool_len_host) return fail(SWB_ERR_INVALID, "null argument");
-  bump_list_epoch(h);
+  bump_state_epochs(h);
   HIP_TRY(hipSetDevice(h->device));
   const int P = n_entries, S = h->p.S, N = h->p.N;
   if (P < 1) return fail(SWB_ERR_INVALID, "pool is empty");
@@ -1697,6 +1721,17 @@
   return SWB_OK;
 }
 
+int swb_task_stats(swb_handle h, int64_t* reused, int64_t* evaluated, void* stream) {
+  if (!h || !reused || !evaluated) return fail(SWB_ERR_INVALID, "null argument");
+  if (!h->d_task_stats) return fail(SWB_ERR_STATE, "swb_task_stats: SWB_LIST_STATS was not set when the handle was created");
+  HIP_TRY(hipSetDevice(h->device));
+  HIP_TRY(hipStreamSynchronize((hipStream_t)stream));
+  unsigned long long w[2] = {0ull, 0ull};
+  HIP_TRY(hipMemcpy(w, h->d_task_stats, sizeof(w), hipMemcpyDeviceToHost));
+  *reused = (int64_t)w[0]; *evaluated = (int64_t)w[1];
+  return SWB_OK;
+}
+
 int swb_frame_stats(swb_handle h, int64_t* copied, int64_t* filled, int64_t* resampled, void* stream) {
   if (!h || !copied || !filled || !resampled) return fail(SWB_ERR_INVALID, "null argument");
   if (!h->d_frame_stats) return fail(SWB_ERR_STATE, "swb_frame_stats: SWB_LIST_STATS was not set when the handle was created");
@@ -1786,7 +1821,7 @@
 
 int swb_set_positions(swb_handle h, const double* x_host, const double* y_host, void* stream) {
   if (!h || !x_host || !y_host) return fail(SWB_ERR_INVALID, "null argument");
-  bump_list_epoch(h);
+  bump_state_epochs(h);
   HIP_TRY(hipSetDevice(h->device));
   HIP_TRY(hipStreamSynchronize((hipStream_t)stream));
   const size_t NS = (size_t)h->p.N * h->p.S;
@@ -1864,6 +1899,7 @@
                 "may have redrawn the entries it plays; pool_id = 0 skips the check)", (unsigned long long)pool_id,
                 (unsigned long long)h->pool_id);
   HIP_TRY(hipSetDevice(h->device));
+  if (++h->task_epoch == 0u) h->task_epoch = 1u;
   uint32_t* const rhdr = h->d_rhdr ? h->d_rhdr.ptr : nullptr;
   h->pool_uniform = false;
   const size_t threads = (size_t)h->p.N * h->p.S;
@@ -1923,7 +1959,7 @@
   if (have_angle) dst->d_p_angle.swap(t_angle);
   if (have_color) dst->d_p_color.swap(t_color);
   dst->d_pool_base.swap(t_base); dst->d_pool_len.swap(t_len);
-  bump_list_epoch(dst);
+  bump_state_epochs(dst);
   dst->rollout_stale = true;
   bind_pool(dst, have_angle, have_color);
   dst->pool_entries = P;
@@ -2063,7 +2099,7 @@
 int swb_set_sprite_attr(swb_handle h, int32_t env, int32_t sprite, int32_t attr, double value, const double* delta,
                         const int8_t* label, void* stream) {
   if (!h) return fail(SWB_ERR_INVALID, "null handle");
-  bump_list_epoch(h);
+  bump_state_epochs(h);
   if (!h->have_pool || !h->have_shapes) return fail(SWB_ERR_STATE, "no pool / shape table installed");
   if (env < 0 || env >= h->p.N) return fail(SWB_ERR_INVALID, "environment %d out of range", env);
   if (attr < SWB_ATTR_SHAPE || attr > SWB_ATTR_SCALE) return fail(SWB_ERR_INVALID, "unknown sprite attribute %d", attr);
@@ -2115,7 +2151,7 @@
 
 int swb_set_sprite_cell_labels(swb_handle h, int32_t env, int32_t sprite, const int8_t* cells, void* stream) {
   if (!h || !cells) return fail(SWB_ERR_INVALID, "null argument");
-  bump_list_epoch(h);
+  bump_state_epochs(h);
   if (!h->keyed) return fail(SWB_ERR_INVALID, "no task of this handle keys on position");
   if (env < 0 || env >= h->p.N || sprite < 0 || sprite >= h->p.S) return fail(SWB_ERR_INVALID, "environment %d / sprite %d out of range", env, sprite);
   HIP_TRY(hipSetDevice(h->device));
@@ -2153,6 +2189,7 @@
 
 int swb_variant(swb_handle h, swb_variant_info* out) {
   if (!h || !out) return fail(SWB_ERR_INVALID, "null argument");
+  out->task_cache_bytes = (int64_t)(h->d_task_cache.count * sizeof(swb_task_record));
   if (h->large_frames) {
     const variant* v0 = &kVariants[0];
     out->nw = v0->nw; out->ncol = 1; out->vs = 0;
diff --git a/spriteworld_amd/csrc/swb_kernels.hip.inc b/spriteworld_amd/csrc/swb_kernels.hip.inc
--- a/spriteworld_amd/csrc/swb_kernels.hip.inc
+++ b/spriteworld_amd/csrc/swb_kernels.hip.inc
@@ -30,6 +30,14 @@
 #define SWB_VSLOTS 8
 #define SWB_TUNED_SPRITES 16
 #define PRECISION_BITS 22
+
+struct swb_task_record {
+  uint32_t tr_lo, tr_hi;
+  uint8_t ok, err;
+  uint16_t pad_;
+  uint32_t stamp;
+};
+static_assert(sizeof(swb_task_record) == 16, "a task record is one 16-byte load");
 
 struct swb_params {
   int32_t N, S, AA;
@@ -128,6 +136,10 @@
   int32_t split_pad_;
   unsigned long long* split_stats;
   const uint8_t* active;
+  swb_task_record* task_cache;
+  uint32_t task_epoch;
+  uint32_t task_pad_;
+  unsigned long long* task_stats;
 };
 
 template <typename T>
@@ -447,13 +459,13 @@
 }
 
 template <typename SC>
-__device__ __forceinline__ int eval_task_wave(const swb_params& p, int n, double px, double py, const int8_t* label,
+__device__ __forceinline__ int eval_task_wave(const swb_params& p, int n_tasks, int n, double px, double py, const int8_t* label,
                                               SC* sc, double* reward, int* success) {
   const int l = lane_id();
   int err = 0;
   double r0 = 0.0;
   int ok0 = 0;
-  for (int t = 0; t < p.n_tasks; ++t) {
+  for (int t = 0; t < n_tasks; ++t) {
     const swb_task& tk = p.tasks[t];
     const int8_t* lab = label + t * p.S;
     double r = 0.0;
@@ -468,7 +480,7 @@
   const double* r = sc->tr;
   const int* ok = sc->tok;
   int succ = (p.meta_termination == SWB_TERM_ALL);
-  for (int t = 0; t < p.n_tasks; ++t) succ = (p.meta_termination == SWB_TERM_ALL) ? (succ && ok[t]) : (succ || ok[t]);
+  for (int t = 0; t < n_tasks; ++t) succ = (p.meta_termination == SWB_TERM_ALL) ? (succ && ok[t]) : (succ || ok[t]);
   double agg;
   const double qnan = __longlong_as_double(0x7ff8000000000000ll);
   if (p.meta_aggregator == SWB_AGG_SUM || p.meta_aggregator == SWB_AGG_MEAN) {
@@ -476,22 +488,22 @@
     double v[SWB_MAX_TASKS];
 #pragma unroll
     for (int t = 0; t < SWB_MAX_TASKS; ++t) {
-      const double x = (t < p.n_tasks) ? r[t] : 0.0;
+      const double x = (t < n_tasks) ? r[t] : 0.0;
       const bool isn = (x != x);
       v[t] = isn ? 0.0 : x;
-      cnt += (t < p.n_tasks) && !isn;
-    }
-    if (p.n_tasks < 8) {
+      cnt += (t < n_tasks) && !isn;
+    }
+    if (n_tasks < 8) {
       agg = -0.0;
 #pragma unroll
-      for (int t = 0; t < SWB_MAX_TASKS; ++t) if (t < p.n_tasks) agg = __dadd_rn(agg, v[t]);
+      for (int t = 0; t < SWB_MAX_TASKS; ++t) if (t < n_tasks) agg = __dadd_rn(agg, v[t]);
     } else {
       agg = __dadd_rn(__dadd_rn(__dadd_rn(v[0], v[1]), __dadd_rn(v[2], v[3])), __dadd_rn(__dadd_rn(v[4], v[5]), __dadd_rn(v[6], v[7])));
     }
     if (p.meta_aggregator == SWB_AGG_MEAN) agg = __ddiv_rn(agg, (double)cnt);
   } else {
     agg = qnan;
-    for (int t = 0; t < p.n_tasks; ++t) {
+    for (int t = 0; t < n_tasks; ++t) {
       if (r[t] != r[t]) continue;
       if (agg != agg) agg = r[t];
       else if (p.meta_aggregator == SWB_AGG_MAX ? (r[t] > agg) : (r[t] < agg)) agg = r[t];
@@ -662,7 +674,19 @@
   return step_cost{cost, cost_f32, cost_is_f32, step_count, changed};
 }
 
-template <bool OV, typename SC>
+__device__ __forceinline__ uint32_t load_task_record(const swb_params& p, int env) {
+  const int l = lane_id();
+  uint32_t w = 0u;
+  if (p.task_cache != nullptr && l < 4) w = reinterpret_cast<const uint32_t*>(p.task_cache)[4 * (size_t)env + l];
+  return w;
+}
+template <typename SC>
+__device__ __forceinline__ void park_task_record(const swb_params& p, uint32_t w, SC* tscratch) {
+  static_assert(sizeof(SC::pres) == sizeof(swb_task_record), "the record waits in task_scratch::pres");
+  if (p.task_cache != nullptr && lane_id() < 4) tscratch->pres[lane_id()] = w;
+}
+
+template <bool OV, bool CACHE = true, typename SC>
 __device__ __forceinline__ uint32_t finish_step(const swb_params& p, int env, const env_state& es, const step_cost& c, SC* tscratch) {
   const int l = lane_id(), S = p.S, n = es.n;
   const double px = es.px, py = es.py;
@@ -685,8 +709,35 @@
   const bool oof_l = (l < n) && !(px >= 0. && py >= 0. && px <= 1. && py <= 1.);
   const int oof = __ballot(oof_l) != 0ull;
   double tr = 0.0; int ok = 0;
-  const int terr = eval_task_wave(p, n, px, py, tscratch->labels, tscratch, &tr, &ok);
+  int n_tasks = p.n_tasks;
+  if constexpr (CACHE) {
+    if (p.task_cache != nullptr) {
+      const uint32_t stamp = tscratch->pres[3];
+      if (__ballot(stamp != p.task_epoch || c.changed || es.first) == 0ull) n_tasks = -1;
+    }
+  }
+  int terr = eval_task_wave(p, n_tasks, n, px, py, tscratch->labels, tscratch, &tr, &ok);
+  const bool reuse = CACHE && n_tasks < 0;
+  if constexpr (CACHE) {
+    if (reuse) {
+      const uint32_t w0 = tscratch->pres[0], w1 = tscratch->pres[1], w2 = tscratch->pres[2];
+      tr = __longlong_as_double((long long)(((unsigned long long)w1 << 32) | w0));
+      ok = (int)(w2 & 0xffu);
+      terr = (int)((w2 >> 8) & 0xffu);
+    }
+  }
   if (l == 0) {
+    if constexpr (CACHE) {
+      if (p.task_cache != nullptr && !reuse) {
+        const unsigned long long trb = (unsigned long long)__double_as_longlong(tr);
+        uint4 rec;
+        rec.x = (uint32_t)trb; rec.y = (uint32_t)(trb >> 32);
+        rec.z = (uint32_t)(ok & 0xff) | ((uint32_t)(terr & 0xff) << 8);
+        rec.w = p.task_epoch;
+        *reinterpret_cast<uint4*>(&p.task_cache[env]) = rec;
+      }
+      if (p.task_stats != nullptr) atomicAdd(&p.task_stats[reuse ? 0 : 1], 1ull);
+    }
     if (p.success) p.success[env] = (uint8_t)ok;
     if (p.render_only) {
     } else if (es.first) {
@@ -1631,7 +1682,9 @@
   if constexpr (!PAINT) {
     if (p.list_epoch != 0u && l <= SWB_MAX_CG + 2) L->outrow[l] = p.rhdr[(size_t)env * SWB_RHDR_DWORDS + SWB_RHDR_COST + l];
   }
+  const uint32_t task_rec_l = load_task_record(p, env);
   env_state es = load_env_state<OV>(p, env, tscratch);
+  park_task_record(p, task_rec_l, tscratch);
   const int n = es.n, nv_l = es.nv_l;
   const double scale_l = es.scale_l;
   uint32_t rgb_reg = 0u;
@@ -2490,7 +2543,9 @@
   swb_ms_lds* M = reinterpret_cast<swb_ms_lds*>(smem);
   task_scratch_t<SWB_MAX_SPRITES>* tscratch = &M->ts;
   double2* cpath = M->path;
+  const uint32_t task_rec_l = load_task_record(p, env);
   env_state es = load_env_state<OV>(p, env, tscratch);
+  park_task_record(p, task_rec_l, tscratch);
   auto hit = [&](int s2, double tx, double ty) __attribute__((always_inline)) {
     const int nv = __builtin_amdgcn_readlane(es.nv_l, s2), so = __builtin_amdgcn_readlane(es.so_l, s2);
     const double sc = readlane_d(es.scale_l, s2), ca = readlane_d(es.ca_l, s2), sa = readlane_d(es.sa_l, s2);
@@ -2702,7 +2757,7 @@
       return contains_point_wave(cpath, nv, tx, ty);
     };
     const step_cost sc = act_and_move(q, v, es, hit);
-    err |= finish_step<false>(q, v, es, sc, tscratch);
+    err |= finish_step<false, false>(q, v, es, sc, tscratch);
     if constexpr (KEEP) {
       const size_t slot = (size_t)k * gridDim.x + v;
       ep += es.first ? 1 : 0;
diff --git a/spriteworld_amd/engine.py b/spriteworld_amd/engine.py
--- a/spriteworld_amd/engine.py
+++ b/spriteworld_amd/engine.py
@@ -375,6 +375,11 @@
     self._check(self.lib.swb_list_stats(self._h, C.byref(kept), C.byref(built), self._stream()))
     return kept.value, built.value
 
+  def task_stats(self):
+    reused, evaluated = C.c_int64(0), C.c_int64(0)
+    self._check(self.lib.swb_task_stats(self._h, C.byref(reused), C.byref(evaluated), self._stream()))
+    return reused.value, evaluated.value
+
   def frame_stats(self):
     w = [C.c_int64(0) for _ in range(3)]
     self._check(self.lib.swb_frame_stats(self._h, C.byref(w[0]), C.byref(w[1]), C.byref(w[2]), self._stream()))
```
